# POSTECH-CVLab/PyTorch-StudioGAN

Hardware: AMD Instinct MI355X
Metric: images/sec (G+D step) BigGAN ImageNet-128 bs256 (higher is better)
Workload: dtype bf16

## Files before the change

### include/sgamd.h

```cpp
#ifndef SGAMD_H
#define SGAMD_H
#include <stdint.h>
#ifdef __cplusplus
extern "C" {
#endif

typedef void* sg_stream_t;

#define SG_DTYPE_F32 0
#define SG_DTYPE_BF16 1
#define SG_DTYPE_F64 2

#define SG_PIX_RELU 1
#define SG_PIX_UPSAMPLE 2
#define SG_PIX_QUAD 4
#define SG_PIX_TRANSPOSED 8
#define SG_EPI_OUT_F32 1
#define SG_EPI_ATOMIC 2
#define SG_EPI_POOL 4
#define SG_EPI_RELU 8
#define SG_EPI_RES_F32 16

const char* sg_last_error(void);
int sg_version(void);
int sg_prof_enable(int on);
int sg_prof_collect(double* out, int nkinds);

typedef struct {
  int dtype;
  int N, Hs, Ws, C, ldx;
  int Ho, Wo, Cout;
  int R, S, stride, pad_h, pad_w;
  int pix_flags, epi_flags;
  float alpha, beta;
  const void* x; const void* w;
  const float* bias; const void* res; const void* mask; void* out; const float* alpha_ptr;
  int ldo, ldr, ldm;
} sg_conv_fwd_desc;
int sg_conv2d_fwd(const sg_conv_fwd_desc* d, sg_stream_t stream);
int sg_set_f32_mode(int mode);
int sg_get_f32_mode(void);
long long sg_f32_split_launches(int mode);

typedef struct {
  sg_conv_fwd_desc main;
  const void* x2; const void* w2; const float* bias2;
  int C2, ldx2, x2_up;
  float* stats;
} sg_conv_skip_desc;
int sg_conv2d_fwd_skip_stat_rows(const sg_conv_skip_desc* d);
int sg_conv2d_fwd_skip(const sg_conv_skip_desc* d, sg_stream_t stream);
int sg_conv2d_fwd_skip_ok(const sg_conv_skip_desc* d);
long long sg_conv_rs_launches(void);

#define SG_Q_POOL 0
#define SG_Q_UP 1
typedef struct {
  int dtype, form;
  int N, Hl, Wl;
  int C, ldx, Cout;
  int pix_flags, epi_flags;
  float alpha, beta;
  const void* x; const void* wq;
  const float* bias; const void* res; const void* mask; void* out; const float* alpha_ptr;
  int ldo, ldr, ldm;
  const void* x2; const void* w2q; const float* bias2;
  int C2, ldx2;
  float* stats;
  int x2_norelu;
} sg_convq_desc;
int sg_conv2d_q_stat_rows(const sg_convq_desc* d);
int sg_conv2d_q(const sg_convq_desc* d, sg_stream_t stream);
int sg_conv2d_q_ok(const sg_convq_desc* d);
int sg_quad_pack(int dtype, int mode, const void* src, void* dst, int M, int Cs, sg_stream_t stream);
typedef struct { const void* src; void* dst; int M, Cs, mode, pad_; } sg_quad_item;
int sg_quad_pack_batch(int dtype, const sg_quad_item* items_dev, const sg_quad_item* items_host, int n, sg_stream_t stream);
typedef struct {
  int dtype, form;
  int N, Hl, Wl;
  int C, ldx, x_flags;
  int Cout, ldg;
  float alpha; const float* alpha_ptr;
  const void* x; const void* dy; float* dw; float* dbias;
  float* work; long long work_floats;
  int splits;
} sg_convq_wgrad_desc;
int sg_conv2d_q_wgrad_plan(const sg_convq_wgrad_desc* d, int* splits, long long* work_floats);
int sg_conv2d_q_wgrad(const sg_convq_wgrad_desc* d, sg_stream_t stream);
int sg_prof_collect_ex(double* out, int nkinds);
int sg_prof_collect_tags(double* out, int ntags);

typedef struct {
  int dtype;
  int N;
  int xHs, xWs, C, ldx, x_flags;
  int gHs, gWs, Cout, ldg, g_flags;
  int Ho, Wo;
  int R, S, stride, pad_h, pad_w;
  float alpha;
  const void* x; const void* dy; float* dw;
  const float* alpha_ptr;
  int splits;
  int no_tr;
  float* work; long long work_floats;
  float* dbias;
} sg_conv_wgrad_desc;
int sg_conv2d_wgrad(const sg_conv_wgrad_desc* d, sg_stream_t stream);
int sg_conv2d_wgrad_fuses_bias(const sg_conv_wgrad_desc* d);
int sg_conv2d_wgrad_plan(const sg_conv_wgrad_desc* d, int* splits, long long* work_floats);

typedef struct {
  int dtype, p_form, q_form;
  int I, J, K, batch;
  const void* p; long long p_bstride; int ldp;
  const void* q; long long q_bstride; int ldq;
  void* out; long long out_bstride; int ldo;
  const float* bias; const void* res; long long res_bstride; int ldr; float beta;
  float alpha; const float* alpha_ptr;
  int epi_flags; int splits; int no_tr;
} sg_gemm_desc;
int sg_gemm(const sg_gemm_desc* d, sg_stream_t stream);
typedef struct { const float* w; const float* y; const float* bias; float* out; int rows, K, ldy, ldo; } sg_linear_item;
int sg_linear_group(const sg_linear_item* items_dev, const sg_linear_item* items_host, int n, int B, sg_stream_t stream);

int sg_nchw_to_nhwc(int dtype, const float* src, void* dst, int N, int C, int H, int W, int ldo, sg_stream_t s);
int sg_nhwc_to_nchw(int dtype, const void* src, float* dst, int N, int C, int H, int W, int lds, int apply_tanh, sg_stream_t s);
int sg_nchw_grad_to_nhwc(int dtype, const float* dy, const float* y, void* dst, int N, int C, int H, int W, int ldo, int apply_tanh, sg_stream_t s);
int sg_avgpool2_fwd(int dtype, const void* x, void* y, int N, int H, int W, int C, sg_stream_t s);
int sg_avgpool2_bwd(int dtype, const void* dy, void* dx, int N, int H, int W, int C, sg_stream_t s);
int sg_maxpool2_fwd(int dtype, const void* x, int ldx, void* y, int ldy, uint8_t* idx, int N, int H, int W, int C, sg_stream_t s);
int sg_maxpool2_bwd(int dtype, const void* dy, int ldy, const uint8_t* idx, void* dx, int ldx, int N, int H, int W, int C, sg_stream_t s);
int sg_softmax_rows(int dtype, const float* s_in, void* p_out, long long rows, int cols, sg_stream_t st);
int sg_softmax_rows_bwd(int dtype, const void* p, const float* dp, void* ds, long long rows, int cols, sg_stream_t st);
int sg_convert(int src_dtype, int dst_dtype, const void* x, void* y, long long n, sg_stream_t s);
int sg_add_relu(int dtype, const void* a, const void* x, void* out, long long n, sg_stream_t s);
int sg_relu_mask(int dtype, const void* dy, const void* x, void* dx, long long n, sg_stream_t s);
int sg_axpby(int dtype, const void* x, void* y, long long n, float a, float b, sg_stream_t s);
int sg_dot(int dtype, const void* x, const void* y, long long n, float* out, float scale, const float* scale_ptr, sg_stream_t s);
int sg_colsum(int dtype, const void* x, int ldx, const void* mask, int ldm, long long rows, int C, float* out, float alpha, sg_stream_t s);

int sg_bn_partial_stats(int dtype, const void* x, int ldx, long long rows, int C, double* partial, sg_stream_t s);
int sg_bn_stats_from_tiles(const float* stats, int nrows, int C, double* partial, sg_stream_t s);
int sg_bn_finalize(const double* partial, double count, int C, float eps, float momentum, float* mean, float* invstd,
                   float* running_mean, float* running_var, sg_stream_t s);
typedef void* sg_comm_t;
int sg_comm_unique_id(void* out128);
int sg_comm_init_rank(const void* id128, int nranks, int rank, sg_comm_t* comm);
int sg_comm_size(sg_comm_t comm, int* nranks);
int sg_comm_destroy(sg_comm_t comm);
int sg_allreduce_flat(sg_comm_t comm, void* buf, long long count, int dtype, sg_stream_t s);
int sg_bn_stats_sync(int dtype, const void* x, int ldx, long long rows, int C, double* partial, sg_comm_t comm, float eps, float momentum,
                     float* mean, float* invstd, float* running_mean, float* running_var, sg_stream_t s);
int sg_reduce_scatter_flat(sg_comm_t comm, float* buf, long long per_rank, sg_stream_t s);
int sg_allgather_flat(sg_comm_t comm, float* buf, long long per_rank, sg_stream_t s);

typedef void* sg_p2p_t;
int sg_p2p_create(int world, int rank, long long max_doubles, sg_p2p_t* out, void* handle_out64);
int sg_p2p_connect(sg_p2p_t p, const void* handles);
int sg_p2p_destroy(sg_p2p_t p);
int sg_p2p_timeouts(sg_p2p_t p, int* count);
int sg_p2p_allreduce_f64(sg_p2p_t p, double* buf, int n, sg_stream_t s);
int sg_bn_finalize_p2p(sg_p2p_t p, const double* partial, double count, int C, float eps, float momentum, float* mean, float* invstd,
                       float* running_mean, float* running_var, sg_stream_t s);
int sg_bn_stats_sync_p2p(int dtype, const void* x, int ldx, long long rows, int C, double* partial, sg_p2p_t p, float eps, float momentum,
                         float* mean, float* invstd, float* running_mean, float* running_var, sg_stream_t s);
int sg_bn_from_running(const float* running_mean, const float* running_var, int C, float eps, float* mean, float* invstd, sg_stream_t s);
int sg_bn_apply(int dtype, const void* x, void* y, int N, long long HW, int C, const float* mean, const float* invstd,
                const float* gain, const float* bias, int gb_stride_n, int relu, sg_stream_t s);
int sg_bn_bwd_reduce(int dtype, const void* x, const void* dy, int N, long long HW, int C, const float* mean, const float* invstd,
                     const float* gain, const float* bias, int gb_stride_n, int relu, float* sums, sg_stream_t s);
int sg_bn_bwd_finalize(const float* sums, int N, int C, const float* gain, int gb_stride_n, float* dgain, float* dbias,
                       double* chan, sg_stream_t s);
int sg_bn_bwd_apply(int dtype, const void* x, const void* dy, void* dx, int N, long long HW, int C, const float* mean,
                    const float* invstd, const float* gain, const float* bias, int gb_stride_n, int relu,
                    const double* chan, double count, int use_batch_stats, sg_stream_t s);
int sg_bn_bwd_apply_res(int dtype, const void* x, const void* dy, void* dx, int N, long long HW, int C, const float* mean,
                        const float* invstd, const float* gain, const float* bias, int gb_stride_n, int relu,
                        const double* chan, double count, int use_batch_stats, const void* res, sg_stream_t s);

int sg_bn_bwd2_reduce(int dtype, const void* x, const void* dy, const void* u, int N, long long HW, int C, const float* mean,
                      const float* invstd, const float* gain, const float* bias, int relu, float* sums, sg_stream_t s);
int sg_bn_bwd2_finalize(const float* sums, int N, int C, double* chan, sg_stream_t s);
int sg_bn_bwd2_dgain(const double* chan_local, const double* chan, double count, const float* invstd, int C,
                     int use_batch_stats, float* dgain, sg_stream_t s);
int sg_bn_bwd2_apply(int dtype, const void* x, const void* dy, const void* u, void* g_dy, void* g_x, int N, long long HW, int C,
                     const float* mean, const float* invstd, const float* gain, const float* bias, int relu, const double* chan,
                     double count, int use_batch_stats, sg_stream_t s);

typedef struct {
  const float* w;
  float* u; float* v;
  float* sigma;
  float* u_snap; float* v_snap;
  void* w_fwd;
  void* w_dgrad;
  float* w_f32;
  int rows, cols;
  int Cin, RS;
  int do_power_iter;
  int apply_sn;
  int rows_pad;
  long long work_off;
  int trans;
  int dgrad_noflip;
  int Cin_pad;
} sg_sn_layer;
int sg_sn_forward(int dtype, const sg_sn_layer* layers_dev, const sg_sn_layer* layers_host, int n, float eps, float* work, long long work_floats, sg_stream_t s);

typedef struct {
  const float* dwt;
  const float* w;
  const float* u; const float* v; const float* sigma;
  float* dw;
  int rows, cols, Cin, RS, natural, apply_sn, trans;
  int Cin_pad;
} sg_sn_bwd_layer;
int sg_sn_backward(const sg_sn_bwd_layer* layers_dev, const sg_sn_bwd_layer* layers_host, int n, float* work, long long work_floats, sg_stream_t s);

int sg_embedding_fwd(const float* table, const int64_t* idx, float* out, int B, int dim, int num, sg_stream_t s);
int sg_embedding_bwd(const float* dout, const int64_t* idx, float* dtable, int B, int dim, int num, sg_stream_t s);
int sg_relu_sum_hw_fwd(int dtype, const void* x, float* h, int B, int HW, int C, sg_stream_t s);
int sg_relu_sum_hw_bwd(int dtype, const void* x, const float* dh, void* dx, int B, int HW, int C, sg_stream_t s);
int sg_pd_head_fwd(const float* h, const float* w1, const float* b1, const float* emb, float* adv, int B, int C, sg_stream_t s);
int sg_pd_head_bwd(const float* h, const float* w1, const float* emb, const float* dadv, float* dh, float* dw1, float* db1,
                   float* demb, int B, int C, sg_stream_t s);
int sg_loss_d(int kind, const float* real, const float* fake, int B, float* loss, float* d_real, float* d_fake, sg_stream_t s);
int sg_loss_g(int kind, const float* fake, int B, float* loss, float* d_fake, sg_stream_t s);

int sg_interp_rows(const float* real, const float* fake, const float* alpha, float* out, int B, long long n, sg_stream_t s);
int sg_gp_fwd(int kind, const float* grads, int B, long long n, float* norms, float* loss, sg_stream_t s);
int sg_gp_bwd(int kind, const float* grads, const float* norms, const float* gout, float* dgrads, int B, long long n, sg_stream_t s);
int sg_masked_sum_hw(int dtype, const void* t, const void* x, float* out, int B, int HW, int C, sg_stream_t s);

int sg_attn_fwd_flash_ok(int B, int HW, int HW4, int Dp, int Cg);
int sg_attn_fwd_fused(const void* theta, const void* phi, const void* g, float* lse, void* O, float* O32, int B, int HW, int HW4, int Dp, int Cg, sg_stream_t s);
int sg_attn_bwd_fused_ok(int B, int HW, int HW4, int Dp, int Cg);
int sg_attn_bwd_fused(const void* theta, const void* phi, const void* g, const void* dO, const float* O32, const float* lse, float* delta, void* dtheta, void* dphi,
                      void* dg, int B, int HW, int HW4, int Dp, int Cg, sg_stream_t s);

int sg_attn_proj_ok(int B, int H, int W, int C, int ldx, int Dp, int Cg);
int sg_attn_proj_fwd(const void* x, int ldx, const void* w_theta, const void* w_phi, const void* w_g, void* theta, void* phi, void* g,
                     uint8_t* idx_phi, uint8_t* idx_g, int B, int H, int W, int C, int Dp, int Cg, int relu, sg_stream_t s);
int sg_attn_proj_bwd_data(const void* dtheta, const void* dphi, const void* dg, const uint8_t* idx_phi, const uint8_t* idx_g, const void* wd_theta,
                          const void* wd_phi, const void* wd_g, const void* res, void* dx, int B, int H, int W, int C, int Dp, int Cg, sg_stream_t s);

int sg_slice_up_fwd(int dtype, const void* x, void* y, int N, int Hs, int Ws, int ldx, int C, int up, sg_stream_t s);
int sg_slice_up_bwd(int dtype, const void* dy, void* dx, int N, int Hs, int Ws, int ldx, int C, int up, sg_stream_t s);
int sg_copy_channels(int dtype, const void* src, int ld_src, void* dst, int ld_dst, long long rows, int C, sg_stream_t s);

int sg_adam_ema(float* p, const float* g, float* m, float* v, float* ema, long long n, float lr, float beta1, float beta2,
                float eps, float wd, int step, float ema_decay, float grad_scale, sg_stream_t s);
int sg_ema_lerp(const float* src, float* ema, long long n, float decay, sg_stream_t s);

int sg_lecam(const float* real, const float* fake, int B, float ema_real, float ema_fake, float* loss, float* d_real, float* d_fake, sg_stream_t s);
int sg_u8_to_nhwc(int dtype, const uint8_t* x, const uint8_t* flip, void* y, int N, int H, int W, int cpad, sg_stream_t s);

int sg_quantize_resize_normalize(int dtype, const float* x, void* out, uint8_t* quant_out, int N, int C, int H, int W,
                                 int OH, int OW, int quantize, sg_stream_t s);
int sg_quantize_resize_normalize_ms(int dtype, const float* x, void* out, uint8_t* quant_out, int N, int C, int H, int W,
                                    int OH, int OW, int quantize, const float* mean, const float* std, sg_stream_t s);
int sg_pool2d(int dtype, const void* x, void* y, int N, int H, int W, int C, int k, int stride, int pad, int mode, int ldy, int c_off, sg_stream_t s);
int sg_pil_resize_normalize(int dtype, const float* x, void* out, float* tmp, int N, int C, int H, int W, int OH, int OW,
                            const int* bounds_h, const double* kk_h, int ksize_h, const int* bounds_v, const double* kk_v, int ksize_v,
                            int quantize, sg_stream_t s);
int sg_pil_resize_normalize_ms(int dtype, const float* x, void* out, float* tmp, int N, int C, int H, int W, int OH, int OW,
                               const int* bounds_h, const double* kk_h, int ksize_h, const int* bounds_v, const double* kk_v, int ksize_v,
                               int quantize, const float* mean, const float* std, sg_stream_t s);
int sg_global_avgpool(int dtype, const void* x, float* y, int N, int HW, int C, sg_stream_t s);
int sg_topk_hits(const float* scores, int ld, int ncls, const int64_t* labels, int k, int N, uint8_t* hits, sg_stream_t s);
int sg_topk_select(const float* x, int n, int k, float* vals, int* idx, sg_stream_t s);
int sg_topk_scatter(const float* g, const int* idx, int k, float* dx, int n, sg_stream_t s);
int sg_feat_moments_accumulate(const float* f, int n, int C, double* sum_f, double* sum_ff, sg_stream_t s);
int sg_gather_images_u8(const uint8_t* src, const int64_t* idx, const uint8_t* flip, uint8_t* dst, int B, int H, int W,
                        const int64_t* lab_src, int64_t* lab_dst, sg_stream_t s);
int sg_row_normalize_fwd(const float* x, float* y, float* inv, int rows, int cols, float eps, sg_stream_t s);
int sg_row_normalize_bwd(const float* y, const float* inv, const float* dy, float* dx, int rows, int cols, sg_stream_t s);
int sg_row_dot(const float* a, const float* b, float* p, int rows, int cols, sg_stream_t s);
int sg_row_scale(const float* g, const float* x, float* out, int rows, int cols, int accumulate, sg_stream_t s);
int sg_class_loss(int kind, const float* z, const int64_t* label, int rows, int cols, float* row_loss, float* loss, float* dz, sg_stream_t s);
int sg_contrastive_loss(int kind, const float* S, const float* p, const int64_t* label, int B, float temperature, float m_p,
                        float* row_loss, float* loss, float* dS, float* dp, sg_stream_t s);
int sg_gather_cols(const float* z, const int64_t* label, int rows, int cols, float* out, sg_stream_t s);
int sg_scatter_cols(const float* g, const int64_t* label, int rows, int cols, float* dz, sg_stream_t s);
int sg_layernorm_rows(int out_dtype, const float* x, long long pitch, const float* gamma, const float* beta, void* y, long long ldo, int rows, int C,
                      float eps, sg_stream_t s);
int sg_vit_tokens(const float* patch, const float* cls, const float* pos, float* x, int B, int N, int C, sg_stream_t s);
int sg_gelu_f32(const float* x, float* y, long long n, sg_stream_t s);
int sg_tok_gemm(int epi, const void* a, int lda, const void* w, const float* bias, void* out, int ldo, int M, int N, int K, sg_stream_t s);
int sg_mha_fwd_ok(int B, int N, int H, int D);
int sg_mha_fwd(const void* qkv, void* out, int B, int N, int H, int D, float scale, sg_stream_t s);
long long sg_tok_gemm_launches(void);
long long sg_mha_launches(void);

int sg_row_sqnorm(const float* f, int n, int C, float* sq, sg_stream_t s);
int sg_kth_smallest_rows(const float* D, long long ld, int rows, int cols, int k, const float* row_add, float* out, sg_stream_t s);
int sg_prdc_rows(const float* D, long long ld, int rows, int cols, const float* row_add, const float* r2_row, const float* r2_col,
                 int* col_cnt, uint8_t* row_any, float* row_min, sg_stream_t s);
int sg_chol_lower(double* A, int n, int* flag, sg_stream_t s);
int sg_dgemm_tn(const double* A, const double* B, double* C, int n, sg_stream_t s);
int sg_jacobi_sweep(double* M, int n, double* offd, sg_stream_t s);
int sg_row_norm_sum(const double* M, int n, double* out, sg_stream_t s);

int sg_bias_act(int dtype, const void* x, const void* b, const void* xref, const void* yref, const void* dy, void* y, long long n,
                long long step_b, int size_b, int grad, int act, float alpha, float gain, float clamp, sg_stream_t s);
int sg_upfirdn2d(int dtype, const void* x, const float* f, void* y, int planes, int H, int W, int fh, int fw, int upx, int upy,
                 int downx, int downy, int padx0, int padx1, int pady0, int pady1, int flip_filter, float gain, sg_stream_t s);
int sg_filtered_lrelu(int dtype, const void* x, const float* fu, const float* fd, const void* b, void* y, int N, int C, int H, int W,
                      int fu_n, int fd_n, int up, int down, int px0, int px1, int py0, int py1, float gain, float slope, float clamp,
                      int flip_filter, sg_stream_t s);

#define SG_AUG_BRIGHTNESS 1
#define SG_AUG_SATURATION 2
#define SG_AUG_CONTRAST 4
#define SG_AUG_FLIP 8
#define SG_AUG_TRANSLATE 16
#define SG_AUG_TRANSLATE_REFLECT 32
#define SG_AUG_CUTOUT 64
typedef struct {
  int N, C, H, W;
  int ops;
  int cut_h, cut_w;
  int max_t;
  const float* color;
  const int* geom;
} sg_aug_desc;
int sg_augment_work_floats(const sg_aug_desc* d);
int sg_augment_fwd(const sg_aug_desc* d, const float* x, float* y, float* work, sg_stream_t s);
int sg_augment_bwd(const sg_aug_desc* d, const float* dy, float* dx, float* work, sg_stream_t s);
int sg_mse_work_floats(void);
int sg_mse_fwd(const float* a, const float* b, long long n, float* work, float* loss, sg_stream_t s);
int sg_mse_bwd(const float* a, const float* b, const float* gout, long long n, float* da, float* db, sg_stream_t s);
int sg_loss_ls_d(const float* real, const float* fake, int B, float* loss, float* d_real, float* d_fake, sg_stream_t s);
int sg_loss_ls_g(const float* fake, int B, float* loss, float* d_fake, sg_stream_t s);
int sg_fm_work_floats(int C);
int sg_fm_loss(const float* real_h, const float* fake_h, int B, int C, float* work, float* loss, float* d_fake, sg_stream_t s);
int sg_exp_fwd(const float* x, float* y, long long n, sg_stream_t s);
int sg_exp_bwd(const float* dy, const float* y, float* dx, long long n, sg_stream_t s);
int sg_normal_nll(const float* x, const float* mu, const float* var, int B, int K, float* loss, float* dmu, float* dvar, sg_stream_t s);
int sg_maxpool2_gather(int dtype, const void* x, int ldx, const uint8_t* idx, void* y, int ldy, int N, int H, int W, int C, sg_stream_t s);
int sg_softmax_rows_bwd2(const float* P, const float* dP, const float* u, float* gP, long long rows, int cols, sg_stream_t s);
int sg_scale_by_ptr(int dtype, const void* x, const float* sigma, void* y, long long n, sg_stream_t s);
int sg_tanh_bwd(const float* dy, const float* y, float* t, long long n, sg_stream_t s);
int sg_tanh_bwd2(const float* g, const float* dy, const float* y, float* out, long long n, sg_stream_t s);
int sg_clamp_flat(float* p, long long n, float lo, float hi, sg_stream_t s);
int sg_select_rows(const uint8_t* flag, const float* a, const float* b, float* out, int N, long long row, sg_stream_t s);
int sg_sign_count(const float* logit, int B, float* acc, sg_stream_t s);
int sg_reflect_pad2d_fwd(const float* x, float* y, int planes, int H, int W, int l, int r, int t, int b, sg_stream_t s);
int sg_reflect_pad2d_bwd(const float* dy, float* dx, int planes, int H, int W, int l, int r, int t, int b, sg_stream_t s);
int sg_affine_sample_fwd(const float* x, const float* theta, float* y, int N, int C, int Hi, int Wi, int Ho, int Wo, sg_stream_t s);
int sg_affine_sample_bwd(const float* dy, const float* theta, float* dx, int N, int C, int Hi, int Wi, int Ho, int Wo, sg_stream_t s);
int sg_color_affine(const float* x, const float* M, float* y, int N, int C, int HW, int transpose, sg_stream_t s);
int sg_fir_reflect(const float* x, const float* taps, float* y, int N, int C, int H, int W, int T, int axis, int transpose, sg_stream_t s);
int sg_ada_noise_cutout(const float* x, const float* noise, const float* sigma, const float* cut, float* y, int N, int C, int H, int W, sg_stream_t s);

#ifdef __cplusplus
}
#endif
#endif
```

### pytorch-studiogan_amd/_lib.py

```python
import ctypes as C
import os
import subprocess
import sys

import torch

_HERE = os.path.dirname(os.path.abspath(__file__))
LIB_PATH = os.path.join(_HERE, "libsgamd.so")
if os.environ.get("SG_LIBSGAMD"):
    LIB_PATH = os.path.abspath(os.environ["SG_LIBSGAMD"])
CSRC = os.path.join(_HERE, "csrc")

F32, BF16, F64 = 0, 1, 2
PIX_RELU, PIX_UPSAMPLE, PIX_QUAD, PIX_TRANSPOSED = 1, 2, 4, 8
Q_POOL, Q_UP = 0, 1
EPI_OUT_F32, EPI_ATOMIC, EPI_POOL, EPI_RELU, EPI_RES_F32 = 1, 2, 4, 8, 16

_vp, _i, _f, _ll = C.c_void_p, C.c_int, C.c_float, C.c_longlong


class ConvFwdDesc(C.Structure):
    _fields_ = [("dtype", _i), ("N", _i), ("Hs", _i), ("Ws", _i), ("C", _i), ("ldx", _i), ("Ho", _i), ("Wo", _i), ("Cout", _i),
                ("R", _i), ("S", _i), ("stride", _i), ("pad_h", _i), ("pad_w", _i), ("pix_flags", _i), ("epi_flags", _i),
                ("alpha", _f), ("beta", _f), ("x", _vp), ("w", _vp), ("bias", _vp), ("res", _vp), ("mask", _vp), ("out", _vp),
                ("alpha_ptr", _vp), ("ldo", _i), ("ldr", _i), ("ldm", _i)]


class ConvSkipDesc(C.Structure):
    _fields_ = [("main", ConvFwdDesc), ("x2", _vp), ("w2", _vp), ("bias2", _vp), ("C2", _i), ("ldx2", _i), ("x2_up", _i), ("stats", _vp)]


class ConvWgradDesc(C.Structure):
    _fields_ = [("dtype", _i), ("N", _i), ("xHs", _i), ("xWs", _i), ("C", _i), ("ldx", _i), ("x_flags", _i), ("gHs", _i), ("gWs", _i),
                ("Cout", _i), ("ldg", _i), ("g_flags", _i), ("Ho", _i), ("Wo", _i), ("R", _i), ("S", _i), ("stride", _i),
                ("pad_h", _i), ("pad_w", _i), ("alpha", _f), ("x", _vp), ("dy", _vp), ("dw", _vp), ("alpha_ptr", _vp),
                ("splits", _i), ("no_tr", _i), ("work", _vp), ("work_floats", _ll), ("dbias", _vp)]


class ConvQDesc(C.Structure):
    _fields_ = [("dtype", _i), ("form", _i), ("N", _i), ("Hl", _i), ("Wl", _i), ("C", _i), ("ldx", _i), ("Cout", _i),
                ("pix_flags", _i), ("epi_flags", _i), ("alpha", _f), ("beta", _f), ("x", _vp), ("wq", _vp), ("bias", _vp), ("res", _vp),
                ("mask", _vp), ("out", _vp), ("alpha_ptr", _vp), ("ldo", _i), ("ldr", _i), ("ldm", _i),
                ("x2", _vp), ("w2q", _vp), ("bias2", _vp), ("C2", _i), ("ldx2", _i), ("stats", _vp), ("x2_norelu", _i)]


class ConvQWgradDesc(C.Structure):
    _fields_ = [("dtype", _i), ("form", _i), ("N", _i), ("Hl", _i), ("Wl", _i), ("C", _i), ("ldx", _i), ("x_flags", _i), ("Cout", _i),
                ("ldg", _i), ("alpha", _f), ("alpha_ptr", _vp), ("x", _vp), ("dy", _vp), ("dw", _vp), ("dbias", _vp), ("work", _vp),
                ("work_floats", _ll), ("splits", _i)]


class QuadItem(C.Structure):
    _fields_ = [("src", _vp), ("dst", _vp), ("M", _i), ("Cs", _i), ("mode", _i), ("pad_", _i)]


class LinearItem(C.Structure):
    _fields_ = [("w", _vp), ("y", _vp), ("bias", _vp), ("out", _vp), ("rows", _i), ("K", _i), ("ldy", _i), ("ldo", _i)]


class GemmDesc(C.Structure):
    _fields_ = [("dtype", _i), ("p_form", _i), ("q_form", _i), ("I", _i), ("J", _i), ("K", _i), ("batch", _i),
                ("p", _vp), ("p_bstride", _ll), ("ldp", _i), ("q", _vp), ("q_bstride", _ll), ("ldq", _i),
                ("out", _vp), ("out_bstride", _ll), ("ldo", _i), ("bias", _vp), ("res", _vp), ("res_bstride", _ll), ("ldr", _i),
                ("beta", _f), ("alpha", _f), ("alpha_ptr", _vp), ("epi_flags", _i), ("splits", _i), ("no_tr", _i)]


class SnLayer(C.Structure):
    _fields_ = [("w", _vp), ("u", _vp), ("v", _vp), ("sigma", _vp), ("u_snap", _vp), ("v_snap", _vp), ("w_fwd", _vp), ("w_dgrad", _vp),
                ("w_f32", _vp), ("rows", _i), ("cols", _i), ("Cin", _i), ("RS", _i), ("do_power_iter", _i), ("apply_sn", _i),
                ("rows_pad", _i), ("work_off", _ll), ("trans", _i), ("dgrad_noflip", _i), ("Cin_pad", _i)]


class SnBwdLayer(C.Structure):
    _fields_ = [("dwt", _vp), ("w", _vp), ("u", _vp), ("v", _vp), ("sigma", _vp), ("dw", _vp), ("rows", _i), ("cols", _i),
                ("Cin", _i), ("RS", _i), ("natural", _i), ("apply_sn", _i), ("trans", _i), ("Cin_pad", _i)]


class AugDesc(C.Structure):
    _fields_ = [("N", _i), ("C", _i), ("H", _i), ("W", _i), ("ops", _i), ("cut_h", _i), ("cut_w", _i), ("max_t", _i), ("color", _vp), ("geom", _vp)]


AUG_BRIGHTNESS, AUG_SATURATION, AUG_CONTRAST, AUG_FLIP, AUG_TRANSLATE, AUG_TRANSLATE_REFLECT, AUG_CUTOUT = 1, 2, 4, 8, 16, 32, 64

_lib = None


def build(force=False, verbose=False):
    cmd = ["make", "-C", CSRC, "-j", str(max(2, os.cpu_count() or 2))]
    if force:
        subprocess.run(["make", "-C", CSRC, "clean"], check=True, stdout=subprocess.DEVNULL)
    res = subprocess.run(cmd, stdout=subprocess.PIPE, stderr=subprocess.STDOUT, text=True)
    if verbose or res.returncode != 0:
        sys.stderr.write(res.stdout)
    if res.returncode != 0:
        raise RuntimeError("building libsgamd.so failed")
    return LIB_PATH


_PROTOS = {
    "sg_prof_enable": [_i],
    "sg_prof_collect": [C.POINTER(C.c_double), _i],
    "sg_conv2d_fwd": [C.POINTER(ConvFwdDesc), _vp],
    "sg_conv2d_fwd_skip": [C.POINTER(ConvSkipDesc), _vp],
    "sg_conv2d_fwd_skip_ok": [C.POINTER(ConvSkipDesc)],
    "sg_conv_rs_launches": [],
    "sg_conv2d_q": [C.POINTER(ConvQDesc), _vp],
    "sg_conv2d_q_ok": [C.POINTER(ConvQDesc)],
    "sg_conv2d_q_stat_rows": [C.POINTER(ConvQDesc)],
    "sg_conv2d_fwd_skip_stat_rows": [C.POINTER(ConvSkipDesc)],
    "sg_bn_stats_from_tiles": [_vp, _i, _i, _vp, _vp],
    "sg_quad_pack": [_i, _i, _vp, _vp, _i, _i, _vp],
    "sg_quad_pack_batch": [_i, _vp, C.POINTER(QuadItem), _i, _vp],
    "sg_linear_group": [_vp, C.POINTER(LinearItem), _i, _i, _vp],
    "sg_conv2d_q_wgrad_plan": [C.POINTER(ConvQWgradDesc), C.POINTER(_i), C.POINTER(_ll)],
    "sg_conv2d_q_wgrad": [C.POINTER(ConvQWgradDesc), _vp],
    "sg_prof_collect_ex": [C.POINTER(C.c_double), _i],
    "sg_prof_collect_tags": [C.POINTER(C.c_double), _i],
    "sg_conv2d_wgrad": [C.POINTER(ConvWgradDesc), _vp],
    "sg_conv2d_wgrad_plan": [C.POINTER(ConvWgradDesc), C.POINTER(_i), C.POINTER(_ll)],
    "sg_conv2d_wgrad_fuses_bias": [C.POINTER(ConvWgradDesc)],
    "sg_gemm": [C.POINTER(GemmDesc), _vp],
    "sg_nchw_to_nhwc": [_i, _vp, _vp, _i, _i, _i, _i, _i, _vp],
    "sg_nhwc_to_nchw": [_i, _vp, _vp, _i, _i, _i, _i, _i, _i, _vp],
    "sg_nchw_grad_to_nhwc": [_i, _vp, _vp, _vp, _i, _i, _i, _i, _i, _i, _vp],
    "sg_avgpool2_fwd": [_i, _vp, _vp, _i, _i, _i, _i, _vp],
    "sg_avgpool2_bwd": [_i, _vp, _vp, _i, _i, _i, _i, _vp],
    "sg_maxpool2_fwd": [_i, _vp, _i, _vp, _i, _vp, _i, _i, _i, _i, _vp],
    "sg_maxpool2_bwd": [_i, _vp, _i, _vp, _vp, _i, _i, _i, _i, _i, _vp],
    "sg_softmax_rows": [_i, _vp, _vp, _ll, _i, _vp],
    "sg_softmax_rows_bwd": [_i, _vp, _vp, _vp, _ll, _i, _vp],
    "sg_axpby": [_i, _vp, _vp, _ll, _f, _f, _vp],
    "sg_convert": [_i, _i, _vp, _vp, _ll, _vp],
    "sg_add_relu": [_i, _vp, _vp, _vp, _ll, _vp],
    "sg_relu_mask": [_i, _vp, _vp, _vp, _ll, _vp],
    "sg_dot": [_i, _vp, _vp, _ll, _vp, _f, _vp, _vp],
    "sg_colsum": [_i, _vp, _i, _vp, _i, _ll, _i, _vp, _f, _vp],
    "sg_bn_partial_stats": [_i, _vp, _i, _ll, _i, _vp, _vp],
    "sg_bn_finalize": [_vp, C.c_double, _i, _f, _f, _vp, _vp, _vp, _vp, _vp],
    "sg_comm_unique_id": [_vp],
    "sg_comm_init_rank": [_vp, _i, _i, C.POINTER(_vp)],
    "sg_comm_size": [_vp, C.POINTER(_i)],
    "sg_comm_destroy": [_vp],
    "sg_allreduce_flat": [_vp, _vp, _ll, _i, _vp],
    "sg_bn_stats_sync": [_i, _vp, _i, _ll, _i, _vp, _vp, _f, _f, _vp, _vp, _vp, _vp, _vp],
    "sg_set_f32_mode": [_i],
    "sg_get_f32_mode": [],
    "sg_f32_split_launches": [_i],
    "sg_reduce_scatter_flat": [_vp, _vp, _ll, _vp],
    "sg_allgather_flat": [_vp, _vp, _ll, _vp],
    "sg_p2p_create": [_i, _i, _ll, C.POINTER(_vp), _vp],
    "sg_p2p_connect": [_vp, _vp],
    "sg_p2p_destroy": [_vp],
    "sg_p2p_timeouts": [_vp, C.POINTER(_i)],
    "sg_p2p_allreduce_f64": [_vp, _vp, _i, _vp],
    "sg_bn_finalize_p2p": [_vp, _vp, C.c_double, _i, _f, _f, _vp, _vp, _vp, _vp, _vp],
    "sg_bn_stats_sync_p2p": [_i, _vp, _i, _ll, _i, _vp, _vp, _f, _f, _vp, _vp, _vp, _vp, _vp],
    "sg_bn_from_running": [_vp, _vp, _i, _f, _vp, _vp, _vp],
    "sg_bn_apply": [_i, _vp, _vp, _i, _ll, _i, _vp, _vp, _vp, _vp, _i, _i, _vp],
    "sg_bn_bwd_reduce": [_i, _vp, _vp, _i, _ll, _i, _vp, _vp, _vp, _vp, _i, _i, _vp, _vp],
    "sg_bn_bwd_finalize": [_vp, _i, _i, _vp, _i, _vp, _vp, _vp, _vp],
    "sg_bn_bwd_apply": [_i, _vp, _vp, _vp, _i, _ll, _i, _vp, _vp, _vp, _vp, _i, _i, _vp, C.c_double, _i, _vp],
    "sg_bn_bwd_apply_res": [_i, _vp, _vp, _vp, _i, _ll, _i, _vp, _vp, _vp, _vp, _i, _i, _vp, C.c_double, _i, _vp, _vp],
    "sg_bn_bwd2_reduce": [_i, _vp, _vp, _vp, _i, _ll, _i, _vp, _vp, _vp, _vp, _i, _vp, _vp],
    "sg_bn_bwd2_finalize": [_vp, _i, _i, _vp, _vp],
    "sg_bn_bwd2_dgain": [_vp, _vp, C.c_double, _vp, _i, _i, _vp, _vp],
    "sg_bn_bwd2_apply": [_i, _vp, _vp, _vp, _vp, _vp, _i, _ll, _i, _vp, _vp, _vp, _vp, _i, _vp, C.c_double, _i, _vp],
    "sg_attn_fwd_flash_ok": [_i, _i, _i, _i, _i],
    "sg_attn_fwd_fused": [_vp, _vp, _vp, _vp, _vp, _vp, _i, _i, _i, _i, _i, _vp],
    "sg_attn_bwd_fused_ok": [_i, _i, _i, _i, _i],
    "sg_attn_bwd_fused": [_vp, _vp, _vp, _vp, _vp, _vp, _vp, _vp, _vp, _vp, _i, _i, _i, _i, _i, _vp],
    "sg_attn_proj_ok": [_i, _i, _i, _i, _i, _i, _i],
    "sg_attn_proj_fwd": [_vp, _i, _vp, _vp, _vp, _vp, _vp, _vp, _vp, _vp, _i, _i, _i, _i, _i, _i, _i, _vp],
    "sg_attn_proj_bwd_data": [_vp, _vp, _vp, _vp, _vp, _vp, _vp, _vp, _vp, _vp, _i, _i, _i, _i, _i, _i, _vp],
    "sg_slice_up_fwd": [_i, _vp, _vp, _i, _i, _i, _i, _i, _i, _vp],
    "sg_slice_up_bwd": [_i, _vp, _vp, _i, _i, _i, _i, _i, _i, _vp],
    "sg_copy_channels": [_i, _vp, _i, _vp, _i, _ll, _i, _vp],
    "sg_interp_rows": [_vp, _vp, _vp, _vp, _i, _ll, _vp],
    "sg_gp_fwd": [_i, _vp, _i, _ll, _vp, _vp, _vp],
    "sg_gp_bwd": [_i, _vp, _vp, _vp, _vp, _i, _ll, _vp],
    "sg_masked_sum_hw": [_i, _vp, _vp, _vp, _i, _i, _i, _vp],
    "sg_sn_forward": [_i, _vp, C.POINTER(SnLayer), _i, _f, _vp, _ll, _vp],
    "sg_sn_backward": [_vp, C.POINTER(SnBwdLayer), _i, _vp, _ll, _vp],
    "sg_embedding_fwd": [_vp, _vp, _vp, _i, _i, _i, _vp],
    "sg_embedding_bwd": [_vp, _vp, _vp, _i, _i, _i, _vp],
    "sg_relu_sum_hw_fwd": [_i, _vp, _vp, _i, _i, _i, _vp],
    "sg_relu_sum_hw_bwd": [_i, _vp, _vp, _vp, _i, _i, _i, _vp],
    "sg_pd_head_fwd": [_vp, _vp, _vp, _vp, _vp, _i, _i, _vp],
    "sg_pd_head_bwd": [_vp, _vp, _vp, _vp, _vp, _vp, _vp, _vp, _i, _i, _vp],
    "sg_loss_d": [_i, _vp, _vp, _i, _vp, _vp, _vp, _vp],
    "sg_loss_g": [_i, _vp, _i, _vp, _vp, _vp],
    "sg_adam_ema": [_vp, _vp, _vp, _vp, _vp, _ll, _f, _f, _f, _f, _f, _i, _f, _f, _vp],
    "sg_ema_lerp": [_vp, _vp, _ll, _f, _vp],
    "sg_quantize_resize_normalize": [_i, _vp, _vp, _vp, _i, _i, _i, _i, _i, _i, _i, _vp],
    "sg_pil_resize_normalize": [_i, _vp, _vp, _vp, _i, _i, _i, _i, _i, _i, _vp, _vp, _i, _vp, _vp, _i, _i, _vp],
    "sg_quantize_resize_normalize_ms": [_i, _vp, _vp, _vp, _i, _i, _i, _i, _i, _i, _i, C.POINTER(_f), C.POINTER(_f), _vp],
    "sg_pil_resize_normalize_ms": [_i, _vp, _vp, _vp, _i, _i, _i, _i, _i, _i, _vp, _vp, _i, _vp, _vp, _i, _i, C.POINTER(_f), C.POINTER(_f), _vp],
    "sg_layernorm_rows": [_i, _vp, _ll, _vp, _vp, _vp, _ll, _i, _i, _f, _vp],
    "sg_vit_tokens": [_vp, _vp, _vp, _vp, _i, _i, _i, _vp],
    "sg_gelu_f32": [_vp, _vp, _ll, _vp],
    "sg_tok_gemm": [_i, _vp, _i, _vp, _vp, _vp, _i, _i, _i, _i, _vp],
    "sg_mha_fwd_ok": [_i, _i, _i, _i],
    "sg_mha_fwd": [_vp, _vp, _i, _i, _i, _i, _f, _vp],
    "sg_tok_gemm_launches": [],
    "sg_mha_launches": [],
    "sg_pool2d": [_i, _vp, _vp, _i, _i, _i, _i, _i, _i, _i, _i, _i, _i, _vp],
    "sg_global_avgpool": [_i, _vp, _vp, _i, _i, _i, _vp],
    "sg_feat_moments_accumulate": [_vp, _i, _i, _vp, _vp, _vp],
    "sg_topk_hits": [_vp, _i, _i, _vp, _i, _i, _vp, _vp],
    "sg_row_normalize_fwd": [_vp, _vp, _vp, _i, _i, _f, _vp],
    "sg_row_normalize_bwd": [_vp, _vp, _vp, _vp, _i, _i, _vp],
    "sg_row_dot": [_vp, _vp, _vp, _i, _i, _vp],
    "sg_row_scale": [_vp, _vp, _vp, _i, _i, _i, _vp],
    "sg_class_loss": [_i, _vp, _vp, _i, _i, _vp, _vp, _vp, _vp],
    "sg_contrastive_loss": [_i, _vp, _vp, _vp, _i, _f, _f, _vp, _vp, _vp, _vp, _vp],
    "sg_gather_cols": [_vp, _vp, _i, _i, _vp, _vp],
    "sg_scatter_cols": [_vp, _vp, _i, _i, _vp, _vp],
    "sg_chol_lower": [_vp, _i, _vp, _vp],
    "sg_dgemm_tn": [_vp, _vp, _vp, _i, _vp],
    "sg_jacobi_sweep": [_vp, _i, _vp, _vp],
    "sg_row_norm_sum": [_vp, _i, _vp, _vp],
    "sg_row_sqnorm": [_vp, _i, _i, _vp, _vp],
    "sg_kth_smallest_rows": [_vp, _ll, _i, _i, _i, _vp, _vp, _vp],
    "sg_prdc_rows": [_vp, _ll, _i, _i, _vp, _vp, _vp, _vp, _vp, _vp, _vp],
    "sg_topk_select": [_vp, _i, _i, _vp, _vp, _vp],
    "sg_lecam": [_vp, _vp, _i, _f, _f, _vp, _vp, _vp, _vp],
    "sg_u8_to_nhwc": [_i, _vp, _vp, _vp, _i, _i, _i, _i, _vp],
    "sg_gather_images_u8": [_vp, _vp, _vp, _vp, _i, _i, _i, _vp, _vp, _vp],
    "sg_topk_scatter": [_vp, _vp, _i, _vp, _i, _vp],
    "sg_bias_act": [_i, _vp, _vp, _vp, _vp, _vp, _vp, _ll, _ll, _i, _i, _i, _f, _f, _f, _vp],
    "sg_upfirdn2d": [_i, _vp, _vp, _vp, _i, _i, _i, _i, _i, _i, _i, _i, _i, _i, _i, _i, _i, _i, _f, _vp],
    "sg_filtered_lrelu": [_i, _vp, _vp, _vp, _vp, _vp, _i, _i, _i, _i, _i, _i, _i, _i, _i, _i, _i, _i, _f, _f, _f, _i, _vp],
    "sg_augment_work_floats": [C.POINTER(AugDesc)],
    "sg_augment_fwd": [C.POINTER(AugDesc), _vp, _vp, _vp, _vp],
    "sg_augment_bwd": [C.POINTER(AugDesc), _vp, _vp, _vp, _vp],
    "sg_mse_work_floats": [],
    "sg_mse_fwd": [_vp, _vp, _ll, _vp, _vp, _vp],
    "sg_mse_bwd": [_vp, _vp, _vp, _ll, _vp, _vp, _vp],
    "sg_loss_ls_d": [_vp, _vp, _i, _vp, _vp, _vp, _vp],
    "sg_loss_ls_g": [_vp, _i, _vp, _vp, _vp],
    "sg_fm_work_floats": [_i],
    "sg_fm_loss": [_vp, _vp, _i, _i, _vp, _vp, _vp, _vp],
    "sg_exp_fwd": [_vp, _vp, _ll, _vp],
    "sg_exp_bwd": [_vp, _vp, _vp, _ll, _vp],
    "sg_normal_nll": [_vp, _vp, _vp, _i, _i, _vp, _vp, _vp, _vp],
    "sg_maxpool2_gather": [_i, _vp, _i, _vp, _vp, _i, _i, _i, _i, _i, _vp],
    "sg_softmax_rows_bwd2": [_vp, _vp, _vp, _vp, _ll, _i, _vp],
    "sg_scale_by_ptr": [_i, _vp, _vp, _vp, _ll, _vp],
    "sg_tanh_bwd": [_vp, _vp, _vp, _ll, _vp],
    "sg_tanh_bwd2": [_vp, _vp, _vp, _vp, _ll, _vp],
    "sg_clamp_flat": [_vp, _ll, _f, _f, _vp],
    "sg_select_rows": [_vp, _vp, _vp, _vp, _i, _ll, _vp],
    "sg_sign_count": [_vp, _i, _vp, _vp],
    "sg_reflect_pad2d_fwd": [_vp, _vp, _i, _i, _i, _i, _i, _i, _i, _vp],
    "sg_reflect_pad2d_bwd": [_vp, _vp, _i, _i, _i, _i, _i, _i, _i, _vp],
    "sg_affine_sample_fwd": [_vp, _vp, _vp, _i, _i, _i, _i, _i, _i, _vp],
    "sg_affine_sample_bwd": [_vp, _vp, _vp, _i, _i, _i, _i, _i, _i, _vp],
    "sg_color_affine": [_vp, _vp, _vp, _i, _i, _i, _i, _vp],
    "sg_fir_reflect": [_vp, _vp, _vp, _i, _i, _i, _i, _i, _i, _i, _vp],
    "sg_ada_noise_cutout": [_vp, _vp, _vp, _vp, _vp, _i, _i, _i, _i, _vp],
}


def exported_symbols():
    return sorted(list(_PROTOS.keys()) + ["sg_last_error", "sg_version"])


def lib():
    global _lib
    if _lib is None:
        if not os.path.exists(LIB_PATH):
            raise RuntimeError(
                f"{LIB_PATH} is missing: run `python -c 'import __graft_entry__ as g; g.build()'` (make -C {CSRC}). "
                "There is no CPU/eager fallback on the product path.")
        l = C.CDLL(LIB_PATH)
        l.sg_last_error.restype = C.c_char_p
        l.sg_version.restype = _i
        for name, args in _PROTOS.items():
            fn = getattr(l, name)
            fn.argtypes = args
            fn.restype = _i
        l.sg_conv_rs_launches.restype = _ll
        l.sg_tok_gemm_launches.restype = _ll
        l.sg_mha_launches.restype = _ll
        l.sg_f32_split_launches.restype = _ll
        f32_mode = {"bf16x3": 3, "bf16x6": 6}.get(os.environ.get("SG_F32_MODE", "exact"), 0)
        if f32_mode:
            l.sg_set_f32_mode(f32_mode)
        _lib = l
    return _lib


def check(rc, name=""):
    if rc != 0:
        raise RuntimeError(f"{name}: {lib().sg_last_error().decode()} (rc={rc})")


_STATE_WRITERS = frozenset(("sg_adam_ema", "sg_ema_lerp", "sg_allreduce_flat", "sg_clamp_flat", "sg_allgather_flat"))
write_epoch = [0]


def call(name, *args):
    if name in _STATE_WRITERS:
        write_epoch[0] += 1
    rc = getattr(lib(), name)(*args)
    if rc != 0:
        raise RuntimeError(f"{name}: {lib().sg_last_error().decode()} (rc={rc})")


def stream():
    return torch.cuda.current_stream().cuda_stream


def upload_bytes(raw, device):
    t = torch.frombuffer(bytearray(raw), dtype=torch.uint8)
    if torch.device(device).type == "cuda":
        return t.pin_memory().to(device, non_blocking=True)
    return t.to(device)


def dt(t):
    d = t if isinstance(t, torch.dtype) else t.dtype
    if d == torch.float32:
        return F32
    if d == torch.bfloat16:
        return BF16
    raise RuntimeError(f"unsupported dtype {d} (float32 / bfloat16 only)")


def require_gpu(dev):
    if dev.type != "cuda":
        raise RuntimeError("studiogan_amd modules run on the GPU only (no CPU fallback on the product path)")


def ptr(t):
    if t is None:
        return None
    if not t.is_cuda:
        raise RuntimeError("studiogan_amd kernels need a GPU tensor (no CPU fallback on the product path)")
    return t.data_ptr()
```

### pytorch-studiogan_amd/csrc/conv.hip

```cpp
#include <type_traits>
#include "conv_common.h"
#include "conv_v2.h"

int g_sg_f32_mode = 0;
long long g_sg_f32_split_launches[2] = {0, 0};
extern "C" int sg_set_f32_mode(int mode) {
  SG_CHECK(mode == 0 || mode == 3 || mode == 6, "sg_set_f32_mode: 0 (exact fp32 MFMA), 3 (bf16x3 split) or 6 (bf16x6 split)");
  g_sg_f32_mode = mode;
  return 0;
}
extern "C" int sg_get_f32_mode() { return g_sg_f32_mode; }
extern "C" long long sg_f32_split_launches(int mode) {
  if (mode != 3 && mode != 6) return -1;
  return __atomic_load_n(&g_sg_f32_split_launches[mode == 6], __ATOMIC_RELAXED);
}

template <typename T, class LP, class LQ, int SPLIT>
static void conv_fwd_tiles(const LP& lp, const LQ& lq, const Epilogue<T>& e, int I, int J, int K, hipStream_t st) {
  if (I <= 32) sg_launch_gemm<T, LP, LQ, 32, 256, 1, 4, true, SPLIT>(lp, lq, e, I, J, K, 1, 1, st);
  else if (I % 128 != 0 && (I % 96 == 0 || (I < 128 && I > 64))) sg_launch_gemm<T, LP, LQ, 96, 256, 1, 4, true, SPLIT>(lp, lq, e, I, J, K, 1, 1, st);
  else sg_launch_gemm<T, LP, LQ, 128, 128, 2, 2, true, SPLIT>(lp, lq, e, I, J, K, 1, 1, st);
}

template <typename T, bool FAST>
static void conv_fwd_launch(const sg_conv_fwd_desc* d, const Epilogue<T>& e, int I, int J, int K, int pflags, hipStream_t st) {
  typedef StridedKC<T, FAST> LP;
  typedef ConvPixKC<T, FAST> LQ;
  LP lp;
  lp.base = (const T*)d->w; lp.bstride = 0; lp.ld = K; lp.rows = I; lp.K = K;
  lp.vec_ok = (K % ET<T>::VEC == 0) && aligned16(d->w);
  LQ lq;
  fill_geom<T>(lq.g, d->x, d->N, d->Hs, d->Ws, d->C, d->ldx, d->Ho, d->Wo, d->R, d->S, d->stride, d->pad_h, d->pad_w, pflags);
  lq.rows = J; lq.K = K;
  if constexpr (sizeof(T) == 4 && FAST) {
    const int mode = g_sg_f32_mode;
    if (mode == 3) { sg_f32_split_count(3); return conv_fwd_tiles<T, LP, LQ, 3>(lp, lq, e, I, J, K, st); }
    if (mode == 6) { sg_f32_split_count(6); return conv_fwd_tiles<T, LP, LQ, 6>(lp, lq, e, I, J, K, st); }
  }
  conv_fwd_tiles<T, LP, LQ, 0>(lp, lq, e, I, J, K, st);
}

static bool conv_fwd_v2_try(const ConvFwdProblem& pb, hipStream_t st) {
  const sg_conv_fwd_desc* d = pb.d;
  const int I = pb.I, J = pb.J, K = pb.K, pflags = pb.pflags;
  const char mode = env_mode("SG_CONV_V2");
  const bool force = mode == 'f';
  if (mode == '0' || (pflags & SG_PIX_TRANSPOSED)) return false;
  if (d->stride != 1 && (d->stride != 2 || (pflags & (SG_PIX_UPSAMPLE | SG_PIX_QUAD)))) return false;
  if (d->C % 8 || d->ldx % 8 || d->R * d->S > 25 || J < 256) return false;
  if (pb.xbytes >= (1ll << 31) || pb.wbytes >= (1ll << 30)) return false;
  if (!aligned16(d->x) || !aligned16(d->w)) return false;
  if (!epi_bf16_rows_ok(pb.e)) return false;
  const int tj = (J + 255) / 256;
  int best_tiles = 0;
  int best = cout_tile_search(I, tj, best_tiles);
  if (!best && I % 8 == 0 && I >= 32) {
    int best_pad = 0;
    for (int c = 0; c < 3; c++) {
      const int padded = ((I + kCoutTiles[c] - 1) / kCoutTiles[c]) * kCoutTiles[c];
      if (2 * padded > 3 * I) continue;
      const int tiles = (padded / kCoutTiles[c]) * tj;
      if (!best || padded < best_pad) { best = kCoutTiles[c]; best_pad = padded; best_tiles = tiles; }
    }
  }
  int min_tiles = 160;
  if (const char* mt = getenv("SG_CONV_V2_MIN_TILES")) { const int v = atoi(mt); if (v > 0) min_tiles = v; }
  if (!best || (best_tiles < min_tiles && !force)) return false;
  ConvV2Params p;
  p.x = (const bf16_t*)d->x; p.w = (const bf16_t*)d->w;
  p.N = d->N; p.Hs = d->Hs; p.Ws = d->Ws; p.C = d->C; p.ldx = d->ldx;
  p.Hin = d->Hs * (pb.up ? 2 : 1); p.Win = d->Ws * (pb.up ? 2 : 1); p.Ho = d->Ho; p.Wo = d->Wo;
  p.R = d->R; p.S = d->S; p.pad_h = d->pad_h; p.pad_w = d->pad_w; p.flags = pflags; p.stride = d->stride;
  p.I = I; p.J = J; p.K = K; p.cpt = d->C / 8; p.ntap = d->R * d->S;
  p.wshift = pb.wshift; p.hshift = pb.hshift;
  p.xbytes = (unsigned)pb.xbytes; p.wbytes = (unsigned)pb.wbytes;
  const Epilogue<bf16_t>& e = pb.e;
  int rc = 0;
  if (best == 192) rc = sg_launch_conv_v2<192, 4, 2, 256, 7>(p, e, st);
  else if (best == 128) rc = sg_launch_conv_v2<128, 4, 2, 256, 7>(p, e, st);
  else {
    if (J >= 512 * 256) rc = sg_launch_conv_v2<96, 8, 1, 512, 1>(p, e, st);
    else rc = sg_launch_conv_v2<96, 8, 1, 256, 1>(p, e, st);
  }
  return rc == 0;
}

template <typename T> static int conv_fwd_t(const sg_conv_fwd_desc* d, hipStream_t st) {
  const int K = d->R * d->S * d->C;
  const int I = d->Cout;
  const long long Jll = (long long)d->N * d->Ho * d->Wo;
  SG_CHECK(Jll < (1ll << 31), "sg_conv2d_fwd: too many output pixels");
  SG_CHECK((long long)d->N * d->Hs * d->Ws * d->ldx < (1ll << 31), "sg_conv2d_fwd: input tensor too large for 32-bit element offsets");
  const int J = (int)Jll;
  int pflags = d->pix_flags;
  if (d->epi_flags & SG_EPI_POOL) {
    SG_CHECK((d->Ho % 2 == 0) && (d->Wo % 2 == 0), "sg_conv2d_fwd: pooled output needs even Ho, Wo");
    pflags |= SG_PIX_QUAD;
  } else {
    pflags &= ~SG_PIX_QUAD;
  }
  const bool w_vec = (K % ET<T>::VEC == 0) && aligned16(d->w);
  const bool x_vec = (d->C % ET<T>::VEC == 0) && (d->ldx % ET<T>::VEC == 0) && aligned16(d->x);
  const Epilogue<T> e = make_epilogue<T>(d, I, J);
  const int prof = sg_prof_begin(st, 2.0 * (double)I * (double)J * (double)K, 0);
  int eng = SG_ENG_CONV_GEMM;
  if constexpr (std::is_same_v<T, bf16_t>) {
    if (w_vec && x_vec) {
      const ConvFwdProblem pb = conv_fwd_problem(d, e, I, J, K, pflags);
      if (sg_conv_fwd_sk_try(pb, st)) eng = SG_ENG_CONV_SK;
      else if (sg_conv_fwd_rs_try(pb, st)) eng = SG_ENG_CONV_RS;
      else if (sg_conv_fwd_v4_try(pb, st)) eng = SG_ENG_CONV_V4;
      else if (sg_conv_fwd_v3_try(pb, st)) eng = SG_ENG_CONV_V3;
      else if (conv_fwd_v2_try(pb, st)) eng = SG_ENG_CONV_V2;
    }
  }
  if (eng == SG_ENG_CONV_GEMM) {
    if (w_vec && x_vec) conv_fwd_launch<T, true>(d, e, I, J, K, pflags, st);
    else conv_fwd_launch<T, false>(d, e, I, J, K, pflags, st);
  }
  {
    const double es = sizeof(T), jout = (d->epi_flags & SG_EPI_POOL) ? (double)J / 4.0 : (double)J;
    const double b = es * ((double)d->N * d->Hs * d->Ws * d->C + (double)I * K + jout * I * (1.0 + (d->mask ? 1.0 : 0.0) + (d->res ? 1.0 : 0.0)));
    sg_prof_tag(prof, eng, b);
  }
  sg_prof_end(st, prof);
  SG_LAUNCH_CHECK();
  return 0;
}

static int conv_fwd_skip(const sg_conv_skip_desc* sk, hipStream_t st, bool dry) {
  const sg_conv_fwd_desc* d = &sk->main;
  if (d->dtype != SG_DTYPE_BF16 || d->R != 3 || d->S != 3 || d->stride != 1 || (d->pix_flags & (SG_PIX_UPSAMPLE | SG_PIX_TRANSPOSED))) return 0;
  const int K = 9 * d->C, I = d->Cout;
  const long long Jll = (long long)d->N * d->Ho * d->Wo;
  if (Jll >= (1ll << 31) || (long long)d->N * d->Hs * d->Ws * d->ldx >= (1ll << 31)) return 0;
  const int J = (int)Jll;
  int pflags = d->pix_flags;
  if (d->epi_flags & SG_EPI_POOL) { if ((d->Ho & 1) || (d->Wo & 1)) return 0; pflags |= SG_PIX_QUAD; } else pflags &= ~SG_PIX_QUAD;
  const ConvFwdProblem pb = conv_fwd_problem(d, make_epilogue<bf16_t>(d, I, J), I, J, K, pflags);
  if (dry) return sg_conv_fwd_v4_skip_try(pb, sk, st, true) ? 1 : 0;
  const int prof = sg_prof_begin(st, 2.0 * (double)I * (double)J * ((double)K + (double)sk->C2), 0);
  const bool ok = sg_conv_fwd_v4_skip_try(pb, sk, st, false);
  {
    const double jout = (d->epi_flags & SG_EPI_POOL) ? (double)J / 4.0 : (double)J;
    const double x2 = (double)d->N * (sk->x2_up ? (d->Ho / 2) * (d->Wo / 2) : d->Ho * d->Wo) * sk->C2;
    sg_prof_tag(prof, SG_ENG_CONV_V4_SKIP, 2.0 * ((double)d->N * d->Hs * d->Ws * d->C + x2 + (double)I * (K + sk->C2) + jout * I));
  }
  sg_prof_end(st, prof);
  return ok ? 1 : 0;
}
extern "C" int sg_conv2d_fwd_skip_stat_rows(const sg_conv_skip_desc* d) {
  if (!d) return 0;
  const long long J = (long long)d->main.N * d->main.Ho * d->main.Wo;
  return (int)((J + 255) / 256);
}
extern "C" int sg_conv2d_fwd_skip_ok(const sg_conv_skip_desc* d) {
  if (!d || !d->main.x || !d->main.w || !d->main.out || !d->x2 || !d->w2) return 0;
  return conv_fwd_skip(d, nullptr, true);
}
extern "C" int sg_conv2d_fwd_skip(const sg_conv_skip_desc* d, sg_stream_t stream) {
  SG_CHECK(d && d->main.x && d->main.w && d->main.out && d->x2 && d->w2, "sg_conv2d_fwd_skip: null pointer");
  SG_CHECK(conv_fwd_skip(d, (hipStream_t)stream, false) == 1, "sg_conv2d_fwd_skip: problem not eligible for the fused kernel (ask sg_conv2d_fwd_skip_ok first)");
  SG_LAUNCH_CHECK();
  return 0;
}

extern "C" int sg_conv2d_fwd(const sg_conv_fwd_desc* d, sg_stream_t stream) {
  SG_CHECK(d && d->x && d->w && d->out, "sg_conv2d_fwd: null pointer");
  SG_CHECK(d->N > 0 && d->C > 0 && d->Cout > 0 && d->R > 0 && d->S > 0 && d->stride > 0, "sg_conv2d_fwd: bad shape");
  SG_CHECK(!(d->epi_flags & SG_EPI_ATOMIC), "sg_conv2d_fwd: atomic epilogue not supported");
  if (d->dtype == SG_DTYPE_F32) return conv_fwd_t<float>(d, (hipStream_t)stream);
  if (d->dtype == SG_DTYPE_BF16) return conv_fwd_t<bf16_t>(d, (hipStream_t)stream);
  sg_set_error("sg_conv2d_fwd: bad dtype");
  return -1;
}
```

### pytorch-studiogan_amd/csrc/conv_common.h

```cpp
#pragma once
#include <stdlib.h>
#include "gemm_core.h"
#include "../../include/sgamd.h"

static inline int ilog2_exact(int v) {
  if (v <= 0 || (v & (v - 1))) return -1;
  int s = 0;
  while ((1 << s) < v) s++;
  return s;
}
static inline bool aligned16(const void* p) { return (((uintptr_t)p) & 15) == 0; }

template <typename T>
static void fill_geom(PixGeom<T>& g, const void* x, int N, int Hs, int Ws, int C, int ldx, int Ho, int Wo, int R, int S,
                      int stride, int pad_h, int pad_w, int flags) {
  g.x = (const T*)x; g.N = N; g.Hs = Hs; g.Ws = Ws;
  const int up = (flags & SG_PIX_UPSAMPLE) ? 2 : 1;
  g.Hin = Hs * up; g.Win = Ws * up; g.C = C; g.ldx = ldx; g.Ho = Ho; g.Wo = Wo;
  g.R = R; g.S = S; g.stride = stride; g.pad_h = pad_h; g.pad_w = pad_w; g.flags = flags;
  g.vec_ok = (C % ET<T>::VEC == 0) && (ldx % ET<T>::VEC == 0) && aligned16(x);
  g.wshift = ilog2_exact(Wo); g.hshift = ilog2_exact(Ho);
}

static inline char env_mode(const char* name) { const char* m = getenv(name); return m ? m[0] : 0; }

static inline long long bf16_extent(long long npix, int ld, int C) { return ((npix - 1) * ld + C) * 2; }

template <typename D> static inline bool is_3x3_s1_p1(const D* d) { return d->R == 3 && d->S == 3 && d->stride == 1 && d->pad_h == 1 && d->pad_w == 1; }

static inline int cout_blocks(int Cout) { return Cout % 96 == 0 ? 3 : Cout % 64 == 0 ? 2 : 0; }

static const int kCoutTiles[3] = {192, 128, 96};
static inline int cout_tile_search(int I, int tj, int& best_tiles) {
  int best = 0;
  best_tiles = 0;
  for (int c = 0; c < 3; c++) {
    if (I % kCoutTiles[c]) continue;
    const int tiles = (I / kCoutTiles[c]) * tj;
    if (tiles >= 512) { best = kCoutTiles[c]; best_tiles = tiles; break; }
    if (tiles > best_tiles) { best = kCoutTiles[c]; best_tiles = tiles; }
  }
  return best;
}

template <typename T, typename D> static Epilogue<T> make_epilogue(const D* d, int I, int J) {
  Epilogue<T> e;
  e.out = d->out; e.out_bstride = 0; e.ldo = d->ldo; e.bias = d->bias;
  e.res = d->res; e.res_bstride = 0; e.ldr = d->ldr; e.beta = d->beta;
  e.mask = (const T*)d->mask; e.mask_bstride = 0; e.ldm = d->ldm; e.split_stride = 0;
  e.alpha = d->alpha; e.alpha_ptr = d->alpha_ptr; e.flags = d->epi_flags; e.I = I; e.J = J;
  return e;
}
static inline bool epi_bf16_rows_ok(const Epilogue<bf16_t>& e) {
  if ((e.flags & (SG_EPI_ATOMIC | SG_EPI_OUT_F32)) || (e.ldo & 7) || !aligned16(e.out)) return false;
  if (e.mask && ((e.ldm & 7) || !aligned16(e.mask))) return false;
  if (e.res && ((e.flags & SG_EPI_RES_F32) || (e.ldr & 7) || !aligned16(e.res))) return false;
  return true;
}

struct ConvFwdProblem {
  const sg_conv_fwd_desc* d;
  Epilogue<bf16_t> e;
  int I, J, K, pflags;
  bool up, quad;
  int wshift, hshift;
  long long xbytes, wbytes;
  bool out_is_in_times_up() const { return d->Ho == d->Hs * (up ? 2 : 1) && d->Wo == d->Ws * (up ? 2 : 1); }
};
static inline ConvFwdProblem conv_fwd_problem(const sg_conv_fwd_desc* d, const Epilogue<bf16_t>& e, int I, int J, int K, int pflags) {
  ConvFwdProblem pb;
  pb.d = d; pb.e = e; pb.I = I; pb.J = J; pb.K = K; pb.pflags = pflags;
  pb.up = (pflags & SG_PIX_UPSAMPLE) != 0; pb.quad = (pflags & SG_PIX_QUAD) != 0;
  pb.wshift = ilog2_exact(d->Wo); pb.hshift = ilog2_exact(d->Ho);
  pb.xbytes = bf16_extent((long long)d->N * d->Hs * d->Ws, d->ldx, d->C); pb.wbytes = (long long)I * K * 2;
  return pb;
}

bool sg_conv_fwd_sk_try(const ConvFwdProblem& pb, hipStream_t st);
bool sg_conv_fwd_rs_try(const ConvFwdProblem& pb, hipStream_t st);
bool sg_conv_fwd_v4_try(const ConvFwdProblem& pb, hipStream_t st);
bool sg_conv_fwd_v3_try(const ConvFwdProblem& pb, hipStream_t st);
bool sg_conv_fwd_v4_skip_try(const ConvFwdProblem& pb, const sg_conv_skip_desc* sk, hipStream_t st, bool dry);
```

### pytorch-studiogan_amd/csrc/conv_v2.h

```cpp
#pragma once
#include "gemm_core.h"

struct ConvV2Params {
  const bf16_t* x; const bf16_t* w;
  int N, Hs, Ws, C, ldx;
  int Hin, Win, Ho, Wo;
  int R, S, pad_h, pad_w;
  int stride;
  int flags;
  int I, J, K;
  int cpt;
  int ntap;
  unsigned xbytes, wbytes;
  int wshift, hshift;
};

typedef __attribute__((address_space(1))) const void* sg_gptr_t;
typedef __attribute__((address_space(3))) void* sg_lptr_t;

template <int BI, int BJ, int NW, int TI, int TJ, bool VMAP = false, bool NOSTORE = false>
__device__ __forceinline__ void sg_conv_epilogue(f32x16 (&acc)[TI][TJ], char* smem, const float* sbias, const Epilogue<bf16_t>& epi,
                                                 int i0, int j0, int wi0, int wj0, float al, bool active = true, int vlog = 0, int vadd = 0,
                                                 float* stats = nullptr, int stats_C = 0, int stats_row = 0) {
  auto grow = [&](int jg) -> long long {
    if (VMAP) return (long long)(((jg >> vlog) << (vlog + 2)) + ((jg & ((1 << vlog) - 1)) << 1) + vadd);
    return (long long)jg;
  };
  const int tid = threadIdx.x, lane = tid & 63;
  const bool pool = (epi.flags & SG_EPI_POOL) != 0;
  constexpr int CP = BI * 2 + 16;
  __syncthreads();
  const int rows_out = pool ? BJ / 4 : BJ;
  const int jbase = pool ? (j0 >> 2) : j0, Jout = pool ? (epi.J >> 2) : epi.J;
  constexpr int CPR = BI / 8;
  const bool pre_mask = epi.mask != nullptr, pre_res = epi.res != nullptr;
  const bool pre_both = pre_mask && pre_res;
  const int ncr = ((epi.I - i0 < BI ? epi.I - i0 : BI) + 7) >> 3;
  auto stage_tile = [&](const bf16_t* src, int ld) {
    for (int idx = tid; idx < rows_out * CPR; idx += 64 * NW) {
      const int r = idx / CPR, c = idx - r * CPR;
      const int jg = jbase + r;
      u32x4 t = {0u, 0u, 0u, 0u};
      if (jg < Jout && c < ncr) t = *(const u32x4*)(src + grow(jg) * ld + i0 + c * 8);
      *(u32x4*)(smem + r * CP + c * 16) = t;
    }
  };
  uint32_t mbits[TI * TJ];
#pragma unroll
  for (int q = 0; q < TI * TJ; q++) mbits[q] = 0u;
  if (pre_both) {
    stage_tile(epi.mask, epi.ldm);
    __syncthreads();
    if (active) {
#pragma unroll
      for (int ta = 0; ta < TI; ta++)
#pragma unroll
        for (int tb = 0; tb < TJ; tb++) {
          const int jl = wj0 + tb * 32 + (lane & 31);
          const int jo = pool ? (jl >> 2) : jl;
          uint32_t bits = 0u;
#pragma unroll
          for (int g4 = 0; g4 < 4; g4++) {
            const int il = wi0 + ta * 32 + 8 * g4 + 4 * (lane >> 5);
            const u32x2 m = *(const u32x2*)(smem + jo * CP + il * 2);
#pragma unroll
            for (int e = 0; e < 4; e++) { const bf16_t h = (bf16_t)((m[e >> 1] >> (16 * (e & 1))) & 0xffffu); if (bf2f(h) > 0.f) bits |= 1u << (4 * g4 + e); }
          }
          mbits[ta * TJ + tb] = bits;
        }
    }
    __syncthreads();
    stage_tile((const bf16_t*)epi.res, epi.ldr);
    __syncthreads();
  } else if (pre_mask || pre_res) {
    stage_tile(pre_mask ? epi.mask : (const bf16_t*)epi.res, pre_mask ? epi.ldm : epi.ldr);
    __syncthreads();
  }
  const bool relu_out = (epi.flags & SG_EPI_RELU) != 0;
  if (active) {
#pragma unroll
  for (int ta = 0; ta < TI; ta++)
#pragma unroll
    for (int tb = 0; tb < TJ; tb++) {
      const int jl = wj0 + tb * 32 + (lane & 31);
#pragma unroll
      for (int g4 = 0; g4 < 4; g4++) {
        const int il = wi0 + ta * 32 + 8 * g4 + 4 * (lane >> 5);
        float v[4] = {acc[ta][tb][4 * g4 + 0], acc[ta][tb][4 * g4 + 1], acc[ta][tb][4 * g4 + 2], acc[ta][tb][4 * g4 + 3]};
        if (pool) {
#pragma unroll
          for (int e = 0; e < 4; e++) v[e] = quad_sum(v[e]);
        }
        const int jo = pool ? (jl >> 2) : jl;
        const bool act = (!pool || (lane & 3) == 0) && (jbase + jo < Jout);
        if (act) {
          char* loc = smem + jo * CP + il * 2;
#pragma unroll
          for (int e = 0; e < 4; e++) v[e] *= al;
          if (epi.bias) {
            const f32x4 b = *(const f32x4*)(sbias + il);
#pragma unroll
            for (int e = 0; e < 4; e++) v[e] += b[e];
          }
          if (pre_both) {
            const uint32_t bits = mbits[ta * TJ + tb] >> (4 * g4);
#pragma unroll
            for (int e = 0; e < 4; e++) if (!((bits >> e) & 1u)) v[e] = 0.f;
          } else if (pre_mask) {
            const u32x2 m = *(const u32x2*)loc;
#pragma unroll
            for (int e = 0; e < 4; e++) { const bf16_t h = (bf16_t)((m[e >> 1] >> (16 * (e & 1))) & 0xffffu); if (!(bf2f(h) > 0.f)) v[e] = 0.f; }
          }
          if (pre_res) {
            const u32x2 r = *(const u32x2*)loc;
#pragma unroll
            for (int e = 0; e < 4; e++) { const bf16_t h = (bf16_t)((r[e >> 1] >> (16 * (e & 1))) & 0xffffu); v[e] += epi.beta * bf2f(h); }
          }
          if (relu_out) {
#pragma unroll
            for (int e = 0; e < 4; e++) v[e] = fmaxf(v[e], 0.f);
          }
          u32x2 t;
          t[0] = pack2bf(v[0], v[1]);
          t[1] = pack2bf(v[2], v[3]);
          *(u32x2*)loc = t;
        }
      }
    }
  }
  __syncthreads();
  if (stats) {
    constexpr int PWV = BI / 2 / NW, RG = 64 / PWV;
    const int wv = tid >> 6, pl = lane % PWV, rg = lane / PWV;
    int rows_valid = Jout - jbase;
    if (rows_valid > rows_out) rows_valid = rows_out;
    float s1a = 0.f, s2a = 0.f, s1b = 0.f, s2b = 0.f;
    const int c2 = wv * PWV + pl;
    if (rg < RG) {
      constexpr int NIT = (BJ + RG - 1) / RG;
      const char* base = smem + rg * CP + c2 * 4;
#pragma unroll 8
      for (int k = 0; k < NIT; k++) {
        const int r = rg + k * RG;
        uint32_t v = *(const uint32_t*)(base + (r < BJ ? k * (RG * CP) : 0));
        v = r < rows_valid ? v : 0u;
        const float a = __uint_as_float(v << 16), b = __uint_as_float(v & 0xffff0000u);
        s1a += a; s2a += a * a; s1b += b; s2b += b * b;
      }
    }
    float t1a = s1a, t2a = s2a, t1b = s1b, t2b = s2b;
#pragma unroll
    for (int k = 1; k < RG; k++) {
      t1a += __shfl(s1a, lane + k * PWV, 64); t2a += __shfl(s2a, lane + k * PWV, 64);
      t1b += __shfl(s1b, lane + k * PWV, 64); t2b += __shfl(s2b, lane + k * PWV, 64);
    }
    const int c = i0 + 2 * c2;
    if (rg == 0 && c < epi.I) {
      f32x4 o4 = {t1a, t2a, t1b, t2b};
      *(f32x4*)(stats + ((long long)stats_row * stats_C + c) * 2) = o4;
    }
  }
  {
    bf16_t* o = (bf16_t*)epi.out;
    for (int idx = tid; idx < rows_out * CPR; idx += 64 * NW) {
      const int r = idx / CPR, c = idx - r * CPR;
      const int jg = jbase + r;
      if (NOSTORE) {
        const u32x4 v = *(const u32x4*)(smem + r * CP + c * 16);
        if (v[0] == 0x12345678u && v[1] == 0x9abcdef0u) *(u32x4*)(o + grow(jg) * epi.ldo + i0 + c * 8) = v;
      } else if (jg < Jout && c < ncr) *(u32x4*)(o + grow(jg) * epi.ldo + i0 + c * 8) = *(const u32x4*)(smem + r * CP + c * 16);
    }
  }
}

template <int BI, int WJ, int WI, int BJ, int SCHED, bool RELU, bool UP>
__global__ __launch_bounds__(64 * WJ * WI) void sg_conv_v2_kernel(ConvV2Params p, Epilogue<bf16_t> epi, int tilesI, int tilesJ) {
  constexpr int NW = WJ * WI;
  constexpr int QB = BJ * 128, PB = BI * 128, BUF = QB + PB;
  constexpr int NQ = BJ / 8 / NW;
  constexpr int NPI = (BI / 8 + NW - 1) / NW;
  constexpr int TJ = BJ / WJ / 32, TI = BI / WI / 32;
  static_assert(NW == 8 || NW == 4, "4 or 8 waves");
  static_assert(BJ % (8 * NW) == 0, "pixel tile / DMA groups");
  static_assert(BJ % (WJ * 32) == 0 && BI % (WI * 32) == 0, "tile/wave mismatch");
  extern __shared__ __attribute__((aligned(16))) char smem[];

  const int tid = threadIdx.x, lane = tid & 63;
  const int wave = __builtin_amdgcn_readfirstlane(tid >> 6);
  const int nt = tilesI * tilesJ;
  int bid = blockIdx.x;
  {
    const int xcd = bid & 7, q = nt >> 3, r = nt & 7;
    bid = (xcd < r ? xcd * (q + 1) : r * (q + 1) + (xcd - r) * q) + (bid >> 3);
  }
  const int tI = bid % tilesI, tJ = bid / tilesI;
  const int i0 = tI * BI, j0 = tJ * BJ;
  float* sbias = (float*)(smem + 2 * BUF);
  if (epi.bias) {
    for (int i = tid; i < BI; i += 64 * NW) sbias[i] = (i0 + i < epi.I) ? epi.bias[i0 + i] : 0.f;
  }

  const auto rsx = __builtin_amdgcn_make_buffer_rsrc((void*)p.x, 0, (int)p.xbytes, 0x00020000);
  const auto rsw = __builtin_amdgcn_make_buffer_rsrc((void*)p.w, 0, (int)p.wbytes, 0x00020000);
  const int sub = lane >> 3;
  const int lc = (lane & 7) ^ ((4 * wave + (lane >> 4)) & 7);
  const unsigned ldx2 = 2u * (unsigned)p.ldx;
  unsigned qoff[NQ];
  unsigned qinv[NQ];
  bool qph[NQ], qpw[NQ];
#pragma unroll
  for (int i = 0; i < NQ; i++) {
    const int row = j0 + 8 * (wave + NW * i) + sub;
    int n, ho, wo;
    if (p.flags & SG_PIX_QUAD) {
      const int q = row >> 2, dy = (row >> 1) & 1, dx = row & 1;
      const int Wq = p.Wo >> 1, Hq = p.Ho >> 1;
      int wq, hq;
      if (p.wshift >= 1 && p.hshift >= 1) { wq = q & (Wq - 1); const int t = q >> (p.wshift - 1); hq = t & (Hq - 1); n = t >> (p.hshift - 1); }
      else { wq = q % Wq; const int t = q / Wq; hq = t % Hq; n = t / Hq; }
      ho = 2 * hq + dy; wo = 2 * wq + dx;
    } else if (p.wshift >= 0 && p.hshift >= 0) {
      wo = row & (p.Wo - 1); const int t = row >> p.wshift; ho = t & (p.Ho - 1); n = t >> p.hshift;
    } else {
      wo = row % p.Wo; const int t = row / p.Wo; ho = t % p.Ho; n = t / p.Ho;
    }
    unsigned m = 0;
    if (row < p.J) {
      int t = 0;
      for (int rr = 0; rr < p.R; rr++) {
        const bool hok = (unsigned)(ho * p.stride - p.pad_h + rr) < (unsigned)p.Hin;
        for (int ss = 0; ss < p.S; ss++, t++)
          if (hok && (unsigned)(wo * p.stride - p.pad_w + ss) < (unsigned)p.Win) m |= 1u << t;
      }
    }
    qinv[i] = ~m;
    qph[i] = UP && (ho & 1); qpw[i] = UP && (wo & 1);
    const int hs = UP ? (ho >> 1) : ho * p.stride, ws = UP ? (wo >> 1) : wo * p.stride;
    qoff[i] = ((unsigned)(n * p.Hs + hs) * (unsigned)p.Ws + (unsigned)ws) * ldx2;
  }
  unsigned poff[NPI];
#pragma unroll
  for (int i = 0; i < NPI; i++) {
    const int g = wave + NW * i;
    const int row = i0 + 8 * g + sub;
    poff[i] = ((g < BI / 8) && (row < p.I)) ? (unsigned)row * (unsigned)p.K * 2u : 0x40000000u;
  }
  int q = lc, tap = lc / p.cpt, c8 = lc - tap * p.cpt, tr = tap / p.S, ts = tap - tr * p.S;

  unsigned kd0 = 0, kdh1 = 0, kdw1 = 0, kw = 0;
  auto position = [&]() {
    const int dr = tr - p.pad_h, ds = ts - p.pad_w;
    if (UP) {
      const unsigned rowb = (unsigned)p.Ws * ldx2;
      kd0 = (unsigned)(dr >> 1) * rowb + (unsigned)(ds >> 1) * ldx2 + (unsigned)c8 * 16u;
      kdh1 = ((unsigned)((dr + 1) >> 1) - (unsigned)(dr >> 1)) * rowb;
      kdw1 = ((unsigned)((ds + 1) >> 1) - (unsigned)(ds >> 1)) * ldx2;
    } else {
      kd0 = (unsigned)(dr * p.Ws + ds) * ldx2 + (unsigned)c8 * 16u;
    }
    kw = (tap < p.ntap) ? (unsigned)q * 16u : 0x40000000u;
  };
  position();

  auto piece = [&](int buf, int i) {
    char* qd = smem + buf * BUF;
    char* pd = qd + QB;
    if (i < NQ) {
      unsigned off = qoff[i] + kd0;
      if (UP) off += (qph[i] ? kdh1 : 0u) + (qpw[i] ? kdw1 : 0u);
      off |= ((qinv[i] >> tap) & 1u) << 31;
      __builtin_amdgcn_raw_ptr_buffer_load_lds(rsx, (sg_lptr_t)(qd + (wave + NW * i) * 1024), 16, (int)off, 0, 0, 0);
    } else {
      const int j = i - NQ;
      if (NW * (j + 1) <= BI / 8 || wave + NW * j < BI / 8) {
        __builtin_amdgcn_raw_ptr_buffer_load_lds(rsw, (sg_lptr_t)(pd + (wave + NW * j) * 1024), 16, (int)(poff[j] + kw), 0, 0, 0);
      }
    }
  };
  auto advance = [&]() {
    q += 8;
    if (p.cpt >= 8) {
      c8 += 8;
      const bool w = c8 >= p.cpt;
      c8 -= w ? p.cpt : 0;
      tap += w ? 1 : 0; ts += w ? 1 : 0;
      const bool w2 = ts == p.S;
      ts = w2 ? 0 : ts; tr += w2 ? 1 : 0;
    } else {
      tap = q / p.cpt; c8 = q - tap * p.cpt;
      tr = tap / p.S; ts = tap - tr * p.S;
    }
    position();
  };
  auto issue = [&](int buf) {
#pragma unroll
    for (int i = 0; i < NQ + NPI; i++) piece(buf, i);
    advance();
  };

  f32x16 acc[TI][TJ];
#pragma unroll
  for (int a = 0; a < TI; a++)
#pragma unroll
    for (int b = 0; b < TJ; b++)
#pragma unroll
      for (int r = 0; r < 16; r++) acc[a][b][r] = 0.f;

  const int wj = wave % WJ, wi = wave / WJ;
  const int wj0 = wj * (BJ / WJ), wi0 = wi * (BI / WI);
  const int frow = lane & 31, fhi = lane >> 5;

  const int nk = (SCHED == 5 || SCHED == 6) ? 1 : (p.K / 8 + 7) / 8;
  issue(0);
  __syncthreads();
  constexpr int NP = NQ + NPI, PPS = (NP + 3) / 4;
  for (int kt = 0; kt < nk; kt++) {
    const bool more = (SCHED == 2 || SCHED == 4) ? false : (kt + 1 < nk);
    if ((SCHED == 0 || SCHED == 3 || SCHED == 7) && more) issue((kt + 1) & 1);
    const char* qs = smem + (kt & 1) * BUF;
    const char* ps = qs + QB;
    const int krem = p.K - kt * 64;
    const int nks = krem >= 64 ? 4 : ((krem + 15) >> 4);
    if (SCHED == 7) {
      bf16x8_t pf[2][TI], qf[2][TJ];
      auto load = [&](int ks, int slot) {
#pragma unroll
        for (int a = 0; a < TI; a++) {
          const int row = wi0 + a * 32 + frow;
          const int ch = (ks * 2 + fhi) ^ ((row >> 1) & 7);
          u32x4 v = *(const u32x4*)(ps + row * 128 + ch * 16);
          pf[slot][a] = __builtin_bit_cast(bf16x8_t, v);
        }
#pragma unroll
        for (int b = 0; b < TJ; b++) {
          const int row = wj0 + b * 32 + frow;
          const int ch = (ks * 2 + fhi) ^ ((row >> 1) & 7);
          u32x4 v = *(const u32x4*)(qs + row * 128 + ch * 16);
          if (RELU) v = relu16<bf16_t>(v);
          qf[slot][b] = __builtin_bit_cast(bf16x8_t, v);
        }
      };
      load(0, 0);
#pragma unroll
      for (int ks = 0; ks < 4; ks++) {
        if (ks < 3 && __builtin_expect(ks + 1 < nks, 1)) load(ks + 1, (ks + 1) & 1);
        if (__builtin_expect(ks < nks, 1)) {
#pragma unroll
          for (int a = 0; a < TI; a++)
#pragma unroll
            for (int b = 0; b < TJ; b++)
              acc[a][b] = __builtin_amdgcn_mfma_f32_32x32x16_bf16(pf[ks & 1][a], qf[ks & 1][b], acc[a][b], 0, 0, 0);
        }
      }
    } else {
#pragma unroll
    for (int ks = 0; ks < 4; ks++) {
      bf16x8_t pf[TI], qf[TJ];
      if ((SCHED == 3 || SCHED == 4) && kt > 0) {
#pragma unroll
        for (int a = 0; a < TI; a++) { u32x4 z = {(unsigned)kt, 1u, 2u, 3u}; asm volatile("" : "+v"(z)); pf[a] = __builtin_bit_cast(bf16x8_t, z); }
#pragma unroll
        for (int b = 0; b < TJ; b++) { u32x4 z = {(unsigned)ks, 5u, 6u, 7u}; asm volatile("" : "+v"(z)); qf[b] = __builtin_bit_cast(bf16x8_t, z); }
      } else {
#pragma unroll
      for (int a = 0; a < TI; a++) {
        const int row = wi0 + a * 32 + frow;
        const int ch = (ks * 2 + fhi) ^ ((row >> 1) & 7);
        u32x4 v = *(const u32x4*)(ps + row * 128 + ch * 16);
        pf[a] = __builtin_bit_cast(bf16x8_t, v);
      }
#pragma unroll
      for (int b = 0; b < TJ; b++) {
        const int row = wj0 + b * 32 + frow;
        const int ch = (ks * 2 + fhi) ^ ((row >> 1) & 7);
        u32x4 v = *(const u32x4*)(qs + row * 128 + ch * 16);
        if (RELU) v = relu16<bf16_t>(v);
        qf[b] = __builtin_bit_cast(bf16x8_t, v);
      }
      }
      if (SCHED == 1 && more) {
#pragma unroll
        for (int i = ks * PPS; i < (ks + 1) * PPS && i < NP; i++) piece((kt + 1) & 1, i);
      }
      if (__builtin_expect(ks < nks, 1)) {
#pragma unroll
        for (int a = 0; a < TI; a++)
#pragma unroll
          for (int b = 0; b < TJ; b++)
            acc[a][b] = __builtin_amdgcn_mfma_f32_32x32x16_bf16(pf[a], qf[b], acc[a][b], 0, 0, 0);
      }
    }
    }
    if (SCHED == 1 && more) advance();
    __syncthreads();
  }

  float al = epi.alpha;
  if (epi.alpha_ptr) al *= *epi.alpha_ptr;
  if (SCHED == 6) {
    float t = 0.f;
#pragma unroll
    for (int ta = 0; ta < TI; ta++)
#pragma unroll
      for (int tb = 0; tb < TJ; tb++) t += acc[ta][tb][0];
    if (t == 1234.5f) *(float*)epi.out = t;
    return;
  }
  sg_conv_epilogue<BI, BJ, NW, TI, TJ>(acc, smem, sbias, epi, i0, j0, wi0, wj0, al);
}

template <int BI, int WJ, int WI, int BJ, int SCHED, bool RELU, bool UP>
static inline int sg_launch_conv_v2r(const ConvV2Params& p, const Epilogue<bf16_t>& e, hipStream_t st) {
  constexpr int BUF = (BJ + BI) * 128;
  static bool attr_done = false;
  if (!attr_done) {
    if (hipFuncSetAttribute((const void*)sg_conv_v2_kernel<BI, WJ, WI, BJ, SCHED, RELU, UP>, hipFuncAttributeMaxDynamicSharedMemorySize, 2 * BUF + BI * 4) != hipSuccess) return -1;
    attr_done = true;
  }
  const int tilesI = (p.I + BI - 1) / BI, tilesJ = (p.J + BJ - 1) / BJ;
  hipLaunchKernelGGL((sg_conv_v2_kernel<BI, WJ, WI, BJ, SCHED, RELU, UP>), dim3(tilesI * tilesJ), dim3(64 * WJ * WI), 2 * BUF + BI * 4, st, p, e, tilesI, tilesJ);
  return 0;
}
template <int BI, int WJ, int WI, int BJ = 256, int SCHED = 0>
static inline int sg_launch_conv_v2(const ConvV2Params& p, const Epilogue<bf16_t>& e, hipStream_t st) {
  const bool up = (p.flags & SG_PIX_UPSAMPLE) != 0;
  if (p.flags & SG_PIX_RELU) return up ? sg_launch_conv_v2r<BI, WJ, WI, BJ, SCHED, true, true>(p, e, st) : sg_launch_conv_v2r<BI, WJ, WI, BJ, SCHED, true, false>(p, e, st);
  return up ? sg_launch_conv_v2r<BI, WJ, WI, BJ, SCHED, false, true>(p, e, st) : sg_launch_conv_v2r<BI, WJ, WI, BJ, SCHED, false, false>(p, e, st);
}
```

### pytorch-studiogan_amd/csrc/conv_v3.hip

```cpp
#include "conv_common.h"
#include "conv_v3.h"
extern template int sg_conv_v3_dispatch<2>(int, int, const ConvV3Params&, const Epilogue<bf16_t>&, hipStream_t);

bool sg_conv_fwd_v3_try(const ConvFwdProblem& pb, hipStream_t st) {
  const sg_conv_fwd_desc* d = pb.d;
  const int I = pb.I, J = pb.J, K = pb.K;
  const char mode = env_mode("SG_CONV_V3");
  if (mode == '0') return false;
  const bool force = mode == 'f';
  if (!is_3x3_s1_p1(d) || (pb.pflags & SG_PIX_TRANSPOSED)) return false;
  if (d->C < 64 || d->C % 32 || d->ldx % 8 || !aligned16(d->x) || !aligned16(d->w)) return false;
  if (!pb.out_is_in_times_up()) return false;
  if (pb.wshift < 0 || pb.hshift < 0 || d->Ws < 4 || d->Hs < 2) return false;
  if (pb.xbytes >= (1ll << 31) || pb.wbytes >= (1ll << 30)) return false;
  if (!epi_bf16_rows_ok(pb.e)) return false;
  int best_tiles = 0;
  int best = cout_tile_search(I, (J + 255) / 256, best_tiles);
  if (I <= 32 && I % 8 == 0 && (J >= 512 * 256 || force)) { best = 32; best_tiles = (J + 511) / 512; }
  if (!best || (best_tiles < 160 && !force && !(K >= 1152 && best_tiles >= 16))) return false;
  const int BJ = (best == 32 || (best == 96 && (J >= 512 * 256 || (force && J % 512 == 0)))) ? 512 : 256;
  if ((pb.quad || pb.up) && (BJ % (2 * d->Wo))) return false;
  if (J % d->Wo) return false;
  ConvV3Params p;
  p.x = (const bf16_t*)d->x; p.w = (const bf16_t*)d->w;
  p.W = d->Ws; p.wlog = ilog2_exact(d->Ws); p.C = d->C; p.ldx = d->ldx;
  p.Ho = d->Ho; p.Wo = d->Wo; p.wshift = pb.wshift; p.hshift = pb.hshift; p.flags = pb.pflags;
  p.I = I; p.J = J; p.K = K; p.nslice = (d->C + 63) / 64;
  p.npix_src = d->N * d->Hs * d->Ws;
  p.npx = (pb.up ? BJ / 4 : BJ) + 2 * d->Ws + 16;
  p.xbytes = (unsigned)pb.xbytes; p.wbytes = (unsigned)pb.wbytes;
  p.zero_off = 0; p.bias_off = 0; p.dump_off = 0;
  const bool par = pb.quad && p.wlog >= 4;
  p.pm4 = par ? 4 : 0;
  p.psh = par ? p.wlog - 2 : 0;
  if (((p.npx >> 3) + 7) / 8 >= 19) return false;
  const int rc = (d->C % 64 == 0) ? sg_conv_v3_dispatch<4>(best, BJ, p, pb.e, st) : sg_conv_v3_dispatch<2>(best, BJ, p, pb.e, st);
  return rc == 0;
}
template int sg_conv_v3_dispatch<4>(int, int, const ConvV3Params&, const Epilogue<bf16_t>&, hipStream_t);
```

### pytorch-studiogan_amd/csrc/conv_v4.hip

```cpp
#include "conv_common.h"
#include "conv_v4.h"

bool sg_conv_fwd_v4_try(const ConvFwdProblem& pb, hipStream_t st) { return sg_conv_fwd_v4_skip_try(pb, nullptr, st, false); }
bool sg_conv_fwd_v4_skip_try(const ConvFwdProblem& pb, const sg_conv_skip_desc* sk, hipStream_t st, bool dry) {
  const sg_conv_fwd_desc* d = pb.d;
  const int I = pb.I, J = pb.J;
  const bool up = pb.up, quad = pb.quad;
  const char mode = env_mode("SG_CONV_V4");
  if (mode == '0') return false;
  const bool all = mode == 'a', force = all || mode == 'f' || sk != nullptr;
  if (!is_3x3_s1_p1(d) || (pb.pflags & SG_PIX_TRANSPOSED)) return false;
  if (d->C < 32 || d->C % 32 || d->ldx % 8 || !aligned16(d->x) || !aligned16(d->w)) return false;
  if (!all && !sk && d->C > 384) return false;
  long long x2bytes = 0, w2bytes = 0;
  if (sk) {
    if (up || !sk->x2 || !sk->w2 || sk->C2 < 32 || sk->C2 % 32 || sk->ldx2 % 8 || !aligned16(sk->x2) || !aligned16(sk->w2)) return false;
    if (sk->bias2 && !d->bias) return false;
    if (sk->x2_up && ((d->Ho & 1) || (d->Wo & 1) || quad)) return false;
    const long long npix2 = (long long)d->N * (sk->x2_up ? (d->Ho / 2) * (d->Wo / 2) : d->Ho * d->Wo);
    x2bytes = bf16_extent(npix2, sk->ldx2, sk->C2); w2bytes = (long long)I * sk->C2 * 2;
    if (x2bytes >= (1ll << 31) || w2bytes >= (1ll << 31)) return false;
  }
  if (!pb.out_is_in_times_up()) return false;
  if (pb.wshift < 0 || pb.hshift < 0 || d->Ws < 4 || d->Hs < 2) return false;
  if (pb.xbytes >= (1ll << 31) || pb.wbytes >= (1ll << 31)) return false;
  if (!epi_bf16_rows_ok(pb.e)) return false;
  const int NB = cout_blocks(I);
  if (!NB) return false;
  const int BJ = 256;
  const int tiles = (I / (32 * NB)) * ((J + BJ - 1) / BJ);
  if (!force && tiles < 768) return false;
  if ((quad || up || (sk && sk->x2_up)) && (BJ % (2 * d->Wo))) return false;
  if (J % d->Wo) return false;
  const int npx = (((up ? BJ / 4 : BJ) + 2 * d->Ws + 16) + 15) & ~15;
  if (sg_conv_v4_lds(NB, npx, nullptr, nullptr, nullptr, sk ? (sk->x2_up ? 3 * 64 * 64 : 2 * 256 * 64) : 0) > 80 * 1024) return false;
  if (dry) return true;
  ConvV4Params p;
  p.x = (const bf16_t*)d->x; p.w = (const bf16_t*)d->w;
  p.W = d->Ws; p.wlog = ilog2_exact(d->Ws); p.C = d->C; p.ldx = d->ldx;
  p.Ho = d->Ho; p.Wo = d->Wo; p.wshift = pb.wshift; p.hshift = pb.hshift; p.flags = pb.pflags;
  p.I = I; p.J = J; p.K = pb.K; p.nslice = d->C / 32;
  p.npix_src = d->N * d->Hs * d->Ws;
  p.npx = npx;
  p.xbytes = (unsigned)pb.xbytes; p.wbytes = (unsigned)pb.wbytes;
  p.wgt_off = p.zero_off = p.bias_off = 0;
  const bool par = quad && p.wlog >= 4;
  p.pm2 = par ? 2 : 0;
  p.psh = par ? p.wlog - 1 : 0;
  p.x2 = nullptr; p.w2 = nullptr; p.bias2 = nullptr; p.C2 = p.ldx2 = p.up2 = p.nslice2 = p.npix2 = 0; p.x2bytes = p.w2bytes = 0;
  p.stats = nullptr;
  if (sk) {
    p.stats = (pb.e.flags & SG_EPI_POOL) ? nullptr : sk->stats;
    p.x2 = (const bf16_t*)sk->x2; p.w2 = (const bf16_t*)sk->w2; p.bias2 = sk->bias2;
    p.C2 = sk->C2; p.ldx2 = sk->ldx2; p.up2 = sk->x2_up ? 1 : 0; p.nslice2 = sk->C2 / 32;
    p.npix2 = d->N * (sk->x2_up ? (d->Ho / 2) * (d->Wo / 2) : d->Ho * d->Wo);
    p.x2bytes = (unsigned)x2bytes; p.w2bytes = (unsigned)w2bytes;
    return (NB == 3 ? sg_launch_conv_v4_skip<3>(p, pb.e, st) : sg_launch_conv_v4_skip<2>(p, pb.e, st)) == 0;
  }
  return (NB == 3 ? sg_launch_conv_v4<3, 2>(p, pb.e, st) : sg_launch_conv_v4<2, 2>(p, pb.e, st)) == 0;
}
```

### pytorch-studiogan_amd/csrc/gemm.hip

```cpp
#include "gemm_core.h"
#include "../../include/sgamd.h"

static inline bool aligned16(const void* p) { return (((uintptr_t)p) & 15) == 0; }

template <typename T, class LP, class LQ, bool TR, int SPLIT>
static void gemm_tiles(const LP& lp, const LQ& lq, const Epilogue<T>& e, int I, int J, int K, int splits, int batch, hipStream_t st) {
  if (I <= 32) sg_launch_gemm<T, LP, LQ, 32, 256, 1, 4, TR, SPLIT>(lp, lq, e, I, J, K, splits, batch, st);
  else if (I % 128 != 0 && (I % 96 == 0 || (I < 128 && I > 64))) sg_launch_gemm<T, LP, LQ, 96, 256, 1, 4, TR, SPLIT>(lp, lq, e, I, J, K, splits, batch, st);
  else sg_launch_gemm<T, LP, LQ, 128, 128, 2, 2, TR, SPLIT>(lp, lq, e, I, J, K, splits, batch, st);
}

template <typename T, class LP, class LQ, bool TR, bool FAST>
static int gemm_launch(const LP& lp, const LQ& lq, const Epilogue<T>& e, const sg_gemm_desc* d, hipStream_t st) {
  const int I = d->I, J = d->J, K = d->K;
  const int splits = d->splits > 1 ? d->splits : 1;
  const int prof = sg_prof_begin(st, 2.0 * (double)I * (double)J * (double)K * (double)d->batch, 2);
  const int mode = (sizeof(T) == 4 && FAST && g_sg_f32_mode == 6) ? 6 : 0;
  if (mode == 6) {
    if constexpr (sizeof(T) == 4 && FAST) { sg_f32_split_count(6); gemm_tiles<T, LP, LQ, TR, 6>(lp, lq, e, I, J, K, splits, d->batch, st); }
  } else {
    gemm_tiles<T, LP, LQ, TR, 0>(lp, lq, e, I, J, K, splits, d->batch, st);
  }
  sg_prof_end(st, prof);
  SG_LAUNCH_CHECK();
  return 0;
}

template <typename T, bool F> static void fill_kc(StridedKC<T, F>& l, const void* p, long long bs, int ld, int rows, int K) {
  l.base = (const T*)p; l.bstride = bs; l.ld = ld; l.rows = rows; l.K = K;
  l.vec_ok = (K % ET<T>::VEC == 0) && (ld % ET<T>::VEC == 0) && (bs % ET<T>::VEC == 0) && aligned16(p);
}
template <typename T, bool F> static void fill_mc(StridedMC<T, F>& l, const void* p, long long bs, int ld, int rows, int K) {
  l.base = (const T*)p; l.bstride = bs; l.ld = ld; l.rows = rows; l.K = K;
  l.vec_ok = (rows % ET<T>::VEC == 0) && (ld % ET<T>::VEC == 0) && (bs % ET<T>::VEC == 0) && aligned16(p);
}

template <typename T, bool TR, bool FAST> static int gemm_forms(const Epilogue<T>& e, const sg_gemm_desc* d, hipStream_t st) {
  typedef StridedKC<T, FAST> KCL;
  typedef StridedMC<T, FAST> MCL;
  if (d->p_form == 0 && d->q_form == 0) {
    KCL lp, lq; fill_kc<T>(lp, d->p, d->p_bstride, d->ldp, d->I, d->K); fill_kc<T>(lq, d->q, d->q_bstride, d->ldq, d->J, d->K);
    return gemm_launch<T, KCL, KCL, TR, FAST>(lp, lq, e, d, st);
  } else if (d->p_form == 0 && d->q_form == 1) {
    KCL lp; MCL lq; fill_kc<T>(lp, d->p, d->p_bstride, d->ldp, d->I, d->K); fill_mc<T>(lq, d->q, d->q_bstride, d->ldq, d->J, d->K);
    return gemm_launch<T, KCL, MCL, TR, FAST>(lp, lq, e, d, st);
  } else if (d->p_form == 1 && d->q_form == 0) {
    MCL lp; KCL lq; fill_mc<T>(lp, d->p, d->p_bstride, d->ldp, d->I, d->K); fill_kc<T>(lq, d->q, d->q_bstride, d->ldq, d->J, d->K);
    return gemm_launch<T, MCL, KCL, TR, FAST>(lp, lq, e, d, st);
  } else {
    MCL lp, lq; fill_mc<T>(lp, d->p, d->p_bstride, d->ldp, d->I, d->K); fill_mc<T>(lq, d->q, d->q_bstride, d->ldq, d->J, d->K);
    return gemm_launch<T, MCL, MCL, TR, FAST>(lp, lq, e, d, st);
  }
}

template <typename T, bool TR> static int gemm_t(const sg_gemm_desc* d, hipStream_t st) {
  Epilogue<T> e;
  e.out = d->out; e.out_bstride = d->out_bstride; e.ldo = d->ldo; e.bias = d->bias;
  e.res = d->res; e.res_bstride = d->res_bstride; e.ldr = d->ldr; e.beta = d->beta;
  e.mask = nullptr; e.mask_bstride = 0; e.ldm = 0; e.split_stride = 0;
  e.alpha = d->alpha; e.alpha_ptr = d->alpha_ptr; e.flags = d->epi_flags; e.I = d->I; e.J = d->J;
  if (d->splits > 1) SG_CHECK(d->epi_flags & SG_EPI_ATOMIC, "sg_gemm: split-K needs the atomic epilogue");
  const int V = ET<T>::VEC;
  auto vec = [&](int form, const void* p, long long bs, int ld, int rows) {
    const bool common = (ld % V == 0) && (bs % V == 0) && aligned16(p);
    return common && (form == 0 ? (d->K % V == 0) : (rows % V == 0));
  };
  if (vec(d->p_form, d->p, d->p_bstride, d->ldp, d->I) && vec(d->q_form, d->q, d->q_bstride, d->ldq, d->J))
    return gemm_forms<T, TR, true>(e, d, st);
  return gemm_forms<T, TR, false>(e, d, st);
}

extern "C" int sg_gemm(const sg_gemm_desc* d, sg_stream_t stream) {
  SG_CHECK(d && d->p && d->q && d->out, "sg_gemm: null pointer");
  SG_CHECK(d->I > 0 && d->J > 0 && d->K > 0 && d->batch > 0, "sg_gemm: bad shape");
  SG_CHECK((d->p_form | d->q_form | 1) == 1, "sg_gemm: operand form must be 0 (KC) or 1 (MC)");
  SG_CHECK(!(d->epi_flags & SG_EPI_POOL), "sg_gemm: pooling epilogue is convolution-only");
  if (d->dtype == SG_DTYPE_F32) return gemm_t<float, true>(d, (hipStream_t)stream);
  if (d->dtype == SG_DTYPE_BF16) {
    if (d->no_tr) return gemm_t<bf16_t, false>(d, (hipStream_t)stream);
    return gemm_t<bf16_t, true>(d, (hipStream_t)stream);
  }
  sg_set_error("sg_gemm: bad dtype");
  return -1;
}
```

### pytorch-studiogan_amd/csrc/gemm_core.h

```cpp
#pragma once
#include "common.h"

#define SG_KC_STRIDE 80

__host__ __device__ constexpr int sg_mc_stride(int B, int es) {
  int s = B * es;
  if (es == 2) {
    while ((s % 128) != 64) s += 16;
    return s;
  }
  return s + 16;
}

template <typename T> __device__ __forceinline__ void set_elem(u32x4& v, int e, T x);
template <> __device__ __forceinline__ void set_elem<float>(u32x4& v, int e, float x) { v[e] = __float_as_uint(x); }
template <> __device__ __forceinline__ void set_elem<bf16_t>(u32x4& v, int e, bf16_t x) {
  v[e >> 1] |= ((uint32_t)x) << (16 * (e & 1));
}

template <typename T, bool FAST = false> struct StridedKC {
  static constexpr bool KC = true;
  static constexpr int VEC = ET<T>::VEC, BK = ET<T>::BK;
  const T* base; long long bstride; int ld; int rows; int K; int vec_ok;
  struct Chunk { const T* p; int k; bool valid; };
  __device__ __forceinline__ void set_batch(int b) { base += (long long)b * bstride; }
  __device__ __forceinline__ void init(Chunk& ch, int row, int k) const {
    ch.valid = row < rows; ch.p = base + (long long)row * ld; ch.k = k;
  }
  __device__ __forceinline__ u32x4 load(const Chunk& ch) const {
    u32x4 v = zero16();
    if (FAST || vec_ok) {
      const bool ok = ch.valid & (ch.k < K);
      const u32x4 t = *(const u32x4*)(ok ? (ch.p + ch.k) : base);
      return ok ? t : v;
    }
    if constexpr (FAST) return v;
    if (!ch.valid || ch.k >= K) return v;
#pragma unroll
    for (int e = 0; e < VEC; e++) if (ch.k + e < K) set_elem<T>(v, e, ch.p[ch.k + e]);
    return v;
  }
  __device__ __forceinline__ void advance(Chunk& ch) const { ch.k += BK; }
};

template <typename T, bool FAST = false> struct StridedMC {
  static constexpr bool KC = false;
  static constexpr int VEC = ET<T>::VEC, BK = ET<T>::BK;
  const T* base; long long bstride; int ld; int rows; int K; int vec_ok;
  struct Chunk { int row; int k; };
  __device__ __forceinline__ void set_batch(int b) { base += (long long)b * bstride; }
  __device__ __forceinline__ void init(Chunk& ch, int row, int k) const { ch.row = row; ch.k = k; }
  __device__ __forceinline__ u32x4 load(const Chunk& ch) const {
    u32x4 v = zero16();
    if (FAST || vec_ok) {
      const bool ok = (ch.k < K) & (ch.row < rows);
      const u32x4 t = *(const u32x4*)(ok ? (base + (long long)ch.k * ld + ch.row) : base);
      return ok ? t : v;
    }
    if constexpr (FAST) return v;
    if (ch.k >= K || ch.row >= rows) return v;
    const T* p = base + (long long)ch.k * ld + ch.row;
#pragma unroll
    for (int e = 0; e < VEC; e++) if (ch.row + e < rows) set_elem<T>(v, e, p[e]);
    return v;
  }
  __device__ __forceinline__ void advance(Chunk& ch) const { ch.k += BK; }
};

#define SG_PIX_RELU 1
#define SG_PIX_UPSAMPLE 2
#define SG_PIX_QUAD 4
#define SG_PIX_TRANSPOSED 8

template <typename T> struct PixGeom {
  const T* x;
  int N, Hs, Ws;
  int Hin, Win;
  int C, ldx;
  int Ho, Wo;
  int R, S, stride, pad_h, pad_w;
  int flags;
  int vec_ok;
  int wshift, hshift;

  __device__ __forceinline__ void pix_decompose(int pix, int& n, int& ho, int& wo) const {
    if (wshift >= 0 && hshift >= 0) {
      wo = pix & (Wo - 1); int t = pix >> wshift; ho = t & (Ho - 1); n = t >> hshift;
    } else {
      wo = pix % Wo; int t = pix / Wo; ho = t % Ho; n = t / Ho;
    }
  }
  __device__ __forceinline__ unsigned tap_off(int n, int ho, int wo, int r, int s, bool& valid) const {
    int h, w;
    bool ok = true;
    if (flags & SG_PIX_TRANSPOSED) {
      int hn = ho + pad_h - r, wn = wo + pad_w - s;
      ok = (hn >= 0) & (wn >= 0);
      if (stride == 2) { ok &= (((hn | wn) & 1) == 0); hn >>= 1; wn >>= 1; }
      else if (stride != 1) { ok &= ((hn % stride) == 0) & ((wn % stride) == 0); hn /= stride; wn /= stride; }
      h = hn; w = wn;
    } else {
      h = ho * stride - pad_h + r; w = wo * stride - pad_w + s;
    }
    ok &= ((unsigned)h < (unsigned)Hin) & ((unsigned)w < (unsigned)Win);
    if (flags & SG_PIX_UPSAMPLE) { h >>= 1; w >>= 1; }
    valid = ok;
    const unsigned off = ((unsigned)(n * Hs + h) * (unsigned)Ws + (unsigned)w) * (unsigned)ldx;
    return ok ? off : 0u;
  }
  __device__ __forceinline__ bool tap(int n, int ho, int wo, int r, int s, const T*& p) const {
    int h, w;
    if (flags & SG_PIX_TRANSPOSED) {
      int hn = ho + pad_h - r, wn = wo + pad_w - s;
      if (hn < 0 || wn < 0) return false;
      if (stride == 2) { if ((hn | wn) & 1) return false; hn >>= 1; wn >>= 1; }
      else if (stride != 1) { if (hn % stride || wn % stride) return false; hn /= stride; wn /= stride; }
      h = hn; w = wn;
    } else {
      h = ho * stride - pad_h + r; w = wo * stride - pad_w + s;
    }
    if (h < 0 || h >= Hin || w < 0 || w >= Win) return false;
    if (flags & SG_PIX_UPSAMPLE) { h >>= 1; w >>= 1; }
    p = x + (unsigned)(((unsigned)(n * Hs + h) * (unsigned)Ws + (unsigned)w) * (unsigned)ldx);
    return true;
  }
};

template <typename T, bool FAST = false> struct ConvPixKC {
  static constexpr bool KC = true;
  static constexpr int VEC = ET<T>::VEC, BK = ET<T>::BK;
  PixGeom<T> g; int rows; int K;
  struct Chunk { int n, ho, wo; int r, s, c; bool valid; };
  __device__ __forceinline__ void set_batch(int) {}
  __device__ __forceinline__ void init(Chunk& ch, int row, int k) const {
    ch.valid = row < rows;
    if (g.flags & SG_PIX_QUAD) {
      int q = row >> 2, dy = (row >> 1) & 1, dx = row & 1;
      int hq, wq;
      int Wq = g.Wo >> 1, Hq = g.Ho >> 1;
      wq = q % Wq; int t = q / Wq; hq = t % Hq; ch.n = t / Hq;
      ch.ho = 2 * hq + dy; ch.wo = 2 * wq + dx;
    } else {
      g.pix_decompose(row, ch.n, ch.ho, ch.wo);
    }
    int rs = k / g.C; ch.c = k - rs * g.C; ch.r = rs / g.S; ch.s = rs - ch.r * g.S;
  }
  __device__ __forceinline__ u32x4 load(const Chunk& ch) const {
    u32x4 v = zero16();
    if (FAST || g.vec_ok) {
      bool ok;
      const unsigned off = g.tap_off(ch.n, ch.ho, ch.wo, ch.r, ch.s, ok);
      ok = ok & ch.valid & (ch.r < g.R);
      const u32x4 t = *(const u32x4*)(g.x + (ok ? off + (unsigned)ch.c : 0u));
      v = ok ? t : v;
    } else if constexpr (!FAST) {
      if (!ch.valid || ch.r >= g.R) return v;
      int r = ch.r, s = ch.s, c = ch.c;
#pragma unroll
      for (int e = 0; e < VEC; e++) {
        if (r < g.R) {
          const T* p;
          if (g.tap(ch.n, ch.ho, ch.wo, r, s, p)) set_elem<T>(v, e, p[c]);
        }
        c++; if (c == g.C) { c = 0; s++; if (s == g.S) { s = 0; r++; } }
      }
    }
    if (g.flags & SG_PIX_RELU) v = relu16<T>(v);
    return v;
  }
  __device__ __forceinline__ void advance(Chunk& ch) const {
    ch.c += BK;
    while (ch.c >= g.C) { ch.c -= g.C; ch.s++; if (ch.s == g.S) { ch.s = 0; ch.r++; } }
  }
};

template <typename T, bool FAST = false> struct ConvPixMC {
  static constexpr bool KC = false;
  static constexpr int VEC = ET<T>::VEC, BK = ET<T>::BK;
  PixGeom<T> g; int rows; int K;
  struct Chunk { int r, s, c; int pix; bool valid; };
  __device__ __forceinline__ void set_batch(int) {}
  __device__ __forceinline__ void init(Chunk& ch, int row, int k) const {
    ch.valid = row < rows;
    int rs = row / g.C; ch.c = row - rs * g.C; ch.r = rs / g.S; ch.s = rs - ch.r * g.S;
    ch.pix = k;
  }
  __device__ __forceinline__ u32x4 load(const Chunk& ch) const {
    u32x4 v = zero16();
    int n, ho, wo;
    if (FAST || g.vec_ok) {
      const bool inb = ch.valid & (ch.pix < K);
      g.pix_decompose(inb ? ch.pix : 0, n, ho, wo);
      bool ok;
      const unsigned off = g.tap_off(n, ho, wo, ch.r, ch.s, ok);
      ok = ok & inb;
      const u32x4 t = *(const u32x4*)(g.x + (ok ? off + (unsigned)ch.c : 0u));
      v = ok ? t : v;
    } else if constexpr (!FAST) {
      if (!ch.valid || ch.pix >= K) return v;
      g.pix_decompose(ch.pix, n, ho, wo);
      int r = ch.r, s = ch.s, c = ch.c;
#pragma unroll
      for (int e = 0; e < VEC; e++) {
        if (r < g.R) {
          const T* p;
          if (g.tap(n, ho, wo, r, s, p)) set_elem<T>(v, e, p[c]);
        }
        c++; if (c == g.C) { c = 0; s++; if (s == g.S) { s = 0; r++; } }
      }
    }
    if (g.flags & SG_PIX_RELU) v = relu16<T>(v);
    return v;
  }
  __device__ __forceinline__ void advance(Chunk& ch) const { ch.pix += BK; }
};

#define SG_EPI_OUT_F32 1
#define SG_EPI_ATOMIC 2
#define SG_EPI_POOL 4
#define SG_EPI_RELU 8
#define SG_EPI_RES_F32 16

template <typename T> struct Epilogue {
  void* out; long long out_bstride; int ldo;
  const float* bias;
  const void* res; long long res_bstride; int ldr; float beta;
  const T* mask; long long mask_bstride; int ldm;
  float alpha; const float* alpha_ptr;
  int flags; int I; int J;
  long long split_stride;

  __device__ __forceinline__ void set_batch(int b) {
    if (flags & (SG_EPI_OUT_F32 | SG_EPI_ATOMIC)) out = (float*)out + (long long)b * out_bstride;
    else out = (T*)out + (long long)b * out_bstride;
    if (res) {
      if (flags & SG_EPI_RES_F32) res = (const float*)res + (long long)b * res_bstride;
      else res = (const T*)res + (long long)b * res_bstride;
    }
    if (mask) mask += (long long)b * mask_bstride;
  }

  __device__ __forceinline__ void store(int j, int i0, float v[4], float a) const {
    if (prep(j, i0, v, a)) write(j, i0, v);
  }
  __device__ __forceinline__ bool prep(int& j, int i0, float v[4], float a) const {
    const int lane = threadIdx.x & 63;
    if (flags & SG_EPI_POOL) {
#pragma unroll
      for (int e = 0; e < 4; e++) v[e] = quad_sum(v[e]);
      if (lane & 3) return false;
      j >>= 2;
    }
    const int Jout = (flags & SG_EPI_POOL) ? (J >> 2) : J;
    if (j >= Jout || i0 >= I) return false;
    const int ne = (I - i0) < 4 ? (I - i0) : 4;
#pragma unroll
    for (int e = 0; e < 4; e++) {
      float x = v[e] * a;
      if (bias && e < ne) x += bias[i0 + e];
      v[e] = x;
    }
    if (mask) {
      const T* m = mask + (long long)j * ldm + i0;
#pragma unroll
      for (int e = 0; e < 4; e++) if (e < ne) { if (!(to_f<T>(m[e]) > 0.f)) v[e] = 0.f; }
    }
    if (res) {
      if (flags & SG_EPI_RES_F32) {
        const float* r = (const float*)res + (long long)j * ldr + i0;
#pragma unroll
        for (int e = 0; e < 4; e++) if (e < ne) v[e] += beta * r[e];
      } else {
        const T* r = (const T*)res + (long long)j * ldr + i0;
#pragma unroll
        for (int e = 0; e < 4; e++) if (e < ne) v[e] += beta * to_f<T>(r[e]);
      }
    }
    if (flags & SG_EPI_RELU) {
#pragma unroll
      for (int e = 0; e < 4; e++) v[e] = fmaxf(v[e], 0.f);
    }
    return true;
  }
  __device__ __forceinline__ void write(int j, int i0, const float v[4]) const {
    const int ne = (I - i0) < 4 ? (I - i0) : 4;
    if (flags & SG_EPI_ATOMIC) {
      float* o = (float*)out + (long long)j * ldo + i0;
#pragma unroll
      for (int e = 0; e < 4; e++) if (e < ne) unsafeAtomicAdd(o + e, v[e]);
    } else if ((flags & SG_EPI_OUT_F32) || sizeof(T) == 4) {
      float* o = (float*)out + (long long)j * ldo + i0;
      if (ne == 4 && ((ldo & 3) == 0) && ((((uintptr_t)out) & 15) == 0)) {
        f32x4 t = {v[0], v[1], v[2], v[3]};
        *(f32x4*)o = t;
      } else {
#pragma unroll
        for (int e = 0; e < 4; e++) if (e < ne) o[e] = v[e];
      }
    } else {
      bf16_t* o = (bf16_t*)out + (long long)j * ldo + i0;
      if (ne == 4 && ((ldo & 3) == 0) && ((((uintptr_t)out) & 7) == 0)) {
        u32x2 t;
        t[0] = (uint32_t)f2bf(v[0]) | ((uint32_t)f2bf(v[1]) << 16);
        t[1] = (uint32_t)f2bf(v[2]) | ((uint32_t)f2bf(v[3]) << 16);
        *(u32x2*)o = t;
      } else {
#pragma unroll
        for (int e = 0; e < 4; e++) if (e < ne) o[e] = f2bf(v[e]);
      }
    }
  }
};

typedef __attribute__((address_space(3))) s16x4 lds_s16x4;

__device__ __forceinline__ bf16x8_t frag_kc_bf16(const char* tile, int row0, int ks) {
  const int l = threadIdx.x & 63;
  const char* p = tile + (row0 + (l & 31)) * SG_KC_STRIDE + (ks * 16 + 8 * (l >> 5)) * 2;
  u32x4 v = *(const u32x4*)p;
  return __builtin_bit_cast(bf16x8_t, v);
}
template <bool TR>
__device__ __forceinline__ bf16x8_t frag_mc_bf16(const char* tile, int pitch, int row0, int ks) {
  const int l = threadIdx.x & 63;
  if (TR) {
    const int g16 = l >> 4, t = l & 15;
    const int r16 = row0 + 16 * (g16 & 1);
    const int k0 = ks * 16 + 8 * (g16 >> 1);
    const char* p = tile + (k0 + (t >> 2)) * pitch + (r16 + 4 * (t & 3)) * 2;
    s16x4 a = __builtin_amdgcn_ds_read_tr16_b64_v4i16((lds_s16x4*)p);
    s16x4 b = __builtin_amdgcn_ds_read_tr16_b64_v4i16((lds_s16x4*)(p + 4 * pitch));
    s16x8 r;
    r[0] = a[0]; r[1] = a[1]; r[2] = a[2]; r[3] = a[3];
    r[4] = b[0]; r[5] = b[1]; r[6] = b[2]; r[7] = b[3];
    return __builtin_bit_cast(bf16x8_t, r);
  } else {
    const int k0 = ks * 16 + 8 * (l >> 5);
    const int row = row0 + (l & 31);
    s16x8 r;
#pragma unroll
    for (int e = 0; e < 8; e++) r[e] = *(const short*)(tile + (k0 + e) * pitch + row * 2);
    return __builtin_bit_cast(bf16x8_t, r);
  }
}
__device__ __forceinline__ float frag_kc_f32(const char* tile, int row0, int kk) {
  const int l = threadIdx.x & 63;
  return *(const float*)(tile + (row0 + (l & 31)) * SG_KC_STRIDE + (kk * 2 + (l >> 5)) * 4);
}
__device__ __forceinline__ float frag_mc_f32(const char* tile, int pitch, int row0, int kk) {
  const int l = threadIdx.x & 63;
  return *(const float*)(tile + (kk * 2 + (l >> 5)) * pitch + (row0 + (l & 31)) * 4);
}

__device__ __forceinline__ void frag_kc_f32_split(const char* tile, int row0, bf16x8_t& hi, bf16x8_t& lo) {
  const int l = threadIdx.x & 63;
  const char* p = tile + (row0 + (l & 31)) * SG_KC_STRIDE + 32 * (l >> 5);
  const f32x4 a = *(const f32x4*)p, b = *(const f32x4*)(p + 16);
  float x[8] = {a[0], a[1], a[2], a[3], b[0], b[1], b[2], b[3]};
  u32x4 h, r;
#pragma unroll
  for (int e = 0; e < 4; e++) {
    const uint32_t hp = pack2bf(x[2 * e], x[2 * e + 1]);
    const float h0 = __uint_as_float(hp << 16), h1 = __uint_as_float(hp & 0xffff0000u);
    h[e] = hp;
    r[e] = pack2bf(x[2 * e] - h0, x[2 * e + 1] - h1);
  }
  hi = __builtin_bit_cast(bf16x8_t, h);
  lo = __builtin_bit_cast(bf16x8_t, r);
}

__device__ __forceinline__ void frag_mc_f32_split(const char* tile, int pitch, int row0, bf16x8_t& hi, bf16x8_t& lo) {
  const int l = threadIdx.x & 63;
  const char* p = tile + (8 * (l >> 5)) * pitch + (row0 + (l & 31)) * 4;
  float x[8];
#pragma unroll
  for (int e = 0; e < 8; e++) x[e] = *(const float*)(p + e * pitch);
  u32x4 h, r;
#pragma unroll
  for (int e = 0; e < 4; e++) {
    const uint32_t hp = pack2bf(x[2 * e], x[2 * e + 1]);
    const float h0 = __uint_as_float(hp << 16), h1 = __uint_as_float(hp & 0xffff0000u);
    h[e] = hp;
    r[e] = pack2bf(x[2 * e] - h0, x[2 * e + 1] - h1);
  }
  hi = __builtin_bit_cast(bf16x8_t, h);
  lo = __builtin_bit_cast(bf16x8_t, r);
}

__device__ __forceinline__ void f32x8_split3(const float (&x)[8], bf16x8_t& hi, bf16x8_t& mid, bf16x8_t& lo) {
  u32x4 h, m, r;
#pragma unroll
  for (int e = 0; e < 4; e++) {
    const uint32_t hp = pack2bf(x[2 * e], x[2 * e + 1]);
    const float r0 = x[2 * e] - __uint_as_float(hp << 16), r1 = x[2 * e + 1] - __uint_as_float(hp & 0xffff0000u);
    const uint32_t mp = pack2bf(r0, r1);
    h[e] = hp;
    m[e] = mp;
    r[e] = pack2bf(r0 - __uint_as_float(mp << 16), r1 - __uint_as_float(mp & 0xffff0000u));
  }
  hi = __builtin_bit_cast(bf16x8_t, h);
  mid = __builtin_bit_cast(bf16x8_t, m);
  lo = __builtin_bit_cast(bf16x8_t, r);
}
__device__ __forceinline__ void frag_kc_f32_split3(const char* tile, int row0, bf16x8_t& hi, bf16x8_t& mid, bf16x8_t& lo) {
  const int l = threadIdx.x & 63;
  const char* p = tile + (row0 + (l & 31)) * SG_KC_STRIDE + 32 * (l >> 5);
  const f32x4 a = *(const f32x4*)p, b = *(const f32x4*)(p + 16);
  const float x[8] = {a[0], a[1], a[2], a[3], b[0], b[1], b[2], b[3]};
  f32x8_split3(x, hi, mid, lo);
}
__device__ __forceinline__ void frag_mc_f32_split3(const char* tile, int pitch, int row0, bf16x8_t& hi, bf16x8_t& mid, bf16x8_t& lo) {
  const int l = threadIdx.x & 63;
  const char* p = tile + (8 * (l >> 5)) * pitch + (row0 + (l & 31)) * 4;
  float x[8];
#pragma unroll
  for (int e = 0; e < 8; e++) x[e] = *(const float*)(p + e * pitch);
  f32x8_split3(x, hi, mid, lo);
}

template <typename T, class LP, class LQ, int BI, int BJ, int WI, int WJ, bool TR, int SPLIT = 0>
__global__ __launch_bounds__(256) void sg_gemm_kernel(LP lp, LQ lq, Epilogue<T> epi, int I, int J, int K,
                                                       int klen, int tilesI, int tilesJ) {
  constexpr int VEC = ET<T>::VEC, BK = ET<T>::BK, ES = sizeof(T);
  constexpr int P_PITCH = LP::KC ? SG_KC_STRIDE : sg_mc_stride(BI, ES);
  constexpr int Q_PITCH = LQ::KC ? SG_KC_STRIDE : sg_mc_stride(BJ, ES);
  constexpr int PB = LP::KC ? BI * SG_KC_STRIDE : BK * P_PITCH;
  constexpr int QB = LQ::KC ? BJ * SG_KC_STRIDE : BK * Q_PITCH;
  constexpr int NP = (BI * 4 + 255) / 256, NQ = (BJ * 4 + 255) / 256;
  constexpr int TI = BI / WI / 32, TJ = BJ / WJ / 32;
  static_assert(WI * WJ == 4, "4 waves");
  static_assert(BI % (WI * 32) == 0 && BJ % (WJ * 32) == 0, "tile/wave mismatch");

  __shared__ __attribute__((aligned(16))) char smem[2 * (PB + QB)];

  const int tid = threadIdx.x, lane = tid & 63, wave = tid >> 6;
  const int nt = tilesI * tilesJ;
  int bid = blockIdx.x;
  {
    const int xcd = bid & 7, q = nt >> 3, r = nt & 7;
    bid = (xcd < r ? xcd * (q + 1) : r * (q + 1) + (xcd - r) * q) + (bid >> 3);
  }
  const int tI = bid % tilesI, tJ = bid / tilesI;
  const int i0 = tI * BI, j0 = tJ * BJ;
  const int k_begin = blockIdx.y * klen;
  const int k_end = (k_begin + klen < K) ? (k_begin + klen) : K;
  if (gridDim.z > 1) { lp.set_batch(blockIdx.z); lq.set_batch(blockIdx.z); epi.set_batch(blockIdx.z); }
  if (epi.split_stride) epi.out = (float*)epi.out + (long long)blockIdx.y * epi.split_stride;

  typename LP::Chunk pc[NP];
  typename LQ::Chunk qc[NQ];
  int p_off[NP], q_off[NQ];
#pragma unroll
  for (int n = 0; n < NP; n++) {
    int c = tid + 256 * n;
    if (c >= BI * 4) c = BI * 4 - 1;
    int row, ko;
    if (LP::KC) { row = c >> 2; ko = (c & 3) * VEC; p_off[n] = row * SG_KC_STRIDE + (c & 3) * 16; }
    else { constexpr int CPR = BI / VEC; row = (c % CPR) * VEC; ko = c / CPR; p_off[n] = ko * P_PITCH + (c % CPR) * 16; }
    lp.init(pc[n], i0 + row, k_begin + ko);
  }
#pragma unroll
  for (int n = 0; n < NQ; n++) {
    int c = tid + 256 * n;
    if (c >= BJ * 4) c = BJ * 4 - 1;
    int row, ko;
    if (LQ::KC) { row = c >> 2; ko = (c & 3) * VEC; q_off[n] = row * SG_KC_STRIDE + (c & 3) * 16; }
    else { constexpr int CPR = BJ / VEC; row = (c % CPR) * VEC; ko = c / CPR; q_off[n] = ko * Q_PITCH + (c % CPR) * 16; }
    lq.init(qc[n], j0 + row, k_begin + ko);
  }

  f32x16 acc[TI][TJ];
#pragma unroll
  for (int a = 0; a < TI; a++)
#pragma unroll
    for (int b = 0; b < TJ; b++)
#pragma unroll
      for (int r = 0; r < 16; r++) acc[a][b][r] = 0.f;

  const int wi = wave % WI, wj = wave / WI;
  const int wi0 = wi * (BI / WI), wj0 = wj * (BJ / WJ);

  u32x4 pr[NP], qr[NQ];
#pragma unroll
  for (int n = 0; n < NP; n++) pr[n] = lp.load(pc[n]);
#pragma unroll
  for (int n = 0; n < NQ; n++) qr[n] = lq.load(qc[n]);
#pragma unroll
  for (int n = 0; n < NP; n++) *(u32x4*)(smem + p_off[n]) = pr[n];
#pragma unroll
  for (int n = 0; n < NQ; n++) *(u32x4*)(smem + PB + q_off[n]) = qr[n];
  __syncthreads();

  const int nk = (k_end - k_begin + BK - 1) / BK;
  for (int it = 0; it < nk; it++) {
    const char* ps = smem + (it & 1) * (PB + QB);
    const char* qs = ps + PB;
    const bool more = (it + 1 < nk);
    if (more) {
#pragma unroll
      for (int n = 0; n < NP; n++) { lp.advance(pc[n]); pr[n] = lp.load(pc[n]); }
#pragma unroll
      for (int n = 0; n < NQ; n++) { lq.advance(qc[n]); qr[n] = lq.load(qc[n]); }
    }
    if constexpr (sizeof(T) == 2) {
#pragma unroll
      for (int ks = 0; ks < 2; ks++) {
        bf16x8_t pf[TI], qf[TJ];
#pragma unroll
        for (int a = 0; a < TI; a++)
          pf[a] = LP::KC ? frag_kc_bf16(ps, wi0 + a * 32, ks) : frag_mc_bf16<TR>(ps, P_PITCH, wi0 + a * 32, ks);
#pragma unroll
        for (int b = 0; b < TJ; b++)
          qf[b] = LQ::KC ? frag_kc_bf16(qs, wj0 + b * 32, ks) : frag_mc_bf16<TR>(qs, Q_PITCH, wj0 + b * 32, ks);
#pragma unroll
        for (int a = 0; a < TI; a++)
#pragma unroll
          for (int b = 0; b < TJ; b++)
            acc[a][b] = __builtin_amdgcn_mfma_f32_32x32x16_bf16(pf[a], qf[b], acc[a][b], 0, 0, 0);
      }
    } else if constexpr (SPLIT == 3) {
      bf16x8_t ph[TI], pl[TI], qh[TJ], ql[TJ];
#pragma unroll
      for (int a = 0; a < TI; a++) {
        if constexpr (LP::KC) frag_kc_f32_split(ps, wi0 + a * 32, ph[a], pl[a]); else frag_mc_f32_split(ps, P_PITCH, wi0 + a * 32, ph[a], pl[a]);
      }
#pragma unroll
      for (int b = 0; b < TJ; b++) {
        if constexpr (LQ::KC) frag_kc_f32_split(qs, wj0 + b * 32, qh[b], ql[b]); else frag_mc_f32_split(qs, Q_PITCH, wj0 + b * 32, qh[b], ql[b]);
      }
#pragma unroll
      for (int a = 0; a < TI; a++)
#pragma unroll
        for (int b = 0; b < TJ; b++) {
          acc[a][b] = __builtin_amdgcn_mfma_f32_32x32x16_bf16(pl[a], qh[b], acc[a][b], 0, 0, 0);
          acc[a][b] = __builtin_amdgcn_mfma_f32_32x32x16_bf16(ph[a], ql[b], acc[a][b], 0, 0, 0);
          acc[a][b] = __builtin_amdgcn_mfma_f32_32x32x16_bf16(ph[a], qh[b], acc[a][b], 0, 0, 0);
        }
    } else if constexpr (SPLIT == 6) {
      bf16x8_t ph[TI], pm[TI], pl[TI], qh[TJ], qm[TJ], ql[TJ];
#pragma unroll
      for (int a = 0; a < TI; a++) {
        if constexpr (LP::KC) frag_kc_f32_split3(ps, wi0 + a * 32, ph[a], pm[a], pl[a]); else frag_mc_f32_split3(ps, P_PITCH, wi0 + a * 32, ph[a], pm[a], pl[a]);
      }
#pragma unroll
      for (int b = 0; b < TJ; b++) {
        if constexpr (LQ::KC) frag_kc_f32_split3(qs, wj0 + b * 32, qh[b], qm[b], ql[b]); else frag_mc_f32_split3(qs, Q_PITCH, wj0 + b * 32, qh[b], qm[b], ql[b]);
      }
#pragma unroll
      for (int a = 0; a < TI; a++)
#pragma unroll
        for (int b = 0; b < TJ; b++) {
          acc[a][b] = __builtin_amdgcn_mfma_f32_32x32x16_bf16(ph[a], ql[b], acc[a][b], 0, 0, 0);
          acc[a][b] = __builtin_amdgcn_mfma_f32_32x32x16_bf16(pl[a], qh[b], acc[a][b], 0, 0, 0);
          acc[a][b] = __builtin_amdgcn_mfma_f32_32x32x16_bf16(pm[a], qm[b], acc[a][b], 0, 0, 0);
          acc[a][b] = __builtin_amdgcn_mfma_f32_32x32x16_bf16(pm[a], qh[b], acc[a][b], 0, 0, 0);
          acc[a][b] = __builtin_amdgcn_mfma_f32_32x32x16_bf16(ph[a], qm[b], acc[a][b], 0, 0, 0);
          acc[a][b] = __builtin_amdgcn_mfma_f32_32x32x16_bf16(ph[a], qh[b], acc[a][b], 0, 0, 0);
        }
    } else {
#pragma unroll
      for (int kk = 0; kk < 8; kk++) {
        float pf[TI], qf[TJ];
#pragma unroll
        for (int a = 0; a < TI; a++)
          pf[a] = LP::KC ? frag_kc_f32(ps, wi0 + a * 32, kk) : frag_mc_f32(ps, P_PITCH, wi0 + a * 32, kk);
#pragma unroll
        for (int b = 0; b < TJ; b++)
          qf[b] = LQ::KC ? frag_kc_f32(qs, wj0 + b * 32, kk) : frag_mc_f32(qs, Q_PITCH, wj0 + b * 32, kk);
#pragma unroll
        for (int a = 0; a < TI; a++)
#pragma unroll
          for (int b = 0; b < TJ; b++)
            acc[a][b] = __builtin_amdgcn_mfma_f32_32x32x2f32(pf[a], qf[b], acc[a][b], 0, 0, 0);
      }
    }
    if (more) {
      char* pd = smem + ((it + 1) & 1) * (PB + QB);
#pragma unroll
      for (int n = 0; n < NP; n++) *(u32x4*)(pd + p_off[n]) = pr[n];
#pragma unroll
      for (int n = 0; n < NQ; n++) *(u32x4*)(pd + PB + q_off[n]) = qr[n];
    }
    __syncthreads();
  }

  float a = epi.alpha;
  if (epi.alpha_ptr) a *= *epi.alpha_ptr;
#pragma unroll
  for (int ta = 0; ta < TI; ta++)
#pragma unroll
    for (int tb = 0; tb < TJ; tb++) {
      const int j = j0 + wj0 + tb * 32 + (lane & 31);
#pragma unroll
      for (int g4 = 0; g4 < 4; g4++) {
        const int ii = i0 + wi0 + ta * 32 + 8 * g4 + 4 * (lane >> 5);
        float v[4] = {acc[ta][tb][4 * g4 + 0], acc[ta][tb][4 * g4 + 1], acc[ta][tb][4 * g4 + 2], acc[ta][tb][4 * g4 + 3]};
        epi.store(j, ii, v, a);
      }
    }
}

struct SgTileCfg { int BI, BJ; };

template <typename T, class LP, class LQ, int BI, int BJ, int WI, int WJ, bool TR = true, int SPLIT = 0>
static inline void sg_launch_gemm(const LP& lp, const LQ& lq, const Epilogue<T>& epi, int I, int J, int K,
                                  int splits, int batch, hipStream_t stream) {
  constexpr int BK = ET<T>::BK;
  const int tilesI = (I + BI - 1) / BI, tilesJ = (J + BJ - 1) / BJ;
  int klen = K;
  if (splits > 1) {
    klen = (K + splits - 1) / splits;
    klen = ((klen + BK - 1) / BK) * BK;
    splits = (K + klen - 1) / klen;
  } else splits = 1;
  dim3 grid(tilesI * tilesJ, splits, batch);
  hipLaunchKernelGGL((sg_gemm_kernel<T, LP, LQ, BI, BJ, WI, WJ, TR, SPLIT>), grid, dim3(256), 0, stream, lp, lq, epi, I, J, K, klen,
                     tilesI, tilesJ);
}
```

### pytorch-studiogan_amd/functional/_base.py

```python
import os

import torch
import torch.distributed as dist

from .. import _lib as L
from .. import comm as _comm
from ..bank import ensure_grad


def _first_order_only(name):
    if torch.is_grad_enabled():
        raise NotImplementedError(name + ": second-order gradients (create_graph=True) are implemented for the discriminator's "
                                         "conv / BN / pooling / self-attention / head path only (gradient penalties, R1)")


def _param_grad_wanted(*params):
    for p in params:
        if p is None or not torch.is_tensor(p) or not p.requires_grad:
            continue
        try:
            if torch._C._will_engine_execute_node(torch.autograd.graph.get_gradient_edge(p).node):
                return True
        except Exception:
            return True
    return False


def _c(t):
    return t if t.is_contiguous() else t.contiguous()


_ZERO_POOL = {}
_ZERO_POOL_BYTES = 8 << 20
_ZERO_POOL_ON = [os.environ.get("SG_ZERO_POOL", "1") != "0"]


def zeros_small(shape, dtype, device):
    if isinstance(shape, int):
        shape = (shape,)
    n = 1
    for d in shape:
        n *= int(d)
    nbytes = n * torch.empty((), dtype=dtype).element_size()
    if not _ZERO_POOL_ON[0] or nbytes == 0 or nbytes > (_ZERO_POOL_BYTES >> 1) or torch.device(device).type != "cuda":
        return torch.zeros(shape, dtype=dtype, device=device)
    key = torch.device(device)
    ent = _ZERO_POOL.get(key)
    step = (nbytes + 255) & ~255
    if ent is None or ent[1] + step > _ZERO_POOL_BYTES:
        ent = _ZERO_POOL[key] = [torch.zeros(_ZERO_POOL_BYTES, dtype=torch.uint8, device=device), 0]
    off = ent[1]
    ent[1] = off + step
    return ent[0][off:off + nbytes].view(dtype).view(shape)


def zeros_like_small(t):
    return zeros_small(tuple(t.shape), t.dtype, t.device)


_SEQ = [0]
_STATS_OFFER = [None]
_BN_FUSED_STATS = [os.environ.get("SG_BN_FUSED_STATS", "1") != "0"]
_CBN_MERGED = [os.environ.get("SG_CBN_MERGED", "1") != "0"]


def _tick():
    _SEQ[0] += 1


def _offer_stats(out, st, rows, C):
    _STATS_OFFER[0] = (_SEQ[0], out.data_ptr(), tuple(out.shape), st, rows, C, out._version)


def _take_stats(x):
    ent, _STATS_OFFER[0] = _STATS_OFFER[0], None
    if ent is None or ent[0] != _SEQ[0] - 1 or ent[1] != x.data_ptr() or ent[2] != tuple(x.shape) or ent[5] != x.shape[3] or ent[6] != x._version:
        return None
    return ent[3], ent[4]


class f32_mode:
    MODES = {"exact": 0, "bf16x3": 3, "bf16x6": 6}

    def __init__(self, mode):
        if mode not in self.MODES:
            raise ValueError(f"f32_mode: {mode!r} (one of {sorted(self.MODES)})")
        self.mode = self.MODES[mode]

    def __enter__(self):
        self.saved = L.lib().sg_get_f32_mode()
        L.call("sg_set_f32_mode", self.mode)
        return self

    def __exit__(self, *exc):
        L.call("sg_set_f32_mode", self.saved)
        return False


def conv2d_raw(x, w_ptr, Cin, Cout, R, S, stride=1, pad_h=0, pad_w=0, pix_flags=0, epi_flags=0, bias=None, res=None, mask=None,
               alpha=1.0, beta=1.0, alpha_ptr=None, out=None, ldx=None, transposed_out_hw=None, out_coff=0, x_coff=0, desc=None):
    N, Hs, Ws = x.shape[0], x.shape[1], x.shape[2]
    ldx = x.shape[3] if ldx is None else ldx
    up = 2 if (pix_flags & L.PIX_UPSAMPLE) else 1
    Hin, Win = Hs * up, Ws * up
    if pix_flags & L.PIX_TRANSPOSED:
        Ho, Wo = transposed_out_hw
    else:
        Ho = (Hin + 2 * pad_h - R) // stride + 1
        Wo = (Win + 2 * pad_w - S) // stride + 1
    pool = bool(epi_flags & L.EPI_POOL)
    Hy, Wy = (Ho // 2, Wo // 2) if pool else (Ho, Wo)
    if out is None:
        odt = torch.float32 if (epi_flags & L.EPI_OUT_F32) else x.dtype
        out = torch.empty((N, Hy, Wy, Cout), dtype=odt, device=x.device)
    d = desc if desc is not None else L.ConvFwdDesc()
    d.dtype = L.dt(x)
    d.N, d.Hs, d.Ws, d.C, d.ldx = N, Hs, Ws, Cin, ldx
    d.Ho, d.Wo, d.Cout = Ho, Wo, Cout
    d.R, d.S, d.stride, d.pad_h, d.pad_w = R, S, stride, pad_h, pad_w
    d.pix_flags, d.epi_flags = pix_flags, epi_flags
    d.alpha, d.beta = alpha, beta
    d.x, d.w = L.ptr(x) + x_coff * x.element_size(), w_ptr
    d.bias = L.ptr(bias)
    d.res = L.ptr(res)
    d.mask = L.ptr(mask)
    d.out = L.ptr(out) + out_coff * out.element_size()
    d.alpha_ptr = L.ptr(alpha_ptr)
    d.ldo = out.shape[-1]
    d.ldr = res.shape[-1] if res is not None else 0
    d.ldm = mask.shape[-1] if mask is not None else 0
    if desc is not None:
        return out
    L.call("sg_conv2d_fwd", d, L.stream())
    return out


def conv2d_skip_raw(x, w_ptr, Cin, Cout, x2, w2_ptr, C2, x2_up=False, pix_flags=0, epi_flags=0, bias=None, bias2=None, alpha=1.0, dry=False, stats=False):
    sk = L.ConvSkipDesc()
    out = conv2d_raw(x, w_ptr, Cin, Cout, 3, 3, 1, 1, 1, pix_flags, epi_flags, bias=bias, alpha=alpha, desc=sk.main)
    sk.x2, sk.w2, sk.bias2 = L.ptr(x2), w2_ptr, L.ptr(bias2)
    sk.C2, sk.ldx2, sk.x2_up = C2, x2.shape[3], 1 if x2_up else 0
    if L.lib().sg_conv2d_fwd_skip_ok(L.C.byref(sk)) != 1:
        return None
    if dry:
        return out
    if stats and not (epi_flags & L.EPI_POOL):
        rows = L.lib().sg_conv2d_fwd_skip_stat_rows(L.C.byref(sk))
        st = torch.empty((rows, Cout, 2), dtype=torch.float32, device=x.device)
        sk.stats = st.data_ptr()
        L.call("sg_conv2d_fwd_skip", sk, L.stream())
        _offer_stats(out, st, rows, Cout)
        return out
    L.call("sg_conv2d_fwd_skip", sk, L.stream())
    return out


def conv2d_wgrad_raw(x, dy, dw_ptr, Cin, Cout, R, S, Ho, Wo, stride=1, pad_h=0, pad_w=0, x_flags=0, g_flags=0, alpha=1.0,
                     alpha_ptr=None, splits=0, no_tr=0, ldg=None, dy_coff=0, dbias=None):
    d = L.ConvWgradDesc()
    d.dtype = L.dt(x)
    d.N = x.shape[0]
    d.xHs, d.xWs, d.C, d.ldx, d.x_flags = x.shape[1], x.shape[2], Cin, x.shape[3], x_flags
    d.gHs, d.gWs, d.Cout, d.ldg, d.g_flags = dy.shape[1], dy.shape[2], Cout, (dy.shape[3] if ldg is None else ldg), g_flags
    d.Ho, d.Wo = Ho, Wo
    d.R, d.S, d.stride, d.pad_h, d.pad_w = R, S, stride, pad_h, pad_w
    d.alpha = alpha
    d.x, d.dy, d.dw = L.ptr(x), L.ptr(dy) + dy_coff * dy.element_size(), dw_ptr
    d.alpha_ptr = L.ptr(alpha_ptr)
    d.splits, d.no_tr = splits, no_tr
    fused = False
    if dbias is not None:
        d.dbias = L.ptr(dbias)
        fused = L.lib().sg_conv2d_wgrad_fuses_bias(L.C.byref(d)) == 1
        if not fused:
            d.dbias = None
    sp, wf = L.C.c_int(0), L.C.c_longlong(0)
    L.call("sg_conv2d_wgrad_plan", d, L.C.byref(sp), L.C.byref(wf))
    work = None
    if wf.value > 0:
        work = torch.empty(wf.value, dtype=torch.float32, device=x.device)
        d.splits, d.work, d.work_floats = sp.value, work.data_ptr(), wf.value
    L.call("sg_conv2d_wgrad", d, L.stream())
    return fused


def quad_pack_raw(src_ptr, dst, mode, M, Cs):
    L.call("sg_quad_pack", L.dt(dst), mode, src_ptr, L.ptr(dst), M, Cs, L.stream())
    return dst


def conv2d_q_raw(x, wq_ptr, form, Cin, Cout, pix_flags=0, epi_flags=0, bias=None, res=None, mask=None, alpha=1.0, beta=1.0, dry=False,
                 x2=None, w2q_ptr=None, bias2=None, stats=False, x2_norelu=False):
    N = x.shape[0]
    if form == L.Q_POOL:
        if x.shape[1] % 2 or x.shape[2] % 2:
            return None
        Hl, Wl = x.shape[1] // 2, x.shape[2] // 2
        oshape = (N, Hl, Wl, Cout)
    else:
        Hl, Wl = x.shape[1], x.shape[2]
        oshape = (N, 2 * Hl, 2 * Wl, Cout)
    if x.dtype != torch.bfloat16:
        return None
    d = L.ConvQDesc()
    d.dtype, d.form = L.dt(x), form
    d.N, d.Hl, d.Wl, d.C, d.ldx, d.Cout = N, Hl, Wl, Cin, x.shape[3], Cout
    d.pix_flags, d.epi_flags, d.alpha, d.beta = pix_flags, epi_flags, alpha, beta
    out = torch.empty(oshape, dtype=x.dtype, device=x.device)
    d.x, d.wq, d.bias, d.res, d.mask, d.out = L.ptr(x), wq_ptr, L.ptr(bias), L.ptr(res), L.ptr(mask), L.ptr(out)
    d.ldo = Cout
    d.ldr = res.shape[-1] if res is not None else 0
    d.ldm = mask.shape[-1] if mask is not None else 0
    if x2 is not None:
        d.x2, d.w2q, d.bias2, d.C2, d.ldx2 = L.ptr(x2), w2q_ptr, L.ptr(bias2), x2.shape[3], x2.shape[3]
        d.x2_norelu = 1 if x2_norelu else 0
    if L.lib().sg_conv2d_q_ok(L.C.byref(d)) != 1:
        return None
    if not dry:
        st = None
        if stats:
            rows = L.lib().sg_conv2d_q_stat_rows(L.C.byref(d))
            st = torch.empty((rows, Cout, 2), dtype=torch.float32, device=x.device)
            d.stats = st.data_ptr()
        L.call("sg_conv2d_q", d, L.stream())
        if st is not None:
            _offer_stats(out, st, rows, Cout)
    return out


def conv2d_q_wgrad_raw(x, dy, dw_ptr, form, Cin, Cout, x_flags=0, alpha=1.0, dbias=None, splits=0):
    if x.dtype != torch.bfloat16:
        return False
    d = L.ConvQWgradDesc()
    d.dtype, d.form = L.dt(x), form
    lo = dy if form == L.Q_POOL else x
    d.N, d.Hl, d.Wl = lo.shape[0], lo.shape[1], lo.shape[2]
    d.C, d.ldx, d.x_flags, d.Cout, d.ldg = Cin, x.shape[3], x_flags, Cout, dy.shape[3]
    d.alpha = alpha
    d.x, d.dy, d.dw, d.dbias = L.ptr(x), L.ptr(dy), dw_ptr, L.ptr(dbias)
    d.splits = splits
    sp, wf = L.C.c_int(0), L.C.c_longlong(0)
    L.call("sg_conv2d_q_wgrad_plan", d, L.C.byref(sp), L.C.byref(wf))
    if sp.value == 0:
        return False
    work = torch.empty(wf.value, dtype=torch.float32, device=x.device)
    d.work, d.work_floats, d.splits = work.data_ptr(), wf.value, sp.value
    L.call("sg_conv2d_q_wgrad", d, L.stream())
    return True


def gemm_raw(dtype, p, p_form, ldp, q, q_form, ldq, out, ldo, I, J, K, batch=1, p_bs=0, q_bs=0, out_bs=0, bias=None, res=None,
             res_bs=0, ldr=0, beta=1.0, alpha=1.0, alpha_ptr=None, epi_flags=0, splits=1, no_tr=0):
    d = L.GemmDesc()
    d.dtype, d.p_form, d.q_form = dtype, p_form, q_form
    d.I, d.J, d.K, d.batch = I, J, K, batch
    d.p = p if isinstance(p, int) else L.ptr(p)
    d.q = q if isinstance(q, int) else L.ptr(q)
    d.out = out if isinstance(out, int) else L.ptr(out)
    d.p_bstride, d.ldp, d.q_bstride, d.ldq, d.out_bstride, d.ldo = p_bs, ldp, q_bs, ldq, out_bs, ldo
    d.bias = bias if (bias is None or isinstance(bias, int)) else L.ptr(bias)
    d.res = res if (res is None or isinstance(res, int)) else L.ptr(res)
    d.res_bstride, d.ldr, d.beta = res_bs, ldr, beta
    d.alpha = alpha
    d.alpha_ptr = L.ptr(alpha_ptr)
    d.epi_flags, d.splits, d.no_tr = epi_flags, splits, no_tr
    L.call("sg_gemm", d, L.stream())


_DGRAD_SPLITK = [os.environ.get("SG_DGRAD_SPLITK", "1") != "0"]


def gemm_dgrad_rows(w_ptr, dy, dx, B, K, O):
    S = 1
    tiles = ((K + 127) // 128) * ((B + 127) // 128)
    if _DGRAD_SPLITK[0] and tiles < 64:
        while S < 32 and tiles * S < 256 and O % (2 * S) == 0 and O // (2 * S) >= 96:
            S *= 2
    if S == 1:
        gemm_raw(L.F32, w_ptr, 1, K, dy, 0, dy.shape[1] if torch.is_tensor(dy) else O, dx, K, K, B, O)
        return dx
    ldq = dy.shape[1]
    ws = torch.empty((S, B, K), dtype=torch.float32, device=dx.device)
    gemm_raw(L.F32, w_ptr, 1, K, dy, 0, ldq, ws, K, K, B, O // S, batch=S, p_bs=(O // S) * K, q_bs=O // S, out_bs=B * K)
    torch.sum(ws, dim=0, out=dx)
    return dx


__all__ = ['L', 'zeros_small', 'zeros_like_small', '_BN_FUSED_STATS', '_CBN_MERGED', '_DGRAD_SPLITK', '_SEQ', '_STATS_OFFER', '_c', '_comm', '_first_order_only', '_offer_stats', '_param_grad_wanted', '_take_stats', '_tick', 'conv2d_q_raw', 'conv2d_q_wgrad_raw', 'conv2d_raw', 'conv2d_skip_raw', 'conv2d_wgrad_raw', 'dist', 'ensure_grad', 'f32_mode', 'gemm_dgrad_rows', 'gemm_raw', 'os', 'quad_pack_raw', 'torch']
```

### pytorch-studiogan_amd/functional/conv.py

```python
import ctypes

from ._base import *

class ConvCfg:
    __slots__ = ("R", "S", "stride", "pad_h", "pad_w", "in_relu", "in_upsample", "out_pool", "stats")

    def __init__(self, R, S, stride=1, pad_h=0, pad_w=0, in_relu=False, in_upsample=False, out_pool=False, stats=False):
        self.R, self.S, self.stride, self.pad_h, self.pad_w = R, S, stride, pad_h, pad_w
        self.in_relu, self.in_upsample, self.out_pool = in_relu, in_upsample, out_pool
        self.stats = stats

    def out_hw(self, Hs, Ws):
        up = 2 if self.in_upsample else 1
        return (Hs * up + 2 * self.pad_h - self.R) // self.stride + 1, (Ws * up + 2 * self.pad_w - self.S) // self.stride + 1

    def pix_flags(self):
        return (L.PIX_RELU if self.in_relu else 0) | (L.PIX_UPSAMPLE if self.in_upsample else 0)

    def epi_flags(self):
        return L.EPI_POOL if self.out_pool else 0

    @property
    def scale(self):
        return 0.25 if self.out_pool else 1.0


class GradLink:
    __slots__ = ("dx", "chain", "pending")

    def __init__(self, chain=False):
        self.dx = None
        self.chain = chain
        self.pending = 0

    def take(self):
        t, self.dx = self.dx, None
        return t


_GRAD_LINK = [os.environ.get("SG_GRAD_LINK", "1") != "0"]


_QUAD = [os.environ.get("SG_QUAD", "1") != "0"]


def _quad_form(rt, cfg, x):
    if not _QUAD[0] or x.dtype != torch.bfloat16 or cfg.R != 3 or cfg.S != 3 or cfg.stride != 1 or cfg.pad_h != 1 or cfg.pad_w != 1:
        return None
    if cfg.out_pool == cfg.in_upsample or rt.trans or rt.RS != 9:
        return None
    if rt.cin_pad % 32 or (rt.rows_pad % 64 and rt.rows_pad % 96):
        return None
    return L.Q_POOL if cfg.out_pool else L.Q_UP


def _conv_fwd(x, rt, slot, cfg, bias, res=None, stats=False):
    bank = rt.bank()
    Cin = x.shape[3]
    form = _quad_form(rt, cfg, x)
    if form is not None:
        y = conv2d_q_raw(x, bank.w_quad(slot, rt, form), form, Cin, rt.rows_pad, L.PIX_RELU if cfg.in_relu else 0, 0, bias=bias, res=res,
                         stats=stats and _BN_FUSED_STATS[0] and rt.rows_pad == rt.rows)
        if y is not None:
            return y
    return conv2d_raw(x, bank.w_fwd(slot, rt), Cin, rt.rows_pad, cfg.R, cfg.S, cfg.stride, cfg.pad_h, cfg.pad_w, cfg.pix_flags(), cfg.epi_flags(),
                      bias=bias, res=res, alpha=cfg.scale)


def _conv_wgrad(x, dy, rt, slot, cfg, dbias=None):
    bank = rt.bank()
    N, Hs, Ws, Cin = x.shape
    form = _quad_form(rt, cfg, x)
    if form is not None and conv2d_q_wgrad_raw(x, dy, bank.dwt(slot, rt), form, Cin, rt.rows_pad, L.PIX_RELU if cfg.in_relu else 0, dbias=dbias):
        return dbias is not None
    Ho, Wo = cfg.out_hw(Hs, Ws)
    return conv2d_wgrad_raw(x, dy, bank.dwt(slot, rt), Cin, rt.rows_pad, cfg.R, cfg.S, Ho, Wo, cfg.stride, cfg.pad_h, cfg.pad_w, cfg.pix_flags(),
                            L.PIX_UPSAMPLE if cfg.out_pool else 0, alpha=cfg.scale, dbias=dbias)


def _conv_dgrad(dy, x, rt, slot, cfg, res=None):
    bank = rt.bank()
    N, Hs, Ws, Cin = x.shape
    form = _quad_form(rt, cfg, x)
    if form is not None and dy.shape[3] == rt.rows_pad:
        dx = conv2d_q_raw(dy, bank.w_quad(slot, rt, 2 + form), 1 - form, rt.rows_pad, Cin, 0, 0, mask=x if cfg.in_relu else None, res=res)
        if dx is not None:
            return dx
    up = 2 if cfg.in_upsample else 1
    Hin, Win = Hs * up, Ws * up
    pool = cfg.out_pool
    if cfg.stride != 1:
        assert not (pool or cfg.in_upsample), "upsample / pooling fusion is stride-1 only"
        return conv2d_raw(dy, bank.w_dgrad(slot, rt), rt.rows_pad, Cin, cfg.R, cfg.S, cfg.stride, cfg.pad_h, cfg.pad_w, L.PIX_TRANSPOSED, 0,
                          mask=x if cfg.in_relu else None, res=res, transposed_out_hw=(Hin, Win), ldx=dy.shape[3])
    pf = L.PIX_UPSAMPLE if pool else 0
    ef = L.EPI_POOL if cfg.in_upsample else 0
    return conv2d_raw(dy, bank.w_dgrad(slot, rt), rt.rows_pad, Cin, cfg.R, cfg.S, 1, cfg.R - 1 - cfg.pad_h, cfg.S - 1 - cfg.pad_w, pf, ef,
                      mask=x if cfg.in_relu else None, res=res, alpha=cfg.scale, ldx=dy.shape[3])


class ConvDgradFn(torch.autograd.Function):

    @staticmethod
    def forward(ctx, dy, x, weight, rt, slot, cfg):
        dy = _c(dy)
        ctx.save_for_backward(dy, x)
        ctx.rt, ctx.slot, ctx.cfg = rt, slot, cfg
        return _conv_dgrad(dy, x, rt, slot, cfg)

    @staticmethod
    def backward(ctx, ddx):
        dy, x = ctx.saved_tensors
        rt, slot, cfg = ctx.rt, ctx.slot, ctx.cfg
        bank = rt.bank()
        t = _c(ddx)
        if cfg.in_relu:
            m = torch.empty_like(t)
            L.call("sg_relu_mask", L.dt(t), L.ptr(t), L.ptr(x), L.ptr(m), t.numel(), L.stream())
            t = m
        N, Hs, Ws, Cin = x.shape
        Ho, Wo = cfg.out_hw(Hs, Ws)
        g_dy = None
        if ctx.needs_input_grad[0]:
            g_dy = conv2d_raw(t, bank.w_fwd(slot, rt), Cin, rt.rows_pad, cfg.R, cfg.S, cfg.stride, cfg.pad_h, cfg.pad_w,
                              L.PIX_UPSAMPLE if cfg.in_upsample else 0, cfg.epi_flags(), alpha=cfg.scale)
        if ctx.needs_input_grad[2]:
            conv2d_wgrad_raw(t, dy, bank.dwt(slot, rt), Cin, rt.rows_pad, cfg.R, cfg.S, Ho, Wo, cfg.stride, cfg.pad_h, cfg.pad_w,
                             L.PIX_UPSAMPLE if cfg.in_upsample else 0, L.PIX_UPSAMPLE if cfg.out_pool else 0, alpha=cfg.scale)
        return g_dy, None, None, None, None, None


class ConvFn(torch.autograd.Function):

    @staticmethod
    def forward(ctx, x, weight, bias, res, rt, slot, cfg, link=None):
        bank = rt.bank()
        x = _c(x)
        N, Hs, Ws, Cin = x.shape
        assert Cin == rt.cin_pad, f"conv input channels {Cin} != {rt.cin_pad}"
        ctx.link = link
        if link is not None and link.chain:
            link.pending += 1
        if res is not None:
            res = _c(res)
        bias_k = bias
        if bias is not None and rt.rows_pad != rt.rows:
            bias_k = zeros_small(rt.rows_pad, torch.float32, x.device)
            bias_k[:rt.rows].copy_(bias.detach())
        _tick()
        y = _conv_fwd(x, rt, slot, cfg, bias_k, res, stats=cfg.stats)
        ctx.save_for_backward(x)
        ctx.rt, ctx.slot, ctx.cfg = rt, slot, cfg
        ctx.bias = bias
        ctx.weight = weight
        ctx.has_res = res is not None
        return y

    @staticmethod
    def backward(ctx, dy):
        (x,) = ctx.saved_tensors
        rt, slot, cfg = ctx.rt, ctx.slot, ctx.cfg
        bank = rt.bank()
        if torch.is_grad_enabled():
            if _param_grad_wanted(ctx.weight, ctx.bias):
                raise NotImplementedError("create_graph=True is supported for input gradients only (WGAN-GP path)")
            dx = ConvDgradFn.apply(dy, x, ctx.weight, rt, slot, cfg) if ctx.needs_input_grad[0] else None
            return dx, None, None, (dy if ctx.has_res else None), None, None, None, None
        dy = _c(dy)
        dx = None
        skip_dx = ctx.link.take() if ctx.link is not None else None
        if ctx.needs_input_grad[0]:
            dx = _conv_dgrad(dy, x, rt, slot, cfg, res=skip_dx)
        elif skip_dx is not None:
            raise RuntimeError("GradLink: a skip gradient was handed over but this convolution's input needs no gradient")
        if ctx.link is not None and ctx.link.chain:
            ctx.link.pending -= 1
            if ctx.link.pending > 0 and dx is not None:
                ctx.link.dx, dx = dx, None
        want_db = ctx.bias is not None and ctx.needs_input_grad[2]
        db_done = False
        if ctx.needs_input_grad[1]:
            g = ensure_grad(ctx.bias) if (want_db and rt.rows_pad == rt.rows) else None
            db_done = _conv_wgrad(x, dy, rt, slot, cfg, dbias=g)
        if want_db and not db_done:
            g = ensure_grad(ctx.bias)
            rows = dy.shape[0] * dy.shape[1] * dy.shape[2]
            L.call("sg_colsum", L.dt(dy), L.ptr(dy), dy.shape[3], None, 0, rows, rt.rows, L.ptr(g), 1.0, L.stream())
        dres = dy if ctx.has_res else None
        return dx, None, None, dres, None, None, None, None


class ConvSkipFn(torch.autograd.Function):

    @staticmethod
    def forward(ctx, h, x, w2, b2, w0, b0, rt2, rt0, slot, cfg2, cfg0, link=None):
        bank = rt2.bank()
        ctx.link = link
        h, x = _c(h), _c(x)
        _tick()
        assert cfg2.R == 3 and cfg0.R == 1 and cfg2.out_pool == cfg0.out_pool and not cfg2.in_upsample and (cfg0.in_relu == cfg2.in_relu or not cfg0.in_relu)
        pf, ef, al = cfg2.pix_flags(), cfg2.epi_flags(), cfg2.scale
        same_relu = cfg0.in_relu == cfg2.in_relu
        y = None
        plain = rt2.rows_pad == rt2.rows and rt0.rows_pad == rt0.rows and b2 is not None and b0 is not None
        if plain and same_relu and h.dtype == torch.bfloat16 and _SKIP_FUSION[0] and (h.shape[1] >= 16 or _SKIP_FUSION[0] == "all") and _quad_form(rt2, cfg2, h) is None:
            y = conv2d_skip_raw(h, bank.w_fwd(slot, rt2), h.shape[3], rt2.rows, x, bank.w_fwd(slot, rt0), x.shape[3], cfg0.in_upsample, pf, ef,
                                bias=b2, bias2=b0, alpha=al, stats=cfg2.stats and _BN_FUSED_STATS[0])
        if y is None and plain and _quad_form(rt2, cfg2, h) == L.Q_POOL and _SKIP_FUSION[0] and (rt0.cin_pad % 32 == 0 or rt0.cin_pad == 8) and not cfg0.in_upsample:
            y = conv2d_q_raw(h, bank.w_quad(slot, rt2, L.Q_POOL), L.Q_POOL, h.shape[3], rt2.rows, pf, 0, bias=b2,
                             x2=x, w2q_ptr=bank.w_quad(slot, rt0, 5 if rt0.cin_pad == 8 else 4), bias2=b0, x2_norelu=not same_relu)
        if y is None:
            hh = _conv_fwd(h, rt2, slot, cfg2, b2)
            y = conv2d_raw(x, bank.w_fwd(slot, rt0), x.shape[3], rt0.rows_pad, 1, 1, 1, 0, 0, cfg0.pix_flags(), ef, bias=b0, res=hh, alpha=al)
        ctx.save_for_backward(h, x)
        ctx.rt2, ctx.rt0, ctx.slot, ctx.cfg2, ctx.cfg0 = rt2, rt0, slot, cfg2, cfg0
        ctx.w2, ctx.b2, ctx.w0, ctx.b0 = w2, b2, w0, b0
        return y

    @staticmethod
    def backward(ctx, dy):
        h, x = ctx.saved_tensors
        rt2, rt0, slot, cfg2, cfg0 = ctx.rt2, ctx.rt0, ctx.slot, ctx.cfg2, ctx.cfg0
        if torch.is_grad_enabled():
            if _param_grad_wanted(ctx.w2, ctx.b2, ctx.w0, ctx.b0):
                raise NotImplementedError("create_graph=True is supported for input gradients only (WGAN-GP path)")
            dh = ConvDgradFn.apply(dy, h, ctx.w2, rt2, slot, cfg2) if ctx.needs_input_grad[0] else None
            dx = ConvDgradFn.apply(dy, x, ctx.w0, rt0, slot, cfg0) if ctx.needs_input_grad[1] else None
            return (dh, dx) + (None,) * 10
        dy = _c(dy)
        bank = rt2.bank()
        outs = []
        want2 = ctx.b2 is not None and ctx.needs_input_grad[3]
        want0 = ctx.b0 is not None and ctx.needs_input_grad[5]
        shared_db = None
        if want2 and want0 and ctx.needs_input_grad[2] and ctx.needs_input_grad[4] and rt2.rows_pad == rt2.rows and rt0.rows == rt2.rows:
            shared_db = zeros_small(rt2.rows, torch.float32, dy.device)
        for inp, rt, cfg, w_i, b_i, wp, bp in ((h, rt2, cfg2, 2, 3, ctx.w2, ctx.b2), (x, rt0, cfg0, 4, 5, ctx.w0, ctx.b0)):
            k = 0 if inp is h else 1
            outs.append(_conv_dgrad(dy, inp, rt, slot, cfg) if ctx.needs_input_grad[k] else None)
            want_db = bp is not None and ctx.needs_input_grad[b_i]
            db_done = False
            if ctx.needs_input_grad[w_i]:
                g = ensure_grad(bp) if (want_db and rt.rows_pad == rt.rows) else None
                if k == 0 and shared_db is not None:
                    g = shared_db
                elif k == 1 and shared_db is not None:
                    g = None
                db_done = _conv_wgrad(inp, dy, rt, slot, cfg, dbias=g)
                if k == 0 and shared_db is not None:
                    if db_done:
                        for bq in (ctx.b2, ctx.b0):
                            L.call("sg_axpby", L.F32, L.ptr(shared_db), L.ptr(ensure_grad(bq)), rt2.rows, 1.0, 1.0, L.stream())
                        continue
                    shared_db = None
                elif k == 1 and shared_db is not None:
                    continue
            if want_db and not db_done:
                g = ensure_grad(bp)
                L.call("sg_colsum", L.dt(dy), L.ptr(dy), dy.shape[3], None, 0, dy.shape[0] * dy.shape[1] * dy.shape[2], rt.rows, L.ptr(g), 1.0, L.stream())
        if ctx.link is not None and outs[1] is not None and _GRAD_LINK[0]:
            ctx.link.dx = outs[1]
            outs[1] = None
        return (outs[0], outs[1]) + (None,) * 10


_SKIP_FUSION = [{"0": False, "all": "all"}.get(os.environ.get("SG_SKIP_FUSION", "1"), True)]


class SliceUpFn(torch.autograd.Function):

    @staticmethod
    def forward(ctx, x, C, up, link=None):
        x = _c(x)
        N, Hs, Ws, ld = x.shape
        ctx.dims = (N, Hs, Ws, ld, C, up)
        ctx.link = link
        if C == ld and up == 1:
            return x.view_as(x)
        y = torch.empty((N, Hs * up, Ws * up, C), dtype=x.dtype, device=x.device)
        L.call("sg_slice_up_fwd", L.dt(x), L.ptr(x), L.ptr(y), N, Hs, Ws, ld, C, up, L.stream())
        return y

    @staticmethod
    def backward(ctx, dy):
        _first_order_only("SliceUpFn")
        N, Hs, Ws, ld, C, up = ctx.dims
        dy = _c(dy)
        if C == ld and up == 1:
            dx = dy
        else:
            dx = torch.empty((N, Hs, Ws, ld), dtype=dy.dtype, device=dy.device)
            L.call("sg_slice_up_bwd", L.dt(dy), L.ptr(dy), L.ptr(dx), N, Hs, Ws, ld, C, up, L.stream())
        if ctx.link is not None and _GRAD_LINK[0]:
            ctx.link.dx, dx = dx, None
        return dx, None, None, None


class CatConvFn(torch.autograd.Function):

    @staticmethod
    def forward(ctx, x, weight, bias, rt, slot):
        bank = rt.bank()
        x = _c(x)
        N, H, W, Cin = x.shape
        Cc = rt.rows
        out = torch.empty((N, H, W, Cin + Cc), dtype=x.dtype, device=x.device)
        L.call("sg_copy_channels", L.dt(x), L.ptr(x), Cin, L.ptr(out), Cin + Cc, N * H * W, Cin, L.stream())
        conv2d_raw(x, bank.w_fwd(slot, rt), Cin, Cc, 1, 1, bias=bias, out=out, out_coff=Cin)
        ctx.save_for_backward(x)
        ctx.rt, ctx.slot, ctx.bias = rt, slot, bias
        ctx.weight = weight
        return out

    @staticmethod
    def backward(ctx, dy):
        (x,) = ctx.saved_tensors
        rt, slot = ctx.rt, ctx.slot
        if torch.is_grad_enabled():
            if _param_grad_wanted(ctx.weight, ctx.bias):
                raise NotImplementedError("create_graph=True is supported for input gradients only (WGAN-GP / R1 path)")
            return (CatConvDgradFn.apply(dy, ctx.weight, rt, slot, x.shape[3]) if ctx.needs_input_grad[0] else None), None, None, None, None
        bank = rt.bank()
        dy = _c(dy)
        N, H, W, Cin = x.shape
        Cc = rt.rows
        ld = Cin + Cc
        dx = None
        if ctx.needs_input_grad[0]:
            dx = conv2d_raw(dy, bank.w_dgrad(slot, rt), Cc, Cin, 1, 1, res=dy, ldx=ld, x_coff=Cin)
        if ctx.needs_input_grad[1]:
            conv2d_wgrad_raw(x, dy, bank.dwt(slot, rt), Cin, Cc, 1, 1, H, W, ldg=ld, dy_coff=Cin)
        if ctx.bias is not None and ctx.needs_input_grad[2]:
            g = ensure_grad(ctx.bias)
            L.call("sg_colsum", L.dt(dy), L.ptr(dy) + Cin * dy.element_size(), ld, None, 0, N * H * W, Cc, L.ptr(g), 1.0, L.stream())
        return dx, None, None, None, None


class CatConvDgradFn(torch.autograd.Function):

    @staticmethod
    def forward(ctx, dy, weight, rt, slot, Cin):
        dy = _c(dy)
        ctx.save_for_backward(dy)
        ctx.rt, ctx.slot, ctx.Cin = rt, slot, Cin
        Cc = rt.rows
        return conv2d_raw(dy, rt.bank().w_dgrad(slot, rt), Cc, Cin, 1, 1, res=dy, ldx=Cin + Cc, x_coff=Cin)

    @staticmethod
    def backward(ctx, ddx):
        (dy,) = ctx.saved_tensors
        rt, slot, Cin = ctx.rt, ctx.slot, ctx.Cin
        bank = rt.bank()
        t = _c(ddx)
        N, H, W, _ = t.shape
        Cc = rt.rows
        g_dy = None
        if ctx.needs_input_grad[0]:
            g_dy = torch.empty((N, H, W, Cin + Cc), dtype=t.dtype, device=t.device)
            L.call("sg_copy_channels", L.dt(t), L.ptr(t), Cin, L.ptr(g_dy), Cin + Cc, N * H * W, Cin, L.stream())
            conv2d_raw(t, bank.w_fwd(slot, rt), Cin, Cc, 1, 1, out=g_dy, out_coff=Cin)
        if ctx.needs_input_grad[1]:
            conv2d_wgrad_raw(t, dy, bank.dwt(slot, rt), Cin, Cc, 1, 1, H, W, ldg=Cin + Cc, dy_coff=Cin)
        return g_dy, None, None, None, None


class ConvTransposeFn(torch.autograd.Function):

    @staticmethod
    def forward(ctx, x, weight, bias, rt, slot, cfg):
        bank = rt.bank()
        x = _c(x)
        N, H, W, Cin = x.shape
        assert Cin == rt.Cin
        Ho = (H - 1) * cfg.stride - 2 * cfg.pad_h + cfg.R
        Wo = (W - 1) * cfg.stride - 2 * cfg.pad_w + cfg.S
        y = conv2d_raw(x, bank.w_fwd(slot, rt), Cin, rt.rows, cfg.R, cfg.S, cfg.stride, cfg.pad_h, cfg.pad_w, L.PIX_TRANSPOSED, 0, bias=bias,
                       transposed_out_hw=(Ho, Wo))
        ctx.save_for_backward(x)
        ctx.rt, ctx.slot, ctx.cfg, ctx.bias = rt, slot, cfg, bias
        return y

    @staticmethod
    def backward(ctx, dy):
        _first_order_only("ConvTransposeFn")
        (x,) = ctx.saved_tensors
        rt, slot, cfg = ctx.rt, ctx.slot, ctx.cfg
        bank = rt.bank()
        dy = _c(dy)
        N, H, W, Cin = x.shape
        dx = None
        if ctx.needs_input_grad[0]:
            dx = conv2d_raw(dy, bank.w_dgrad(slot, rt), rt.rows, Cin, cfg.R, cfg.S, cfg.stride, cfg.pad_h, cfg.pad_w)
        if ctx.needs_input_grad[1]:
            conv2d_wgrad_raw(dy, x, bank.dwt(slot, rt), rt.rows, Cin, cfg.R, cfg.S, H, W, cfg.stride, cfg.pad_h, cfg.pad_w)
        if ctx.bias is not None and ctx.needs_input_grad[2]:
            g = ensure_grad(ctx.bias)
            L.call("sg_colsum", L.dt(dy), L.ptr(dy), dy.shape[3], None, 0, dy.shape[0] * dy.shape[1] * dy.shape[2], rt.rows, L.ptr(g), 1.0, L.stream())
        return dx, None, None, None, None, None


class LinearFn(torch.autograd.Function):

    @staticmethod
    def forward(ctx, x, weight, bias, rt, slot, const_bias):
        bank = rt.bank()
        x = _c(x.float())
        B, K = x.shape
        assert K == rt.cols
        y = torch.empty((B, rt.rows), dtype=torch.float32, device=x.device)
        b = bias if bias is not None else const_bias
        gemm_raw(L.F32, bank.w_f32(slot, rt), 0, K, x, 0, K, y, rt.rows, rt.rows, B, K, bias=b)
        ctx.save_for_backward(x)
        ctx.rt, ctx.slot, ctx.bias = rt, slot, bias
        ctx.weight = weight
        return y

    @staticmethod
    def backward(ctx, dy):
        (x,) = ctx.saved_tensors
        rt, slot = ctx.rt, ctx.slot
        if torch.is_grad_enabled():
            if _param_grad_wanted(ctx.weight, ctx.bias):
                raise NotImplementedError("create_graph=True is supported for input gradients only (gradient penalties, latent optimisation)")
            return (LinearDgradFn.apply(dy, ctx.weight, rt, slot) if ctx.needs_input_grad[0] else None), None, None, None, None, None
        bank = rt.bank()
        dy = _c(dy.float())
        B, K = x.shape
        O = rt.rows
        dx = None
        if ctx.needs_input_grad[0]:
            dx = torch.empty((B, K), dtype=torch.float32, device=x.device)
            gemm_dgrad_rows(bank.w_f32(slot, rt), dy, dx, B, K, O)
        if ctx.needs_input_grad[1]:
            dw = bank.dwt(slot, rt)
            gemm_raw(L.F32, x, 1, K, dy, 1, O, dw, K, K, O, B, res=dw, ldr=K)
        if ctx.bias is not None and ctx.needs_input_grad[2]:
            g = ensure_grad(ctx.bias)
            L.call("sg_colsum", L.F32, L.ptr(dy), O, None, 0, B, O, L.ptr(g), 1.0, L.stream())
        return dx, None, None, None, None, None


class LinearDgradFn(torch.autograd.Function):

    @staticmethod
    def forward(ctx, dy, weight, rt, slot):
        dy = _c(dy.float())
        B, O = dy.shape
        assert O == rt.rows
        ctx.save_for_backward(dy)
        ctx.rt, ctx.slot = rt, slot
        dx = torch.empty((B, rt.cols), dtype=torch.float32, device=dy.device)
        gemm_dgrad_rows(rt.bank().w_f32(slot, rt), dy, dx, B, rt.cols, O)
        return dx

    @staticmethod
    def backward(ctx, ddx):
        (dy,) = ctx.saved_tensors
        rt, slot = ctx.rt, ctx.slot
        bank = rt.bank()
        t = _c(ddx.float())
        B, K = t.shape
        O = rt.rows
        g_dy = None
        if ctx.needs_input_grad[0]:
            g_dy = torch.empty((B, O), dtype=torch.float32, device=t.device)
            gemm_raw(L.F32, bank.w_f32(slot, rt), 0, K, t, 0, K, g_dy, O, O, B, K)
        if ctx.needs_input_grad[1]:
            dw = bank.dwt(slot, rt)
            gemm_raw(L.F32, t, 1, K, dy, 1, O, dw, K, K, O, B, res=dw, ldr=K)
        return g_dy, None, None, None


class CbnAffineFn(torch.autograd.Function):

    @staticmethod
    def forward(ctx, y, wg, wb, rt_g, rt_b, slot, const2):
        bank = rt_g.bank()
        y = _c(y.float())
        B, K = y.shape
        C = rt_g.rows
        assert K == rt_g.cols == rt_b.cols and rt_b.rows == C
        out = torch.empty((B, 2 * C), dtype=torch.float32, device=y.device)
        pg, pb = bank.w_f32(slot, rt_g), bank.w_f32(slot, rt_b)
        ctx.adjacent = pb == pg + 4 * C * K
        if ctx.adjacent:
            gemm_raw(L.F32, pg, 0, K, y, 0, K, out, 2 * C, 2 * C, B, K, bias=const2)
        else:
            gemm_raw(L.F32, pg, 0, K, y, 0, K, out, 2 * C, C, B, K, bias=const2)
            gemm_raw(L.F32, pb, 0, K, y, 0, K, out.data_ptr() + 4 * C, 2 * C, C, B, K)
        ctx.save_for_backward(y)
        ctx.rt_g, ctx.rt_b, ctx.slot = rt_g, rt_b, slot
        return out

    @staticmethod
    def backward(ctx, dgb):
        _first_order_only("CbnAffineFn")
        (y,) = ctx.saved_tensors
        dy = _cbn_affine_backward(y, dgb, ctx.rt_g, ctx.rt_b, ctx.slot, ctx.adjacent, ctx.needs_input_grad[0], ctx.needs_input_grad[1], ctx.needs_input_grad[2])
        return dy, None, None, None, None, None, None


def _cbn_affine_backward(y, dgb, rt_g, rt_b, slot, fwd_adjacent, need_y, need_g, need_b):
    bank = rt_g.bank()
    dgb = _c(dgb.float())
    B, K = y.shape
    C = rt_g.rows
    pg, pb = bank.w_f32(slot, rt_g), bank.w_f32(slot, rt_b)
    dg = bank.dwt(slot, rt_g) if need_g else None
    db = bank.dwt(slot, rt_b) if need_b else None
    both = dg is not None and db is not None
    adjacent = fwd_adjacent and (not both or db == dg + 4 * C * K)
    dy = None
    if need_y:
        dy = torch.empty((B, K), dtype=torch.float32, device=y.device)
        if adjacent:
            gemm_dgrad_rows(pg, dgb, dy, B, K, 2 * C)
        else:
            gemm_raw(L.F32, pg, 1, K, dgb, 0, 2 * C, dy, K, K, B, C)
            gemm_raw(L.F32, pb, 1, K, dgb.data_ptr() + 4 * C, 0, 2 * C, dy, K, K, B, C, res=dy, ldr=K)
    if both and adjacent:
        gemm_raw(L.F32, y, 1, K, dgb, 1, 2 * C, dg, K, K, 2 * C, B)
    else:
        if dg is not None:
            gemm_raw(L.F32, y, 1, K, dgb, 1, 2 * C, dg, K, K, C, B)
        if db is not None:
            gemm_raw(L.F32, y, 1, K, dgb.data_ptr() + 4 * C, 1, 2 * C, db, K, K, C, B)
    return dy


class CbnAffineGroupFn(torch.autograd.Function):

    @staticmethod
    def forward(ctx, slot, metas, yidx, *tensors):
        G = len(tensors) - 2 * len(metas)
        ys = [_c(t.float()) for t in tensors[:G]]
        B, K = ys[0].shape
        bank = metas[0][0].bank()
        dev = ys[0].device
        n = len(metas)
        total = sum(2 * m[0].rows for m in metas)
        out_all = torch.empty(B * total, dtype=torch.float32, device=dev)
        arr = (L.LinearItem * (2 * n))()
        outs, adj, off, k = [], [], 0, 0
        for i, (rt_g, rt_b, const2) in enumerate(metas):
            C = rt_g.rows
            y = ys[yidx[i]]
            assert y.shape == (B, K) and rt_g.cols == K and rt_b.cols == K and rt_b.rows == C
            pg, pb = bank.w_f32(slot, rt_g), bank.w_f32(slot, rt_b)
            a = pb == pg + 4 * C * K
            adj.append(a)
            base = out_all.data_ptr() + 4 * off
            parts = [(pg, 2 * C, const2.data_ptr(), base)] if a else [(pg, C, const2.data_ptr(), base), (pb, C, const2.data_ptr() + 4 * C, base + 4 * C)]
            for (w, rows, bias, o) in parts:
                it = arr[k]
                it.w, it.y, it.bias, it.out, it.rows, it.K, it.ldy, it.ldo = w, y.data_ptr(), bias, o, rows, K, K, 2 * C
                k += 1
            outs.append(out_all[off:off + B * 2 * C].view(B, 2 * C))
            off += B * 2 * C
        raw = bytes(bytearray(arr)[:k * ctypes.sizeof(L.LinearItem)])
        cache = bank.__dict__.setdefault("_linear_group_tabs", {})
        tab = cache.get(raw)
        if tab is None:
            if len(cache) >= 64:
                cache.clear()
            tab = cache[raw] = L.upload_bytes(raw, dev)
        L.call("sg_linear_group", tab.data_ptr(), arr, k, B, L.stream())
        ctx.save_for_backward(*ys)
        ctx.metas, ctx.yidx, ctx.slot, ctx.adj, ctx.G = metas, yidx, slot, adj, G
        ctx._keep = out_all
        return tuple(outs)

    @staticmethod
    def backward(ctx, *dgbs):
        _first_order_only("CbnAffineGroupFn")
        ys = ctx.saved_tensors
        G, n = ctx.G, len(ctx.metas)
        dys = [None] * G
        for i, ((rt_g, rt_b, _), dgb) in enumerate(zip(ctx.metas, dgbs)):
            if dgb is None:
                continue
            g = ctx.yidx[i]
            dy = _cbn_affine_backward(ys[g], dgb, rt_g, rt_b, ctx.slot, ctx.adj[i], ctx.needs_input_grad[3 + g],
                                      ctx.needs_input_grad[3 + G + 2 * i], ctx.needs_input_grad[3 + G + 2 * i + 1])
            if dy is not None:
                dys[g] = dy if dys[g] is None else dys[g].add_(dy)
        return (None, None, None) + tuple(dys) + (None,) * (2 * n)


def cbn_prefetch(slot, pairs):
    slot.cbn_rows = {}
    if not (_CBN_GROUP[0] and _CBN_MERGED[0]):
        return
    ok = [(m, y) for (m, y) in pairs if m.gain.bias is None and m.bias.bias is None and m.gain.__dict__.get("_sg_rt") is not None]
    if len(ok) < 2:
        return
    if ok[0][0].gain._sg_rt.bank().exchange is not None:
        return
    ys, yidx = [], []
    for _, y in ok:
        for j, t in enumerate(ys):
            if t is y:
                yidx.append(j)
                break
        else:
            yidx.append(len(ys))
            ys.append(y)
    if any(t.shape != ys[0].shape for t in ys):
        return
    metas = [(m.gain._sg_rt, m.bias._sg_rt, m._ones2) for m, _ in ok]
    ws = []
    for m, _ in ok:
        ws += [m.gain.master_weight, m.bias.master_weight]
    outs = CbnAffineGroupFn.apply(slot, metas, yidx, *ys, *ws)
    for (m, _), o in zip(ok, outs):
        slot.cbn_rows[id(m)] = o


_CBN_GROUP = [os.environ.get("SG_CBN_GROUP", "1") != "0"]


class EmbeddingFn(torch.autograd.Function):

    @staticmethod
    def forward(ctx, weight, idx):
        idx = _c(idx.long())
        B = idx.numel()
        num, dim = weight.shape
        out = torch.empty((B, dim), dtype=torch.float32, device=weight.device)
        L.call("sg_embedding_fwd", L.ptr(weight), L.ptr(idx), L.ptr(out), B, dim, num, L.stream())
        ctx.save_for_backward(idx)
        ctx.weight = weight
        return out

    @staticmethod
    def backward(ctx, dout):
        _first_order_only("EmbeddingFn")
        (idx,) = ctx.saved_tensors
        w = ctx.weight
        if ctx.needs_input_grad[0]:
            g = ensure_grad(w)
            dout = _c(dout.float())
            L.call("sg_embedding_bwd", L.ptr(dout), L.ptr(idx), L.ptr(g), idx.numel(), w.shape[1], w.shape[0], L.stream())
        return None, None


class SNEmbeddingFn(torch.autograd.Function):

    @staticmethod
    def forward(ctx, weight, idx, rt, slot):
        bank = rt.bank()
        idx = _c(idx.long())
        B = idx.numel()
        out = torch.empty((B, rt.cols), dtype=torch.float32, device=weight.device)
        L.call("sg_embedding_fwd", bank.w_f32(slot, rt), L.ptr(idx), L.ptr(out), B, rt.cols, rt.rows, L.stream())
        ctx.save_for_backward(idx)
        ctx.rt, ctx.slot = rt, slot
        return out

    @staticmethod
    def backward(ctx, dout):
        _first_order_only("SNEmbeddingFn")
        (idx,) = ctx.saved_tensors
        rt, slot = ctx.rt, ctx.slot
        if ctx.needs_input_grad[0]:
            dout = _c(dout.float())
            L.call("sg_embedding_bwd", L.ptr(dout), L.ptr(idx), rt.bank().dwt(slot, rt), idx.numel(), rt.cols, rt.rows, L.stream())
        return None, None, None, None


__all__ = ['CatConvDgradFn', 'CatConvFn', 'CbnAffineFn', 'CbnAffineGroupFn', 'cbn_prefetch', '_CBN_GROUP', 'ConvCfg', 'ConvDgradFn', 'ConvFn', 'ConvSkipFn', 'ConvTransposeFn', 'EmbeddingFn', 'GradLink', 'LinearDgradFn', 'LinearFn', 'SNEmbeddingFn', 'SliceUpFn', '_GRAD_LINK', '_QUAD', '_SKIP_FUSION', '_conv_dgrad', '_conv_fwd', '_conv_wgrad', '_quad_form']
```

Baseline: 2058.

## Compute skip-path dgrad at half resolution and upsample inside the residual epilogue

The discriminator skip-branch 1x1 conv dgrad with a pooled output is now computed at the coarse (pre-upsample) resolution. The result is handed over through GradLink as a half-resolution tensor, which the main conv's dgrad epilogue reads with a nearest-upsample row mapping and an optional residual-before-mask ordering. This removes the full-resolution 1x1 dgrad and the materialised upsampled residual, cutting both FLOPs and memory traffic. Paths that cannot take the half-resolution residual fall back to an explicit upsample plus ReLU mask, which adds extra launches on those paths.

Result: no change. 2068 (median of 6 runs) (+0.5%).

```diff
diff --git a/include/sgamd.h b/include/sgamd.h
--- a/include/sgamd.h
+++ b/include/sgamd.h
@@ -20,6 +20,8 @@
 #define SG_EPI_POOL 4
 #define SG_EPI_RELU 8
 #define SG_EPI_RES_F32 16
+#define SG_EPI_RES_HALF 32
+#define SG_EPI_RES_PREMASK 64
 
 const char* sg_last_error(void);
 int sg_version(void);
@@ -38,6 +40,7 @@
   int ldo, ldr, ldm;
 } sg_conv_fwd_desc;
 int sg_conv2d_fwd(const sg_conv_fwd_desc* d, sg_stream_t stream);
+int sg_conv2d_fwd_res_half_ok(const sg_conv_fwd_desc* d);
 int sg_set_f32_mode(int mode);
 int sg_get_f32_mode(void);
 long long sg_f32_split_launches(int mode);
diff --git a/pytorch-studiogan_amd/_lib.py b/pytorch-studiogan_amd/_lib.py
--- a/pytorch-studiogan_amd/_lib.py
+++ b/pytorch-studiogan_amd/_lib.py
@@ -14,7 +14,7 @@
 F32, BF16, F64 = 0, 1, 2
 PIX_RELU, PIX_UPSAMPLE, PIX_QUAD, PIX_TRANSPOSED = 1, 2, 4, 8
 Q_POOL, Q_UP = 0, 1
-EPI_OUT_F32, EPI_ATOMIC, EPI_POOL, EPI_RELU, EPI_RES_F32 = 1, 2, 4, 8, 16
+EPI_OUT_F32, EPI_ATOMIC, EPI_POOL, EPI_RELU, EPI_RES_F32, EPI_RES_HALF, EPI_RES_PREMASK = 1, 2, 4, 8, 16, 32, 64
 
 _vp, _i, _f, _ll = C.c_void_p, C.c_int, C.c_float, C.c_longlong
 
@@ -101,6 +101,7 @@
     "sg_prof_enable": [_i],
     "sg_prof_collect": [C.POINTER(C.c_double), _i],
     "sg_conv2d_fwd": [C.POINTER(ConvFwdDesc), _vp],
+    "sg_conv2d_fwd_res_half_ok": [C.POINTER(ConvFwdDesc)],
     "sg_conv2d_fwd_skip": [C.POINTER(ConvSkipDesc), _vp],
     "sg_conv2d_fwd_skip_ok": [C.POINTER(ConvSkipDesc)],
     "sg_conv_rs_launches": [],
diff --git a/pytorch-studiogan_amd/csrc/conv.hip b/pytorch-studiogan_amd/csrc/conv.hip
--- a/pytorch-studiogan_amd/csrc/conv.hip
+++ b/pytorch-studiogan_amd/csrc/conv.hip
@@ -50,7 +50,7 @@
   if (d->C % 8 || d->ldx % 8 || d->R * d->S > 25 || J < 256) return false;
   if (pb.xbytes >= (1ll << 31) || pb.wbytes >= (1ll << 30)) return false;
   if (!aligned16(d->x) || !aligned16(d->w)) return false;
-  if (!epi_bf16_rows_ok(pb.e)) return false;
+  if (!epi_bf16_rows_ok(pb.e, true)) return false;
   const int tj = (J + 255) / 256;
   int best_tiles = 0;
   int best = cout_tile_search(I, tj, best_tiles);
@@ -85,6 +85,15 @@
   return rc == 0;
 }
 
+static const char* res_half_refusal(const sg_conv_fwd_desc* d) {
+  if (d->dtype != SG_DTYPE_BF16) return "sg_conv2d_fwd: SG_EPI_RES_HALF is bf16-only";
+  if (!d->res) return "sg_conv2d_fwd: SG_EPI_RES_HALF without a residual";
+  if (d->epi_flags & (SG_EPI_RES_F32 | SG_EPI_POOL)) return "sg_conv2d_fwd: SG_EPI_RES_HALF does not combine with SG_EPI_RES_F32 / SG_EPI_POOL";
+  if ((d->Ho & 1) || (d->Wo & 1)) return "sg_conv2d_fwd: SG_EPI_RES_HALF needs even Ho, Wo";
+  return nullptr;
+}
+extern "C" int sg_conv2d_fwd_res_half_ok(const sg_conv_fwd_desc* d) { return d && d->Ho > 0 && d->Wo > 0 && !res_half_refusal(d) ? 1 : 0; }
+
 template <typename T> static int conv_fwd_t(const sg_conv_fwd_desc* d, hipStream_t st) {
   const int K = d->R * d->S * d->C;
   const int I = d->Cout;
@@ -99,6 +108,8 @@
   } else {
     pflags &= ~SG_PIX_QUAD;
   }
+  if (d->epi_flags & SG_EPI_RES_HALF) { const char* why = res_half_refusal(d); SG_CHECK(!why, why); }
+  if (d->epi_flags & SG_EPI_RES_PREMASK) SG_CHECK(d->mask && d->res && !(d->epi_flags & SG_EPI_POOL), "sg_conv2d_fwd: SG_EPI_RES_PREMASK needs a mask and a residual, without SG_EPI_POOL");
   const bool w_vec = (K % ET<T>::VEC == 0) && aligned16(d->w);
   const bool x_vec = (d->C % ET<T>::VEC == 0) && (d->ldx % ET<T>::VEC == 0) && aligned16(d->x);
   const Epilogue<T> e = make_epilogue<T>(d, I, J);
@@ -120,7 +131,8 @@
   }
   {
     const double es = sizeof(T), jout = (d->epi_flags & SG_EPI_POOL) ? (double)J / 4.0 : (double)J;
-    const double b = es * ((double)d->N * d->Hs * d->Ws * d->C + (double)I * K + jout * I * (1.0 + (d->mask ? 1.0 : 0.0) + (d->res ? 1.0 : 0.0)));
+    const double res = !d->res ? 0.0 : (d->epi_flags & SG_EPI_RES_HALF) ? 0.25 : 1.0;
+    const double b = es * ((double)d->N * d->Hs * d->Ws * d->C + (double)I * K + jout * I * (1.0 + (d->mask ? 1.0 : 0.0) + res));
     sg_prof_tag(prof, eng, b);
   }
   sg_prof_end(st, prof);
@@ -131,6 +143,7 @@
 static int conv_fwd_skip(const sg_conv_skip_desc* sk, hipStream_t st, bool dry) {
   const sg_conv_fwd_desc* d = &sk->main;
   if (d->dtype != SG_DTYPE_BF16 || d->R != 3 || d->S != 3 || d->stride != 1 || (d->pix_flags & (SG_PIX_UPSAMPLE | SG_PIX_TRANSPOSED))) return 0;
+  if (d->epi_flags & (SG_EPI_RES_HALF | SG_EPI_RES_PREMASK)) return 0;
   const int K = 9 * d->C, I = d->Cout;
   const long long Jll = (long long)d->N * d->Ho * d->Wo;
   if (Jll >= (1ll << 31) || (long long)d->N * d->Hs * d->Ws * d->ldx >= (1ll << 31)) return 0;
diff --git a/pytorch-studiogan_amd/csrc/conv_common.h b/pytorch-studiogan_amd/csrc/conv_common.h
--- a/pytorch-studiogan_amd/csrc/conv_common.h
+++ b/pytorch-studiogan_amd/csrc/conv_common.h
@@ -1,5 +1,6 @@
 #pragma once
 #include <stdlib.h>
+#include <type_traits>
 #include "gemm_core.h"
 #include "../../include/sgamd.h"
 
@@ -49,10 +50,13 @@
   e.res = d->res; e.res_bstride = 0; e.ldr = d->ldr; e.beta = d->beta;
   e.mask = (const T*)d->mask; e.mask_bstride = 0; e.ldm = d->ldm; e.split_stride = 0;
   e.alpha = d->alpha; e.alpha_ptr = d->alpha_ptr; e.flags = d->epi_flags; e.I = I; e.J = J;
+  if constexpr (std::is_same_v<D, sg_conv_fwd_desc>) { e.rWo = d->Wo; e.rwshift = ilog2_exact(d->Wo); }
   return e;
 }
-static inline bool epi_bf16_rows_ok(const Epilogue<bf16_t>& e) {
+static inline bool epi_bf16_rows_ok(const Epilogue<bf16_t>& e, bool res_ext_ok = false) {
   if ((e.flags & (SG_EPI_ATOMIC | SG_EPI_OUT_F32)) || (e.ldo & 7) || !aligned16(e.out)) return false;
+  if ((e.flags & (SG_EPI_RES_HALF | SG_EPI_RES_PREMASK)) && (!res_ext_ok || !e.res || (e.flags & SG_EPI_POOL))) return false;
+  if ((e.flags & SG_EPI_RES_HALF) && e.rwshift < 1) return false;
   if (e.mask && ((e.ldm & 7) || !aligned16(e.mask))) return false;
   if (e.res && ((e.flags & SG_EPI_RES_F32) || (e.ldr & 7) || !aligned16(e.res))) return false;
   return true;
diff --git a/pytorch-studiogan_amd/csrc/conv_v2.h b/pytorch-studiogan_amd/csrc/conv_v2.h
--- a/pytorch-studiogan_amd/csrc/conv_v2.h
+++ b/pytorch-studiogan_amd/csrc/conv_v2.h
@@ -35,13 +35,15 @@
   constexpr int CPR = BI / 8;
   const bool pre_mask = epi.mask != nullptr, pre_res = epi.res != nullptr;
   const bool pre_both = pre_mask && pre_res;
+  const bool res_half = !VMAP && (epi.flags & SG_EPI_RES_HALF) != 0;
+  const bool res_first = pre_both && (epi.flags & SG_EPI_RES_PREMASK) != 0;
   const int ncr = ((epi.I - i0 < BI ? epi.I - i0 : BI) + 7) >> 3;
-  auto stage_tile = [&](const bf16_t* src, int ld) {
+  auto stage_tile = [&](const bf16_t* src, int ld, bool half = false) {
     for (int idx = tid; idx < rows_out * CPR; idx += 64 * NW) {
       const int r = idx / CPR, c = idx - r * CPR;
       const int jg = jbase + r;
       u32x4 t = {0u, 0u, 0u, 0u};
-      if (jg < Jout && c < ncr) t = *(const u32x4*)(src + grow(jg) * ld + i0 + c * 8);
+      if (jg < Jout && c < ncr) t = *(const u32x4*)(src + (half ? epi.res_half_row(jg) : grow(jg)) * ld + i0 + c * 8);
       *(u32x4*)(smem + r * CP + c * 16) = t;
     }
   };
@@ -70,10 +72,10 @@
         }
     }
     __syncthreads();
-    stage_tile((const bf16_t*)epi.res, epi.ldr);
+    stage_tile((const bf16_t*)epi.res, epi.ldr, res_half);
     __syncthreads();
   } else if (pre_mask || pre_res) {
-    stage_tile(pre_mask ? epi.mask : (const bf16_t*)epi.res, pre_mask ? epi.ldm : epi.ldr);
+    stage_tile(pre_mask ? epi.mask : (const bf16_t*)epi.res, pre_mask ? epi.ldm : epi.ldr, pre_res && res_half);
     __syncthreads();
   }
   const bool relu_out = (epi.flags & SG_EPI_RELU) != 0;
@@ -102,6 +104,11 @@
 #pragma unroll
             for (int e = 0; e < 4; e++) v[e] += b[e];
           }
+          if (res_first) {
+            const u32x2 r = *(const u32x2*)loc;
+#pragma unroll
+            for (int e = 0; e < 4; e++) { const bf16_t h = (bf16_t)((r[e >> 1] >> (16 * (e & 1))) & 0xffffu); v[e] += epi.beta * bf2f(h); }
+          }
           if (pre_both) {
             const uint32_t bits = mbits[ta * TJ + tb] >> (4 * g4);
 #pragma unroll
@@ -111,7 +118,7 @@
 #pragma unroll
             for (int e = 0; e < 4; e++) { const bf16_t h = (bf16_t)((m[e >> 1] >> (16 * (e & 1))) & 0xffffu); if (!(bf2f(h) > 0.f)) v[e] = 0.f; }
           }
-          if (pre_res) {
+          if (pre_res && !res_first) {
             const u32x2 r = *(const u32x2*)loc;
 #pragma unroll
             for (int e = 0; e < 4; e++) { const bf16_t h = (bf16_t)((r[e >> 1] >> (16 * (e & 1))) & 0xffffu); v[e] += epi.beta * bf2f(h); }
diff --git a/pytorch-studiogan_amd/csrc/conv_v3.hip b/pytorch-studiogan_amd/csrc/conv_v3.hip
--- a/pytorch-studiogan_amd/csrc/conv_v3.hip
+++ b/pytorch-studiogan_amd/csrc/conv_v3.hip
@@ -13,7 +13,7 @@
   if (!pb.out_is_in_times_up()) return false;
   if (pb.wshift < 0 || pb.hshift < 0 || d->Ws < 4 || d->Hs < 2) return false;
   if (pb.xbytes >= (1ll << 31) || pb.wbytes >= (1ll << 30)) return false;
-  if (!epi_bf16_rows_ok(pb.e)) return false;
+  if (!epi_bf16_rows_ok(pb.e, true)) return false;
   int best_tiles = 0;
   int best = cout_tile_search(I, (J + 255) / 256, best_tiles);
   if (I <= 32 && I % 8 == 0 && (J >= 512 * 256 || force)) { best = 32; best_tiles = (J + 511) / 512; }
diff --git a/pytorch-studiogan_amd/csrc/conv_v4.hip b/pytorch-studiogan_amd/csrc/conv_v4.hip
--- a/pytorch-studiogan_amd/csrc/conv_v4.hip
+++ b/pytorch-studiogan_amd/csrc/conv_v4.hip
@@ -24,7 +24,7 @@
   if (!pb.out_is_in_times_up()) return false;
   if (pb.wshift < 0 || pb.hshift < 0 || d->Ws < 4 || d->Hs < 2) return false;
   if (pb.xbytes >= (1ll << 31) || pb.wbytes >= (1ll << 31)) return false;
-  if (!epi_bf16_rows_ok(pb.e)) return false;
+  if (!epi_bf16_rows_ok(pb.e, true)) return false;
   const int NB = cout_blocks(I);
   if (!NB) return false;
   const int BJ = 256;
diff --git a/pytorch-studiogan_amd/csrc/gemm.hip b/pytorch-studiogan_amd/csrc/gemm.hip
--- a/pytorch-studiogan_amd/csrc/gemm.hip
+++ b/pytorch-studiogan_amd/csrc/gemm.hip
@@ -74,7 +74,7 @@
   SG_CHECK(d && d->p && d->q && d->out, "sg_gemm: null pointer");
   SG_CHECK(d->I > 0 && d->J > 0 && d->K > 0 && d->batch > 0, "sg_gemm: bad shape");
   SG_CHECK((d->p_form | d->q_form | 1) == 1, "sg_gemm: operand form must be 0 (KC) or 1 (MC)");
-  SG_CHECK(!(d->epi_flags & SG_EPI_POOL), "sg_gemm: pooling epilogue is convolution-only");
+  SG_CHECK(!(d->epi_flags & (SG_EPI_POOL | SG_EPI_RES_HALF | SG_EPI_RES_PREMASK)), "sg_gemm: pooling epilogue / half-resolution or pre-mask residual are convolution-only");
   if (d->dtype == SG_DTYPE_F32) return gemm_t<float, true>(d, (hipStream_t)stream);
   if (d->dtype == SG_DTYPE_BF16) {
     if (d->no_tr) return gemm_t<bf16_t, false>(d, (hipStream_t)stream);
diff --git a/pytorch-studiogan_amd/csrc/gemm_core.h b/pytorch-studiogan_amd/csrc/gemm_core.h
--- a/pytorch-studiogan_amd/csrc/gemm_core.h
+++ b/pytorch-studiogan_amd/csrc/gemm_core.h
@@ -220,6 +220,8 @@
 #define SG_EPI_POOL 4
 #define SG_EPI_RELU 8
 #define SG_EPI_RES_F32 16
+#define SG_EPI_RES_HALF 32
+#define SG_EPI_RES_PREMASK 64
 
 template <typename T> struct Epilogue {
   void* out; long long out_bstride; int ldo;
@@ -229,6 +231,13 @@
   float alpha; const float* alpha_ptr;
   int flags; int I; int J;
   long long split_stride;
+  int rWo = 0, rwshift = -1;
+
+  __device__ __forceinline__ long long res_half_row(int j) const {
+    if (rwshift >= 1) return (long long)(((j >> (rwshift + 1)) << (rwshift - 1)) + ((j & (rWo - 1)) >> 1));
+    const int w = j % rWo, t = j / rWo;
+    return (long long)(t >> 1) * (rWo >> 1) + (w >> 1);
+  }
 
   __device__ __forceinline__ void set_batch(int b) {
     if (flags & (SG_EPI_OUT_F32 | SG_EPI_ATOMIC)) out = (float*)out + (long long)b * out_bstride;
@@ -260,22 +269,25 @@
       if (bias && e < ne) x += bias[i0 + e];
       v[e] = x;
     }
-    if (mask) {
+    auto apply_mask = [&]() {
       const T* m = mask + (long long)j * ldm + i0;
 #pragma unroll
       for (int e = 0; e < 4; e++) if (e < ne) { if (!(to_f<T>(m[e]) > 0.f)) v[e] = 0.f; }
-    }
+    };
+    const bool res_first = (flags & SG_EPI_RES_PREMASK) != 0;
+    if (mask && !res_first) apply_mask();
     if (res) {
       if (flags & SG_EPI_RES_F32) {
         const float* r = (const float*)res + (long long)j * ldr + i0;
 #pragma unroll
         for (int e = 0; e < 4; e++) if (e < ne) v[e] += beta * r[e];
       } else {
-        const T* r = (const T*)res + (long long)j * ldr + i0;
+        const T* r = (const T*)res + ((flags & SG_EPI_RES_HALF) ? res_half_row(j) : (long long)j) * ldr + i0;
 #pragma unroll
         for (int e = 0; e < 4; e++) if (e < ne) v[e] += beta * to_f<T>(r[e]);
       }
     }
+    if (mask && res_first) apply_mask();
     if (flags & SG_EPI_RELU) {
 #pragma unroll
       for (int e = 0; e < 4; e++) v[e] = fmaxf(v[e], 0.f);
diff --git a/pytorch-studiogan_amd/functional/_base.py b/pytorch-studiogan_amd/functional/_base.py
--- a/pytorch-studiogan_amd/functional/_base.py
+++ b/pytorch-studiogan_amd/functional/_base.py
@@ -95,6 +95,13 @@
     def __exit__(self, *exc):
         L.call("sg_set_f32_mode", self.saved)
         return False
+
+
+def nearest_up2(t):
+    N, H, W, C = t.shape
+    y = torch.empty((N, 2 * H, 2 * W, C), dtype=t.dtype, device=t.device)
+    L.call("sg_slice_up_fwd", L.dt(t), L.ptr(t), L.ptr(y), N, H, W, C, C, 2, L.stream())
+    return y
 
 
 def conv2d_raw(x, w_ptr, Cin, Cout, R, S, stride=1, pad_h=0, pad_w=0, pix_flags=0, epi_flags=0, bias=None, res=None, mask=None,
@@ -131,6 +138,9 @@
     d.ldm = mask.shape[-1] if mask is not None else 0
     if desc is not None:
         return out
+    if (epi_flags & L.EPI_RES_HALF) and L.lib().sg_conv2d_fwd_res_half_ok(L.C.byref(d)) != 1:
+        res = nearest_up2(res)
+        d.res, d.ldr, d.epi_flags = L.ptr(res), res.shape[-1], epi_flags & ~L.EPI_RES_HALF
     L.call("sg_conv2d_fwd", d, L.stream())
     return out
 
@@ -286,4 +296,4 @@
     return dx
 
 
-__all__ = ['L', 'zeros_small', 'zeros_like_small', '_BN_FUSED_STATS', '_CBN_MERGED', '_DGRAD_SPLITK', '_SEQ', '_STATS_OFFER', '_c', '_comm', '_first_order_only', '_offer_stats', '_param_grad_wanted', '_take_stats', '_tick', 'conv2d_q_raw', 'conv2d_q_wgrad_raw', 'conv2d_raw', 'conv2d_skip_raw', 'conv2d_wgrad_raw', 'dist', 'ensure_grad', 'f32_mode', 'gemm_dgrad_rows', 'gemm_raw', 'os', 'quad_pack_raw', 'torch']
+__all__ = ['L', 'zeros_small', 'zeros_like_small', '_BN_FUSED_STATS', '_CBN_MERGED', '_DGRAD_SPLITK', '_SEQ', '_STATS_OFFER', '_c', '_comm', '_first_order_only', '_offer_stats', '_param_grad_wanted', '_take_stats', '_tick', 'conv2d_q_raw', 'conv2d_q_wgrad_raw', 'conv2d_raw', 'conv2d_skip_raw', 'nearest_up2', 'conv2d_wgrad_raw', 'dist', 'ensure_grad', 'f32_mode', 'gemm_dgrad_rows', 'gemm_raw', 'os', 'quad_pack_raw', 'torch']
diff --git a/pytorch-studiogan_amd/functional/conv.py b/pytorch-studiogan_amd/functional/conv.py
--- a/pytorch-studiogan_amd/functional/conv.py
+++ b/pytorch-studiogan_amd/functional/conv.py
@@ -26,16 +26,34 @@
 
 
 class GradLink:
-    __slots__ = ("dx", "chain", "pending")
+    __slots__ = ("dx", "chain", "pending", "half", "mask_x")
 
     def __init__(self, chain=False):
         self.dx = None
         self.chain = chain
         self.pending = 0
-
-    def take(self):
+        self.half = False
+        self.mask_x = None
+
+    def take(self, half_ok=False):
         t, self.dx = self.dx, None
+        if self.half and t is not None and not half_ok:
+            t = _up2_masked(t, self.mask_x)
+        self.half, self.mask_x = False, None
         return t
+
+
+def _up2_masked(t, mask_x):
+    t = nearest_up2(t)
+    if mask_x is not None:
+        m = torch.empty_like(t)
+        L.call("sg_relu_mask", L.dt(t), L.ptr(t), L.ptr(mask_x), L.ptr(m), t.numel(), L.stream())
+        t = m
+    return t
+
+
+def _skip_dgrad_coarse():
+    return os.environ.get("SG_SKIP_DGRAD_COARSE", "1") != "0"
 
 
 _GRAD_LINK = [os.environ.get("SG_GRAD_LINK", "1") != "0"]
@@ -78,7 +96,24 @@
                             L.PIX_UPSAMPLE if cfg.out_pool else 0, alpha=cfg.scale, dbias=dbias)
 
 
+def _conv_dgrad_coarse(dy, x, rt, slot, cfg):
+    assert cfg.R == 1 and cfg.S == 1 and cfg.stride == 1 and cfg.out_pool and not cfg.in_upsample
+    return conv2d_raw(dy, rt.bank().w_dgrad(slot, rt), rt.rows_pad, x.shape[3], 1, 1, 1, 0, 0, 0, 0, alpha=cfg.scale, ldx=dy.shape[3])
+
+
+def _conv_dgrad_res_half(dy, x, rt, slot, cfg, res, res_mask_x):
+    same_mask = res_mask_x is None or (cfg.in_relu and res_mask_x.data_ptr() == x.data_ptr() and res_mask_x.shape == x.shape)
+    quad = _quad_form(rt, cfg, x) is not None and dy.shape[3] == rt.rows_pad
+    if not same_mask or quad or cfg.in_upsample:
+        return _conv_dgrad(dy, x, rt, slot, cfg, res=_up2_masked(res, res_mask_x))
+    return _conv_dgrad_flags(dy, x, rt, slot, cfg, res, L.EPI_RES_HALF | (L.EPI_RES_PREMASK if res_mask_x is not None else 0))
+
+
 def _conv_dgrad(dy, x, rt, slot, cfg, res=None):
+    return _conv_dgrad_flags(dy, x, rt, slot, cfg, res, 0)
+
+
+def _conv_dgrad_flags(dy, x, rt, slot, cfg, res, rh):
     bank = rt.bank()
     N, Hs, Ws, Cin = x.shape
     form = _quad_form(rt, cfg, x)
@@ -91,11 +126,11 @@
     pool = cfg.out_pool
     if cfg.stride != 1:
         assert not (pool or cfg.in_upsample), "upsample / pooling fusion is stride-1 only"
-        return conv2d_raw(dy, bank.w_dgrad(slot, rt), rt.rows_pad, Cin, cfg.R, cfg.S, cfg.stride, cfg.pad_h, cfg.pad_w, L.PIX_TRANSPOSED, 0,
+        return conv2d_raw(dy, bank.w_dgrad(slot, rt), rt.rows_pad, Cin, cfg.R, cfg.S, cfg.stride, cfg.pad_h, cfg.pad_w, L.PIX_TRANSPOSED, rh,
                           mask=x if cfg.in_relu else None, res=res, transposed_out_hw=(Hin, Win), ldx=dy.shape[3])
     pf = L.PIX_UPSAMPLE if pool else 0
     ef = L.EPI_POOL if cfg.in_upsample else 0
-    return conv2d_raw(dy, bank.w_dgrad(slot, rt), rt.rows_pad, Cin, cfg.R, cfg.S, 1, cfg.R - 1 - cfg.pad_h, cfg.S - 1 - cfg.pad_w, pf, ef,
+    return conv2d_raw(dy, bank.w_dgrad(slot, rt), rt.rows_pad, Cin, cfg.R, cfg.S, 1, cfg.R - 1 - cfg.pad_h, cfg.S - 1 - cfg.pad_w, pf, ef | rh,
                       mask=x if cfg.in_relu else None, res=res, alpha=cfg.scale, ldx=dy.shape[3])
 
 
@@ -168,9 +203,10 @@
             return dx, None, None, (dy if ctx.has_res else None), None, None, None, None
         dy = _c(dy)
         dx = None
-        skip_dx = ctx.link.take() if ctx.link is not None else None
-        if ctx.needs_input_grad[0]:
-            dx = _conv_dgrad(dy, x, rt, slot, cfg, res=skip_dx)
+        half, mask_x = (ctx.link.half, ctx.link.mask_x) if ctx.link is not None else (False, None)
+        skip_dx = ctx.link.take(half_ok=True) if ctx.link is not None else None
+        if ctx.needs_input_grad[0]:
+            dx = _conv_dgrad_res_half(dy, x, rt, slot, cfg, skip_dx, mask_x) if half else _conv_dgrad(dy, x, rt, slot, cfg, res=skip_dx)
         elif skip_dx is not None:
             raise RuntimeError("GradLink: a skip gradient was handed over but this convolution's input needs no gradient")
         if ctx.link is not None and ctx.link.chain:
@@ -237,7 +273,10 @@
             shared_db = zeros_small(rt2.rows, torch.float32, dy.device)
         for inp, rt, cfg, w_i, b_i, wp, bp in ((h, rt2, cfg2, 2, 3, ctx.w2, ctx.b2), (x, rt0, cfg0, 4, 5, ctx.w0, ctx.b0)):
             k = 0 if inp is h else 1
-            outs.append(_conv_dgrad(dy, inp, rt, slot, cfg) if ctx.needs_input_grad[k] else None)
+            coarse = (k == 1 and cfg.out_pool and not cfg.in_upsample and ctx.link is not None and not ctx.link.chain and _GRAD_LINK[0] and _skip_dgrad_coarse()
+                      and inp.dtype == torch.bfloat16 and inp.shape[1] % 2 == 0 and inp.shape[2] % 2 == 0)
+            outs.append((_conv_dgrad_coarse if coarse else _conv_dgrad)(dy, inp, rt, slot, cfg) if ctx.needs_input_grad[k] else None)
+            coarse_skip = coarse and outs[-1] is not None
             want_db = bp is not None and ctx.needs_input_grad[b_i]
             db_done = False
             if ctx.needs_input_grad[w_i]:
@@ -259,7 +298,7 @@
                 g = ensure_grad(bp)
                 L.call("sg_colsum", L.dt(dy), L.ptr(dy), dy.shape[3], None, 0, dy.shape[0] * dy.shape[1] * dy.shape[2], rt.rows, L.ptr(g), 1.0, L.stream())
         if ctx.link is not None and outs[1] is not None and _GRAD_LINK[0]:
-            ctx.link.dx = outs[1]
+            ctx.link.dx, ctx.link.half, ctx.link.mask_x = outs[1], coarse_skip, (x if (coarse_skip and cfg0.in_relu) else None)
             outs[1] = None
         return (outs[0], outs[1]) + (None,) * 10
 
@@ -668,4 +707,4 @@
         return None, None, None, None
 
 
-__all__ = ['CatConvDgradFn', 'CatConvFn', 'CbnAffineFn', 'CbnAffineGroupFn', 'cbn_prefetch', '_CBN_GROUP', 'ConvCfg', 'ConvDgradFn', 'ConvFn', 'ConvSkipFn', 'ConvTransposeFn', 'EmbeddingFn', 'GradLink', 'LinearDgradFn', 'LinearFn', 'SNEmbeddingFn', 'SliceUpFn', '_GRAD_LINK', '_QUAD', '_SKIP_FUSION', '_conv_dgrad', '_conv_fwd', '_conv_wgrad', '_quad_form']
+__all__ = ['CatConvDgradFn', 'CatConvFn', 'CbnAffineFn', 'CbnAffineGroupFn', 'cbn_prefetch', '_CBN_GROUP', 'ConvCfg', 'ConvDgradFn', 'ConvFn', 'ConvSkipFn', 'ConvTransposeFn', 'EmbeddingFn', 'GradLink', 'LinearDgradFn', 'LinearFn', 'SNEmbeddingFn', 'SliceUpFn', '_GRAD_LINK', '_QUAD', '_SKIP_FUSION', '_conv_dgrad', '_conv_dgrad_coarse', '_conv_dgrad_flags', '_conv_dgrad_res_half', '_conv_fwd', '_conv_wgrad', '_quad_form']
```
